# QinLab-WFU/CLIP-based-Cross-Modal-Hashing

Measured on AMD Instinct MI355X. Metric: image+text pairs/s encoded+hashed per GPU; mAP@K eval wallclock (64-bit), higher is better.
Workload: dtype bf16

## Files before the change

### clip-based-cross-modal-hashing_amd/cmh_native.py

```python
from __future__ import annotations

import ctypes as C
import os
import threading

import torch

_HERE = os.path.dirname(os.path.abspath(__file__))
LIB_PATH = os.environ.get("CMH_LIB") or os.path.join(_HERE, "csrc", "build", "libcmh.so")

ABI_VERSION = 6
F32, BF16, FP8 = 0, 1, 2
ACT_NONE, ACT_TANH, ACT_RELU = 0, 1, 2
TIE_REFERENCE, TIE_STABLE = 0, 1


class NativeError(RuntimeError):
    pass


class BlockWeights(C.Structure):
    _fields_ = [(n, C.c_void_p) for n in (
        "in_proj_w", "in_proj_b", "out_proj_w", "out_proj_b", "ln1_w", "ln1_b", "ln2_w", "ln2_b",
        "fc_w", "fc_b", "proj_w", "proj_b",
        "in_proj_cs", "out_proj_cs", "fc_cs", "proj_cs")] + [("act_scale", C.c_float * 4)]


class GemmProblem(C.Structure):
    _fields_ = [("x", C.c_void_p), ("w", C.c_void_p), ("bias", C.c_void_p), ("residual", C.c_void_p), ("out", C.c_void_p),
                ("M", C.c_int32), ("N", C.c_int32), ("K", C.c_int32), ("m_dev", C.c_void_p), ("colscale", C.c_void_p),
                ("alpha", C.c_float), ("out_scale", C.c_float)]


class VitWeights(C.Structure):
    _fields_ = [("gemm_dtype", C.c_int32), ("resolution", C.c_int32), ("patch", C.c_int32),
                ("width", C.c_int32), ("layers", C.c_int32), ("embed_dim", C.c_int32),
                ("conv1_w", C.c_void_p), ("class_embedding", C.c_void_p),
                ("positional_embedding", C.c_void_p), ("ln_pre_w", C.c_void_p), ("ln_pre_b", C.c_void_p),
                ("ln_post_w", C.c_void_p), ("ln_post_b", C.c_void_p), ("proj_t", C.c_void_p),
                ("blocks", C.POINTER(BlockWeights))]


class TextWeights(C.Structure):
    _fields_ = [("gemm_dtype", C.c_int32), ("context_length", C.c_int32), ("vocab_size", C.c_int32),
                ("width", C.c_int32), ("layers", C.c_int32), ("embed_dim", C.c_int32),
                ("token_embedding", C.c_void_p), ("positional_embedding", C.c_void_p),
                ("ln_final_w", C.c_void_p), ("ln_final_b", C.c_void_p), ("text_projection_t", C.c_void_p),
                ("blocks", C.POINTER(BlockWeights))]


class BlockGrads(C.Structure):
    _fields_ = [(n, C.c_void_p) for n in (
        "in_proj_w", "in_proj_b", "out_proj_w", "out_proj_b", "ln1_w", "ln1_b", "ln2_w", "ln2_b",
        "fc_w", "fc_b", "proj_w", "proj_b")]


class VitGrads(C.Structure):
    _fields_ = [("conv1_w", C.c_void_p), ("class_embedding", C.c_void_p), ("positional_embedding", C.c_void_p),
                ("ln_pre_w", C.c_void_p), ("ln_pre_b", C.c_void_p), ("ln_post_w", C.c_void_p), ("ln_post_b", C.c_void_p),
                ("proj", C.c_void_p), ("blocks", C.POINTER(BlockGrads))]


class TextGrads(C.Structure):
    _fields_ = [("token_embedding", C.c_void_p), ("positional_embedding", C.c_void_p), ("ln_final_w", C.c_void_p),
                ("ln_final_b", C.c_void_p), ("text_projection", C.c_void_p), ("blocks", C.POINTER(BlockGrads))]


class AdamTensor(C.Structure):
    _fields_ = [("p", C.c_void_p), ("g", C.c_void_p), ("m", C.c_void_p), ("v", C.c_void_p), ("n", C.c_int64),
                ("lr", C.c_float), ("weight_decay", C.c_float), ("max_grad_norm", C.c_float), ("p_bf16", C.c_void_p)]


class Taps(C.Structure):
    _fields_ = [("ptrs", C.POINTER(C.c_void_p)), ("count", C.c_int32)]


_lib = None
_lock = threading.Lock()

_i32, _i64, _f, _p, _sz = C.c_int32, C.c_int64, C.c_float, C.c_void_p, C.c_size_t

SIGNATURES = {
    "cmh_last_error": (C.c_char_p, []),
    "cmh_version": (C.c_int, []),
    "cmh_vit_workspace_bytes": (_sz, [C.POINTER(VitWeights), _i32]),
    "cmh_text_workspace_bytes": (_sz, [C.POINTER(TextWeights), _i32, _i32]),
    "cmh_vit_encode": (C.c_int, [C.POINTER(VitWeights), _p, _i32, _p, _p, _sz, C.POINTER(Taps), _p]),
    "cmh_text_encode": (C.c_int, [C.POINTER(TextWeights), _p, _i32, _i32, _p, _p, _p, _sz, C.POINTER(Taps), _p]),
    "cmh_text_encode_packed": (C.c_int, [C.POINTER(TextWeights), _p, _i32, _i32, _p, _p, _p, _sz, _p]),
    "cmh_vit_calibrate_fp8": (C.c_int, [C.POINTER(VitWeights), _p, _i32, _p, _p, _p, _sz, _p]),
    "cmh_text_calibrate_fp8": (C.c_int, [C.POINTER(TextWeights), _p, _i32, _i32, _p, _p, _p, _sz, _p]),
    "cmh_linear_gemm": (C.c_int, [_i32, _p, _p, _p, _p, _p, _i32, _i32, _i32, _i32, _p]),
    "cmh_layernorm": (C.c_int, [_p, _p, _p, _p, _i32, _i32, _i32, _p]),
    "cmh_attention": (C.c_int, [_i32, _p, _p, _i32, _i32, _i32, _i32, _p, _p]),
    "cmh_gemm_tuning": (C.c_int, [_i32, _i32]),
    "cmh_set_pooled_tail": (C.c_int, [_i32]),
    "cmh_set_gemm_rows": (C.c_int, [_i32]),
    "cmh_set_gemm_grouped": (C.c_int, [_i32]),
    "cmh_set_gemm_lc": (C.c_int, [_i32]),
    "cmh_gemm_route": (C.c_int, [_i32] * 8),
    "cmh_gemm_plan": (C.c_int, [_i32, _i32, C.POINTER(_i32), C.POINTER(_i32), C.POINTER(_i32)]),
    "cmh_set_grad_stream16": (C.c_int, [_i32]),
    "cmh_set_text_token_packing": (C.c_int, [_i32]),
    "cmh_linear_gemm_grouped": (C.c_int, [_i32, C.POINTER(GemmProblem), C.POINTER(GemmProblem), _i32, _p]),
    "cmh_clip_encode_pair": (C.c_int, [C.POINTER(VitWeights), _p, C.POINTER(TextWeights), _p, _i32, _i32, _i32, _p, _p, _p, _p, _sz, _p, _sz, _p]),
    "cmh_clip_encode_pair2": (C.c_int, [C.POINTER(VitWeights), _p, _i32, _p, _i32, C.POINTER(TextWeights), _p, _i32, _i32, _p, _p, _p, _p, _sz, _p, _sz, _p]),
    "cmh_msl_workspace_bytes": (_sz, [_i32]),
    "cmh_msl_loss": (C.c_int, [_p, _p, _p, _i32, _i32, _i32, _p, _p, _sz, _p]),
    "cmh_msl_loss_backward": (C.c_int, [_p, _p, _p, _i32, _i32, _i32, _p, _p, _p, _p, _sz, _p]),
    "cmh_spl_workspace_bytes": (_sz, [_i32]),
    "cmh_spl_loss": (C.c_int, [_p, _p, _p, _i32, _i32, _i32, _f, _f, _p, _p, _sz, _p]),
    "cmh_spl_loss_backward": (C.c_int, [_p, _p, _p, _i32, _i32, _i32, _f, _f, _p, _p, _p, _p, _sz, _p]),
    "cmh_qmi_workspace_bytes": (_sz, [_i32]),
    "cmh_qmi_loss": (C.c_int, [_p, _p, _p, _i32, _i32, _i32, _f, _p, _p, _p, _sz, _p]),
    "cmh_qmi_loss_backward": (C.c_int, [_p, _p, _p, _i32, _i32, _i32, _f, _p, _p, _p, _p, _p, _sz, _p]),
    "cmh_fp8_quantize_weight": (C.c_int, [_p, _p, _p, _i32, _i32, _p]),
    "cmh_fp8_quantize": (C.c_int, [_p, _i32, _p, _i64, _f, _p]),
    "cmh_fp8_dequantize": (C.c_int, [_p, _p, _i64, _f, _p]),
    "cmh_amax": (C.c_int, [_p, _i32, _i64, _p, _p]),
    "cmh_linear_gemm_fp8": (C.c_int, [_p, _p, _p, _f, _p, _p, _p, _f, _i32, _i32, _i32, _i32, _p]),
    "cmh_prof_gemm_begin": (C.c_int, [_i32]),
    "cmh_prof_gemm_end": (C.c_int, [C.POINTER(C.c_double), C.POINTER(C.c_double), C.POINTER(C.c_int64)]),
    "cmh_prof_gemm_by_kernel": (C.c_int, [C.POINTER(C.c_double), C.POINTER(C.c_double), C.POINTER(C.c_int64)]),
    "cmh_cast_f32_to_bf16": (C.c_int, [_p, _p, _i64, _p]),
    "cmh_linear_act": (C.c_int, [_p, _p, _p, _p, _f, _i32, _p, _i32, _i32, _i32, _p]),
    "cmh_pair_softmax": (C.c_int, [_p, _p, _i32, _i32, _p]),
    "cmh_sign_codes": (C.c_int, [_p, _p, _i64, _p]),
    "cmh_pair_argmax_codes": (C.c_int, [_p, _p, _i32, _i32, _p]),
    "cmh_pack_codes": (C.c_int, [_p, _i64, _i32, _p, _p, _p, _p]),
    "cmh_unpack_codes": (C.c_int, [_p, _p, _i64, _i32, _p, _p]),
    "cmh_map_mean": (C.c_int, [_p, _i32, _p, _p]),
    "cmh_pack_labels": (C.c_int, [_p, _i64, _i32, _p, _p, _p]),
    "cmh_hamming_dist": (C.c_int, [_p, _p, _p, _p, _i32, _i64, _i32, _p, _p]),
    "cmh_calc_neighbor": (C.c_int, [_p, _p, _i32, _i32, _i32, _p, _p]),
    "cmh_map_workspace_bytes": (_sz, [_i32, _i64, _i32, _i32]),
    "cmh_hamming_map": (C.c_int, [_p, _p, _p, _p, _p, _p, _i32, _i64, _i32, _i32, _i64, _i32, _i32, _p, _p, _p,
                                  _p, _sz, _p]),
    "cmh_retrieval_workspace_bytes": (_sz, [_i32, _i64, _i32]),
    "cmh_hamming_hist": (C.c_int, [_p, _p, _p, _p, _p, _p, _i32, _i64, _i32, _i32, _p, _p, _sz, _p]),
    "cmh_hamming_topk": (C.c_int, [_p, _p, _p, _p, _p, _p, _i32, _i64, _i32, _i32, _i64, _p, _p, _p, _p, _p, _sz, _p]),
    "cmh_hamming_topk_graded": (C.c_int, [_p, _p, _p, _p, _p, _p, _i32, _i64, _i32, _i32, _i64, _p, _p, _p, _p, _p, _p, _sz, _p]),
    "cmh_label_overlap_workspace_bytes": (_sz, [_i32, _i64, _i32]),
    "cmh_label_overlap_hist": (C.c_int, [_p, _p, _i32, _i64, _i32, _p, _p, _sz, _p]),
    "cmh_loss_workspace_bytes": (_sz, [_i32, _i32, _i32]),
    "cmh_dsph_hyp_loss": (C.c_int, [_p, _p, _p, _p, _i32, _i32, _i32, _f, _f, _p, _p, _sz, _p]),
    "cmh_dchmt_loss": (C.c_int, [_p, _p, _p, _i32, _i32, _i32, _i32, _i32, _i32, _f, _f, _p, _p, _sz, _p]),
    "cmh_batchnorm1d_train": (C.c_int, [_p, _p, _p, _f, _p, _i32, _i32, _p]),
    "cmh_twdh_targets": (C.c_int, [_p, _p, _p, _p, _i32, _i32, _i32, _p]),
    "cmh_twdh_loss": (C.c_int, [_p, _p, _p, _i32, _i32, _p, _p, _sz, _p]),
    "cmh_dnph_loss": (C.c_int, [_p, _p, _p, _p, _p, _p, _p, _p, _i32, _i32, _i32, _f, _f, _p, _p, _sz, _p]),
    "cmh_vit_encode_tokens": (C.c_int, [C.POINTER(VitWeights), _p, _i32, _p, _p, _sz, _p]),
    "cmh_text_encode_tokens": (C.c_int, [C.POINTER(TextWeights), _p, _i32, _i32, _p, _p, _p, _p, _sz, _p]),
    "cmh_text_encode_tokens_packed": (C.c_int, [C.POINTER(TextWeights), _p, _i32, _i32, _p, _p, _p, _p, _sz, _p]),
    "cmh_blocks_workspace_bytes": (_sz, [_i32, _i32, _i32, _i32]),
    "cmh_transformer_blocks": (C.c_int, [C.POINTER(BlockWeights), _i32, _i32, _p, _i32, _i32, _i32, _i32, _p, _p, _sz, _p]),
    "cmh_mith_lta": (C.c_int, [_p, _p, _p, _p, _i32, _i32, _i32, _i32, _i32, _i32, _i32, _p]),
    "cmh_add_positional": (C.c_int, [_p, _p, _i32, _i32, _i32, _p]),
    "cmh_bitwise_hash": (C.c_int, [_p, _p, _p, _p, _i32, _i32, _i32, _p]),
    "cmh_l2_normalize_rows": (C.c_int, [_p, _p, _i32, _i32, _p]),
    "cmh_mith_mix": (C.c_int, [_p, _p, _p, _p, _f, _p, _p, _p, _i64, _p]),
    "cmh_sq_diff_sum": (C.c_int, [_p, _p, _i64, _p, _p, _sz, _p]),
    "cmh_mith_bayesian_loss": (C.c_int, [_p, _p, _p, _p, _i32, _i32, _i32, _i32, _p, _p, _sz, _p]),
    "cmh_info_nce": (C.c_int, [_p, _p, _i32, _i32, _i32, _f, _p, _p, _sz, _p]),
    "cmh_transpose": (C.c_int, [_p, _i32, _p, _i32, _i32, _i32, _p]),
    "cmh_colsum_workspace_bytes": (_sz, [_i32, _i32]),
    "cmh_colsum": (C.c_int, [_p, _i32, _i32, _i32, _p, _p, _sz, _p]),
    "cmh_layernorm_backward_workspace_bytes": (_sz, [_i32, _i32]),
    "cmh_layernorm_backward": (C.c_int, [_p, _i32, _p, _i32, _p, _i32, _i32, _p, _i32, _p, _p, _p, _sz, _p]),
    "cmh_quick_gelu": (C.c_int, [_p, _p, _i64, _i32, _p]),
    "cmh_attention_backward": (C.c_int, [_i32, _p, _p, _p, _p, _i32, _i32, _i32, _i32, _p, _p]),
    "cmh_linear_wgrad_workspace_bytes": (_sz, [_i32, _i32, _i32, _i32]),
    "cmh_linear_wgrad": (C.c_int, [_i32, _p, _i32, _p, _i32, _i32, _i32, _i32, _p, _p, _p, _sz, _p]),
    "cmh_linear_act_backward": (C.c_int, [_p, _p, _p, _p, _p, _f, _i32, _p, _p, _p, _i32, _i32, _i32, _p, _sz, _p]),
    "cmh_head_backward_workspace_bytes": (_sz, [_i32, _i32, _i32]),
    "cmh_pair_softmax_backward": (C.c_int, [_p, _p, _p, _i32, _i32, _p]),
    "cmh_dchmt_loss_backward": (C.c_int, [_p, _p, _p, _i32, _i32, _i32, _i32, _i32, _i32, _f, _f, _p, _p, _p, _p, _sz, _p]),
    "cmh_dsph_hyp_loss_backward": (C.c_int, [_p, _p, _p, _p, _i32, _i32, _i32, _f, _f, _p, _p, _p, _p, _p, _sz, _p]),
    "cmh_dnph_backward_workspace_bytes": (_sz, [_i32, _i32, _i32]),
    "cmh_dnph_loss_backward": (C.c_int, [_p] * 8 + [_i32, _i32, _i32, _f, _f, _p] + [_p] * 5 + [_p, _sz, _p]),
    "cmh_image_preprocess_workspace_bytes": (_sz, [_i32, _i32, _i32, _i32]),
    "cmh_image_preprocess": (C.c_int, [_p, _p, _p, _i32, _i32, _i32, _i32, _i32, C.POINTER(C.c_float), C.POINTER(C.c_float),
                                       _p, _p, _p, _sz, _p]),
    "cmh_vit_forward_train_tokens": (C.c_int, [C.POINTER(VitWeights), _p, _i32, _p, _p, _sz, _p]),
    "cmh_vit_backward_tokens": (C.c_int, [C.POINTER(VitWeights), _i32, _p, C.POINTER(VitGrads), _p, _sz, _p]),
    "cmh_text_forward_train_tokens": (C.c_int, [C.POINTER(TextWeights), _p, _i32, _i32, _p, _p, _p, _p, _sz, _p]),
    "cmh_text_forward_train_tokens_packed": (C.c_int, [C.POINTER(TextWeights), _p, _i32, _i32, _p, _p, _p, _p, _sz, _p]),
    "cmh_text_backward_tokens": (C.c_int, [C.POINTER(TextWeights), _p, _i32, _i32, _p, _p, C.POINTER(TextGrads), _p, _sz, _p]),
    "cmh_blocks_train_bytes": (_sz, [_i32, _i32, _i32, _i32, _i32]),
    "cmh_blocks_forward_train": (C.c_int, [C.POINTER(BlockWeights), _i32, _i32, _p, _p, _i32, _i32, _i32, _p, _sz, _p]),
    "cmh_blocks_backward": (C.c_int, [C.POINTER(BlockWeights), C.POINTER(BlockGrads), _i32, _i32, _p, _p, _i32, _i32, _i32, _p, _sz, _p]),
    "cmh_mith_lta_backward": (C.c_int, [_p, _p, _p, _p, _i32, _i32, _i32, _i32, _i32, _i32, _i32, _p]),
    "cmh_gelu": (C.c_int, [_p, _p, C.c_int64, _p]),
    "cmh_gelu_backward": (C.c_int, [_p, _p, _p, C.c_int64, _p]),
    "cmh_l2_normalize_backward": (C.c_int, [_p, _p, _p, _i32, _i32, _p]),
    "cmh_bitwise_hash_backward": (C.c_int, [_p, _p, _p, _p, _p, _p, _p, _i32, _i32, _i32, _p]),
    "cmh_mith_bayesian_backward_workspace_bytes": (_sz, [_i32, _i32]),
    "cmh_info_nce_workspace_bytes": (_sz, [_i32, _i32]),
    "cmh_mith_bayesian_loss_backward": (C.c_int, [_p, _p, _p, _p, _i32, _i32, _i32, _i32, _p, _p, _p, _sz, _p]),
    "cmh_info_nce_backward": (C.c_int, [_p, _p, _i32, _i32, _i32, _f, _p, _p, _p, _p, _sz, _p]),
    "cmh_sq_diff_sum_backward": (C.c_int, [_p, _p, C.c_int64, _p, _p, _p, _p]),
    "cmh_batchnorm1d_update_running": (C.c_int, [_p, _f, _p, _p, _i32, _i32, _p]),
    "cmh_batchnorm1d_backward": (C.c_int, [_p, _p, _f, _p, _p, _p, _p, _i32, _i32, _p]),
    "cmh_twdh_loss_backward": (C.c_int, [_p, _p, _p, _i32, _i32, _p, _p, _p, _p, _p]),
    "cmh_image_normalize": (C.c_int, [_p, _p, _i32, _i32, C.POINTER(C.c_float), C.POINTER(C.c_float), _p, _p]),
    "cmh_bpe_create": (C.c_int, [C.c_char_p, _sz, C.POINTER(_p)]),
    "cmh_bpe_destroy": (None, [_p]),
    "cmh_bpe_vocab_size": (_i32, [_p]),
    "cmh_bpe_encode_captions": (C.c_int, [_p, C.c_char_p, _p, _i32, _i32, _p, _p, _i32]),
    "cmh_vit_train_bytes": (_sz, [C.POINTER(VitWeights), _i32]),
    "cmh_vit_forward_train": (C.c_int, [C.POINTER(VitWeights), _p, _i32, _p, _p, _sz, _p]),
    "cmh_vit_backward": (C.c_int, [C.POINTER(VitWeights), _i32, _p, C.POINTER(VitGrads), _p, _sz, _p]),
    "cmh_vit_backward_part": (C.c_int, [C.POINTER(VitWeights), _i32, _p, C.POINTER(VitGrads), _p, _sz, _i32, _i32, _p]),
    "cmh_text_train_bytes": (_sz, [C.POINTER(TextWeights), _i32, _i32]),
    "cmh_text_forward_train": (C.c_int, [C.POINTER(TextWeights), _p, _i32, _i32, _p, _p, _p, _sz, _p]),
    "cmh_text_backward": (C.c_int, [C.POINTER(TextWeights), _p, _i32, _i32, _p, _p, C.POINTER(TextGrads), _p, _sz, _p]),
    "cmh_text_backward_part": (C.c_int, [C.POINTER(TextWeights), _p, _i32, _i32, _p, _p, C.POINTER(TextGrads), _p, _sz, _i32, _i32, _p]),
    "cmh_bert_adam_workspace_bytes": (_sz, [_i32, _i64]),
    "cmh_bert_adam_step": (C.c_int, [C.POINTER(AdamTensor), _i32, C.c_double, C.c_double, C.c_double, _p, _sz, _p]),
}


def lib():
    global _lib
    with _lock:
        if _lib is None:
            if not os.path.exists(LIB_PATH):
                raise NativeError(
                    f"{LIB_PATH} is missing: build it with `python __graft_entry__.py` (or `make -C "
                    f"{os.path.dirname(os.path.dirname(LIB_PATH))}`); there is no CPU fallback for the hot path")
            l = C.CDLL(LIB_PATH)
            for name, (res, args) in SIGNATURES.items():
                fn = getattr(l, name)
                fn.restype, fn.argtypes = res, args
            if l.cmh_version() != ABI_VERSION:
                raise NativeError(f"{LIB_PATH}: cmh_version() = {l.cmh_version()}, this binding was written for {ABI_VERSION}; rebuild it")
            _lib = l
    return _lib


def check(rc: int, what: str):
    if rc != 0:
        raise NativeError(f"{what} failed (code {rc}): {lib().cmh_last_error().decode(errors='replace')}")


def require_gpu(*tensors):
    for t in tensors:
        if t is not None and not t.is_cuda:
            raise NativeError("libcmh runs on the GPU only (tensor on %s); there is no CPU fallback" % t.device)


def ptr(t):
    return None if t is None else C.c_void_p(t.data_ptr())


def stream_ptr(device=None):
    return C.c_void_p(torch.cuda.current_stream(device).cuda_stream)


_ws_cache: dict = {}


def workspace(nbytes: int, device, tag: str = "") -> torch.Tensor:
    key = (str(device), int(torch.cuda.current_stream(device).cuda_stream) if torch.cuda.is_available() else 0, tag)
    buf = _ws_cache.get(key)
    if buf is None or buf.numel() < nbytes:
        buf = torch.empty(max(int(nbytes), 256), dtype=torch.uint8, device=device)
        _ws_cache[key] = buf
    return buf


def f32c(t: torch.Tensor) -> torch.Tensor:
    if t.dtype != torch.float32:
        t = t.float()
    return t.contiguous()


def cast_bf16(src: torch.Tensor) -> torch.Tensor:
    src = f32c(src)
    require_gpu(src)
    dst = torch.empty(src.shape, dtype=torch.bfloat16, device=src.device)
    check(lib().cmh_cast_f32_to_bf16(ptr(src), ptr(dst), src.numel(), stream_ptr(src.device)), "cmh_cast_f32_to_bf16")
    return dst


def _kind(t: torch.Tensor) -> int:
    return {torch.float32: 0, torch.bfloat16: 1, torch.float16: 2}[t.dtype]


def fp8_quantize_weight(w: torch.Tensor):
    w = f32c(w)
    require_gpu(w)
    Nn, K = w.shape
    q = torch.empty(Nn, K, dtype=torch.uint8, device=w.device)
    cs = torch.empty(Nn, dtype=torch.float32, device=w.device)
    check(lib().cmh_fp8_quantize_weight(ptr(w), ptr(q), ptr(cs), Nn, K, stream_ptr(w.device)), "cmh_fp8_quantize_weight")
    return q, cs


def fp8_quantize(x: torch.Tensor, scale: float) -> torch.Tensor:
    require_gpu(x)
    x = x.contiguous()
    q = torch.empty(x.shape, dtype=torch.uint8, device=x.device)
    check(lib().cmh_fp8_quantize(ptr(x), _kind(x), ptr(q), x.numel(), float(scale), stream_ptr(x.device)), "cmh_fp8_quantize")
    return q


def fp8_dequantize(q: torch.Tensor, scale: float = 1.0) -> torch.Tensor:
    require_gpu(q)
    q = q.contiguous()
    out = torch.empty(q.shape, dtype=torch.float32, device=q.device)
    check(lib().cmh_fp8_dequantize(ptr(q), ptr(out), q.numel(), float(scale), stream_ptr(q.device)), "cmh_fp8_dequantize")
    return out


def amax(x: torch.Tensor, into: torch.Tensor | None = None) -> torch.Tensor:
    require_gpu(x)
    x = x.contiguous()
    out = torch.zeros(1, dtype=torch.float32, device=x.device) if into is None else into
    check(lib().cmh_amax(ptr(x), _kind(x), x.numel(), ptr(out), stream_ptr(x.device)), "cmh_amax")
    return out


EPI_OUT_FP8 = 4096


def linear_gemm_fp8(x8, w8, colscale, alpha, bias=None, residual=None, quickgelu=False, out="f32", out_scale=1.0):
    require_gpu(x8, w8, colscale, bias, residual)
    if x8.dtype != torch.uint8 or w8.dtype != torch.uint8:
        raise NativeError("linear_gemm_fp8: operands are e4m3 bytes (uint8 tensors)")
    x8, w8 = x8.contiguous(), w8.contiguous()
    M, K = x8.shape
    Nn = w8.shape[0]
    if w8.shape[1] != K or colscale.numel() != Nn or (bias is not None and bias.numel() != Nn) or \
            (residual is not None and tuple(residual.shape) != (M, Nn)):
        raise NativeError(f"linear_gemm_fp8: x {tuple(x8.shape)}, w {tuple(w8.shape)}, colscale / bias / residual shapes do not fit together")
    odt = {"f32": torch.float32, "bf16": torch.bfloat16, "f16": torch.float16, "fp8": torch.uint8}[out]
    o = torch.empty(M, Nn, dtype=odt, device=x8.device)
    res_f16 = residual is not None and residual.dtype == torch.float16
    if residual is not None:
        residual = residual.contiguous() if res_f16 else f32c(residual)
    epi = (EPI_BIAS if bias is not None else 0) | (EPI_QUICKGELU if quickgelu else 0) | (EPI_RESIDUAL if residual is not None else 0) | \
          (EPI_RES_F16 if res_f16 else 0) | {"f32": 0, "bf16": EPI_OUT_BF16, "f16": EPI_OUT_F16, "fp8": EPI_OUT_FP8}[out]
    check(lib().cmh_linear_gemm_fp8(ptr(x8), ptr(w8), ptr(f32c(colscale)), float(alpha), ptr(None if bias is None else f32c(bias)),
                                    ptr(residual), ptr(o), float(out_scale), M, Nn, K, epi, stream_ptr(x8.device)), "cmh_linear_gemm_fp8")
    return o


def set_gemm_grouped(on: int = -1):
    check(lib().cmh_set_gemm_grouped(int(on)), "cmh_set_gemm_grouped")


def linear_gemm_grouped(problems, quickgelu=False, out="f32", m_dev=(None, None)):
    assert len(problems) == 2
    kinds = {("u8" if p["x"].dtype == torch.uint8 else ("bf16" if p["x"].dtype == torch.bfloat16 else "f32")) for p in problems}
    if len(kinds) != 1:
        raise NativeError("linear_gemm_grouped: both problems must share the operand type")
    kind = kinds.pop()
    dt = {"f32": F32, "bf16": BF16, "u8": FP8}[kind]
    odt = {"f32": torch.float32, "bf16": torch.bfloat16, "f16": torch.float16, "fp8": torch.uint8}[out]
    has_bias = problems[0].get("bias") is not None
    has_res = problems[0].get("residual") is not None
    res_f16 = has_res and problems[0]["residual"].dtype == torch.float16
    epi = (EPI_BIAS if has_bias else 0) | (EPI_QUICKGELU if quickgelu else 0) | (EPI_RESIDUAL if has_res else 0) | \
          (EPI_RES_F16 if res_f16 else 0) | {"f32": 0, "bf16": EPI_OUT_BF16, "f16": EPI_OUT_F16, "fp8": EPI_OUT_FP8}[out]
    structs, outs, keep = [], [], []
    for p, md in zip(problems, m_dev):
        x, w = p["x"].contiguous(), p["w"].contiguous()
        require_gpu(x, w, p.get("bias"), p.get("residual"), p.get("colscale"), md)
        M, K = x.shape
        Nn = w.shape[0]
        if w.shape[1] != K or (p.get("bias") is not None) != has_bias or (p.get("residual") is not None) != has_res or \
                (has_bias and p["bias"].numel() != Nn) or (has_res and tuple(p["residual"].shape) != (M, Nn)) or \
                (kind == "u8" and (p.get("colscale") is None or p["colscale"].numel() != Nn)):
            raise NativeError(f"linear_gemm_grouped: x {tuple(x.shape)}, w {tuple(w.shape)}: operand shapes / kinds do not fit together")
        o = torch.empty(M, Nn, dtype=odt, device=x.device)
        bias = f32c(p["bias"]) if has_bias else None
        res = None
        if has_res:
            res = p["residual"].contiguous() if res_f16 else f32c(p["residual"])
        cs = f32c(p["colscale"]) if kind == "u8" else None
        g = GemmProblem(ptr(x), ptr(w), ptr(bias), ptr(res), ptr(o), M, Nn, K, ptr(md), ptr(cs), float(p.get("alpha", 1.0)),
                        float(p.get("out_scale", 1.0)))
        structs.append(g)
        outs.append(o)
        keep += [x, w, bias, res, cs]
    check(lib().cmh_linear_gemm_grouped(dt, C.byref(structs[0]), C.byref(structs[1]), epi, stream_ptr(outs[0].device)),
          "cmh_linear_gemm_grouped")
    return outs


def set_pooled_tail(on: bool):
    check(lib().cmh_set_pooled_tail(1 if on else 0), "cmh_set_pooled_tail")


def set_gemm_rows(on: int = -1):
    check(lib().cmh_set_gemm_rows(int(on)), "cmh_set_gemm_rows")


def set_text_token_packing(on: int):
    check(lib().cmh_set_text_token_packing(int(on)), "cmh_set_text_token_packing")


def set_grad_stream16(on: int):
    check(lib().cmh_set_grad_stream16(int(on)), "cmh_set_grad_stream16")


def set_gemm_lc(mode: int):
    check(lib().cmh_set_gemm_lc(int(mode)), "cmh_set_gemm_lc")


def gemm_route(a, b=None, epi=0, dt=None):
    mb, nb, kb = b if b is not None else (0, 0, 0)
    rc = lib().cmh_gemm_route(BF16 if dt is None else dt, *a, mb, nb, kb, int(epi))
    if rc < 0:
        raise NativeError(f"cmh_gemm_route: {lib().cmh_last_error()}")
    return rc


PLAN_FIELDS = ("family", "rows", "grid", "order", "dge", "res", "grouped")


def gemm_plan(a, b=None, epi=0, dt=None):
    def five(s):
        return (_i32 * 5)(*(tuple(s) + (0, 0))[:5])
    out = (_i32 * 16)()
    check(lib().cmh_gemm_plan(BF16 if dt is None else dt, int(epi), five(a), None if b is None else five(b), out), "cmh_gemm_plan")
    return out[1], [dict(zip(PLAN_FIELDS, out[2 + 7 * i:9 + 7 * i])) for i in range(out[0])]


def gemm_tuning(tile_rows: int = -1, order_group: int = -1):
    check(lib().cmh_gemm_tuning(int(tile_rows), int(order_group)), "cmh_gemm_tuning")


def prof_gemm_begin(max_launches: int):
    check(lib().cmh_prof_gemm_begin(int(max_launches)), "cmh_prof_gemm_begin")


def prof_gemm_end():
    ms, fl, n = C.c_double(), C.c_double(), C.c_int64()
    check(lib().cmh_prof_gemm_end(C.byref(ms), C.byref(fl), C.byref(n)), "cmh_prof_gemm_end")
    return ms.value, fl.value, n.value


def prof_gemm_by_kernel():
    ms, fl, n = (C.c_double * 3)(), (C.c_double * 3)(), (C.c_int64 * 3)()
    check(lib().cmh_prof_gemm_by_kernel(ms, fl, n), "cmh_prof_gemm_by_kernel")
    return {k: (ms[i], fl[i], n[i]) for i, k in enumerate(("gemm_wide_kernel", "gemm_rows_kernel", "fallback"))}


EPI_BIAS, EPI_QUICKGELU, EPI_RESIDUAL, EPI_OUT_BF16 = 1, 2, 4, 8
EPI_RES_F16, EPI_OUT_F16 = 64, 128


def linear_gemm(x, w, bias=None, residual=None, quickgelu=False, out_bf16=False, out_f16=False):
    require_gpu(x, w, bias, residual)
    dt = BF16 if x.dtype == torch.bfloat16 else F32
    if (w.dtype == torch.bfloat16) != (dt == BF16):
        raise NativeError("linear_gemm: x and w must share a dtype")
    if out_bf16 and out_f16:
        raise NativeError("linear_gemm: out_bf16 and out_f16 exclude each other")
    x, w = x.contiguous(), w.contiguous()
    M, K = x.shape
    Nn = w.shape[0]
    if w.dim() != 2 or w.shape[1] != K or (bias is not None and bias.numel() != Nn) or \
            (residual is not None and tuple(residual.shape) != (M, Nn)):
        raise NativeError(f"linear_gemm: x {tuple(x.shape)}, w {tuple(w.shape)}, bias / residual shapes do not fit together")
    odt = torch.bfloat16 if out_bf16 else (torch.float16 if out_f16 else torch.float32)
    out = torch.empty(M, Nn, dtype=odt, device=x.device)
    res_f16 = residual is not None and residual.dtype == torch.float16
    if residual is not None:
        residual = residual.contiguous() if res_f16 else f32c(residual)
    epi = (EPI_BIAS if bias is not None else 0) | (EPI_QUICKGELU if quickgelu else 0) | \
          (EPI_RESIDUAL if residual is not None else 0) | (EPI_OUT_BF16 if out_bf16 else 0) | \
          (EPI_RES_F16 if res_f16 else 0) | (EPI_OUT_F16 if out_f16 else 0)
    check(lib().cmh_linear_gemm(dt, ptr(x), ptr(w), ptr(None if bias is None else f32c(bias)), ptr(residual), ptr(out),
                                M, Nn, K, epi, stream_ptr(x.device)), "cmh_linear_gemm")
    return out


def layernorm(x, w, b, out_bf16=False):
    x, w, b = f32c(x), f32c(w), f32c(b)
    require_gpu(x, w, b)
    M, d = x.shape
    if w.numel() != d or b.numel() != d:
        raise NativeError(f"layernorm: rows of {d} elements, weight {tuple(w.shape)}, bias {tuple(b.shape)}")
    out = torch.empty(M, d, dtype=torch.bfloat16 if out_bf16 else torch.float32, device=x.device)
    check(lib().cmh_layernorm(ptr(x), ptr(w), ptr(b), ptr(out), BF16 if out_bf16 else F32, M, d, stream_ptr(x.device)),
          "cmh_layernorm")
    return out


def attention(qkv, B, T, causal, key_padding_mask=None):
    require_gpu(qkv, key_padding_mask)
    qkv = qkv.contiguous()
    dt = BF16 if qkv.dtype == torch.bfloat16 else F32
    d = qkv.shape[1] // 3
    o = torch.empty(B * T, d, dtype=qkv.dtype, device=qkv.device)
    kpm = None if key_padding_mask is None else key_padding_mask.to(torch.uint8).contiguous()
    check(lib().cmh_attention(dt, ptr(qkv), ptr(o), B, T, d, int(bool(causal)), ptr(kpm), stream_ptr(qkv.device)),
          "cmh_attention")
    return o


def linear_act(x, w, b, act=ACT_NONE, drop_mask=None, p=0.2):
    x, w = f32c(x), f32c(w)
    b = None if b is None else f32c(b)
    require_gpu(x, w, b, drop_mask)
    M, K = x.shape
    N = w.shape[0]
    if w.shape[1] != K:
        raise NativeError(f"linear_act: x [{M},{K}] vs w {tuple(w.shape)}")
    y = torch.empty(M, N, dtype=torch.float32, device=x.device)
    dm = None if drop_mask is None else f32c(drop_mask)
    check(lib().cmh_linear_act(ptr(x), ptr(w), ptr(b), ptr(dm), 1.0 / (1.0 - p), act, ptr(y), M, N, K,
                               stream_ptr(x.device)), "cmh_linear_act")
    return y


def pair_softmax(z):
    z = f32c(z)
    require_gpu(z)
    M, K2 = z.shape
    out = torch.empty_like(z)
    check(lib().cmh_pair_softmax(ptr(z), ptr(out), M, K2 // 2, stream_ptr(z.device)), "cmh_pair_softmax")
    return out


def sign_codes(h):
    h = f32c(h)
    require_gpu(h)
    out = torch.empty_like(h)
    check(lib().cmh_sign_codes(ptr(h), ptr(out), h.numel(), stream_ptr(h.device)), "cmh_sign_codes")
    return out


def pair_argmax_codes(p):
    p = f32c(p)
    require_gpu(p)
    M, K2 = p.shape
    out = torch.empty(M, K2 // 2, dtype=torch.float32, device=p.device)
    check(lib().cmh_pair_argmax_codes(ptr(p), ptr(out), M, K2 // 2, stream_ptr(p.device)), "cmh_pair_argmax_codes")
    return out


def pack_codes(codes, validate=True):
    codes = f32c(codes)
    require_gpu(codes)
    n, K = codes.shape
    W = (K + 31) // 32
    sp = torch.empty(n, W, dtype=torch.int32, device=codes.device)
    nz = torch.empty(n, W, dtype=torch.int32, device=codes.device)
    bad = torch.zeros(1, dtype=torch.int32, device=codes.device)
    check(lib().cmh_pack_codes(ptr(codes), n, K, ptr(sp), ptr(nz), ptr(bad), stream_ptr(codes.device)), "cmh_pack_codes")
    if validate and int(bad.item()):
        raise NativeError("pack_codes: hash codes must be exactly -1, 0 or +1 (sign()/argmax codes)")
    return sp, nz


def unpack_codes(sign_plane, nz_plane, bits: int):
    require_gpu(sign_plane, nz_plane)
    sp, nz = sign_plane.contiguous(), nz_plane.contiguous()
    n, W = sp.shape
    if sp.dtype != torch.int32 or nz.dtype != torch.int32 or tuple(nz.shape) != (n, W) or W != (int(bits) + 31) // 32:
        raise NativeError(f"unpack_codes: planes {tuple(sp.shape)} / {tuple(nz.shape)} do not hold {bits}-bit codes")
    out = torch.empty(n, int(bits), dtype=torch.float32, device=sp.device)
    if n:
        check(lib().cmh_unpack_codes(ptr(sp), ptr(nz), n, int(bits), ptr(out), stream_ptr(sp.device)), "cmh_unpack_codes")
    return out


def map_mean(ap):
    ap = f32c(ap)
    require_gpu(ap)
    out = torch.empty(1, dtype=torch.float32, device=ap.device)
    check(lib().cmh_map_mean(ptr(ap), ap.numel(), ptr(out), stream_ptr(ap.device)), "cmh_map_mean")
    return out[0]


def pack_labels(labels):
    labels = f32c(labels)
    require_gpu(labels)
    n, Cn = labels.shape
    LW = (Cn + 31) // 32
    out = torch.empty(n, LW, dtype=torch.int32, device=labels.device)
    bad = torch.zeros(1, dtype=torch.int32, device=labels.device)
    check(lib().cmh_pack_labels(ptr(labels), n, Cn, ptr(out), ptr(bad), stream_ptr(labels.device)), "cmh_pack_labels")
    if int(bad.item()):
        raise NativeError("pack_labels: labels must be non-negative (multi-hot)")
    return out


def hamming_dist(q_planes, r_planes, bits):
    (qs, qn), (rs, rn) = q_planes, r_planes
    Q, N = qs.shape[0], rs.shape[0]
    W = (bits + 31) // 32
    fit("hamming_dist", (qs, (Q, W)), (qn, (Q, W)), (rs, (N, W)), (rn, (N, W)))
    out = torch.empty(Q, N, dtype=torch.float32, device=qs.device)
    check(lib().cmh_hamming_dist(ptr(qs), ptr(qn), ptr(rs), ptr(rn), Q, N, bits, ptr(out), stream_ptr(qs.device)),
          "cmh_hamming_dist")
    return out


def calc_neighbor(la, lb, classes):
    A, B = la.shape[0], lb.shape[0]
    fit("calc_neighbor", (la, (A, (classes + 31) // 32)), (lb, (B, (classes + 31) // 32)))
    out = torch.empty(A, B, dtype=torch.float32, device=la.device)
    check(lib().cmh_calc_neighbor(ptr(la), ptr(lb), A, B, classes, ptr(out), stream_ptr(la.device)), "cmh_calc_neighbor")
    return out


def hamming_map(q_planes, q_lab, r_planes, r_lab, bits, classes, topk=None, tie_order=TIE_REFERENCE,
                want_perm=False, depth_limit=-1):
    (qs, qn), (rs, rn) = q_planes, r_planes
    dev = qs.device
    Q, N = qs.shape[0], rs.shape[0]
    W, LW = (bits + 31) // 32, (classes + 31) // 32
    fit("hamming_map", (qs, (Q, W)), (qn, (Q, W)), (rs, (N, W)), (rn, (N, W)), (q_lab, (Q, LW)), (r_lab, (N, LW)))
    ap = torch.empty(Q, dtype=torch.float32, device=dev)
    mp = torch.empty(1, dtype=torch.float32, device=dev)
    perm = torch.empty(Q, N, dtype=torch.int32, device=dev) if want_perm else None
    need = lib().cmh_map_workspace_bytes(Q, N, bits, tie_order)
    ws = workspace(need, dev, "map")
    check(lib().cmh_hamming_map(ptr(qs), ptr(qn), ptr(q_lab), ptr(rs), ptr(rn), ptr(r_lab), Q, N, bits, classes,
                                0 if topk is None else int(topk), tie_order, depth_limit, ptr(ap), ptr(mp), ptr(perm),
                                ptr(ws), ws.numel(), stream_ptr(dev)), "cmh_hamming_map")
    return mp[0], ap, perm


def _retrieval_operands(what, q_planes, r_planes, bits, q_lab, r_lab):
    (qs, qn), (rs, rn) = q_planes, r_planes
    require_gpu(qs, qn, rs, rn, q_lab, r_lab)
    Q, N = qs.shape[0], rs.shape[0]
    W = (int(bits) + 31) // 32
    if (q_lab is None) != (r_lab is None):
        raise NativeError(f"{what}: labels on one side only")
    LW = 0 if q_lab is None else q_lab.shape[1]
    fit(what, (qs, (Q, W)), (qn, (Q, W)), (rs, (N, W)), (rn, (N, W)), (q_lab, (Q, LW)), (r_lab, (N, LW)))
    for t in (qs, qn, rs, rn, q_lab, r_lab):
        if t is not None and (t.dtype != torch.int32 or not t.is_contiguous()):
            raise NativeError(f"{what}: packed operands are contiguous int32 tensors (pack_codes / pack_labels)")
    return qs, qn, rs, rn, Q, N, LW


def hamming_hist(q_planes, r_planes, bits, q_lab=None, r_lab=None):
    qs, qn, rs, rn, Q, N, LW = _retrieval_operands("hamming_hist", q_planes, r_planes, bits, q_lab, r_lab)
    dev = qs.device
    counts = torch.empty(Q, 2 * int(bits) + 1, 2, dtype=torch.int32, device=dev)
    ws = workspace(lib().cmh_retrieval_workspace_bytes(Q, N, int(bits)), dev, "retrieval")
    check(lib().cmh_hamming_hist(ptr(qs), ptr(qn), ptr(q_lab), ptr(rs), ptr(rn), ptr(r_lab), Q, N, int(bits), 32 * LW,
                                 ptr(counts), ptr(ws), ws.numel(), stream_ptr(dev)), "cmh_hamming_hist")
    return counts


def hamming_topk(q_planes, r_planes, bits, k, q_lab=None, r_lab=None, want_counts=False):
    qs, qn, rs, rn, Q, N, LW = _retrieval_operands("hamming_topk", q_planes, r_planes, bits, q_lab, r_lab)
    dev = qs.device
    k = int(k)
    if not 1 <= k <= N:
        raise NativeError(f"hamming_topk: k={k} outside [1, N={N}]")
    idx = torch.empty(Q, k, dtype=torch.int32, device=dev)
    dist = torch.empty(Q, k, dtype=torch.float32, device=dev)
    rel = torch.empty(Q, k, dtype=torch.uint8, device=dev) if LW else None
    counts = torch.empty(Q, 2 * int(bits) + 1, 2, dtype=torch.int32, device=dev) if want_counts else None
    ws = workspace(lib().cmh_retrieval_workspace_bytes(Q, N, int(bits)), dev, "retrieval")
    check(lib().cmh_hamming_topk(ptr(qs), ptr(qn), ptr(q_lab), ptr(rs), ptr(rn), ptr(r_lab), Q, N, int(bits), 32 * LW, k,
                                 ptr(idx), ptr(dist), ptr(rel), ptr(counts), ptr(ws), ws.numel(), stream_ptr(dev)),
          "cmh_hamming_topk")
    return (idx, dist, rel, counts) if want_counts else (idx, dist, rel)


GRADE_CLASSES_MAX = 255


def _grade_classes(what, classes, LW):
    classes = min(32 * LW, GRADE_CLASSES_MAX) if classes is None else int(classes)
    if classes < 1 or (classes + 31) // 32 != LW:
        raise NativeError(f"{what}: classes={classes} does not fit label operands of {LW} words")
    return classes


def hamming_topk_graded(q_planes, r_planes, bits, k, q_lab, r_lab, want_counts=False, classes=None):
    if q_lab is None or r_lab is None:
        raise NativeError("hamming_topk_graded: needs the labels of both sides")
    qs, qn, rs, rn, Q, N, LW = _retrieval_operands("hamming_topk_graded", q_planes, r_planes, bits, q_lab, r_lab)
    dev = qs.device
    k = int(k)
    if not 1 <= k <= N:
        raise NativeError(f"hamming_topk_graded: k={k} outside [1, N={N}]")
    classes = _grade_classes("hamming_topk_graded", classes, LW)
    idx = torch.empty(Q, k, dtype=torch.int32, device=dev)
    dist = torch.empty(Q, k, dtype=torch.float32, device=dev)
    grade = torch.empty(Q, k, dtype=torch.uint8, device=dev)
    counts = torch.empty(Q, 2 * int(bits) + 1, 2, dtype=torch.int32, device=dev) if want_counts else None
    ws = workspace(lib().cmh_retrieval_workspace_bytes(Q, N, int(bits)), dev, "retrieval")
    check(lib().cmh_hamming_topk_graded(ptr(qs), ptr(qn), ptr(q_lab), ptr(rs), ptr(rn), ptr(r_lab), Q, N, int(bits), classes, k,
                                        ptr(idx), ptr(dist), None, ptr(grade), ptr(counts), ptr(ws), ws.numel(), stream_ptr(dev)),
          "cmh_hamming_topk_graded")
    return (idx, dist, grade, counts) if want_counts else (idx, dist, grade)


def label_overlap_hist(q_lab, r_lab, classes):
    if q_lab is None or r_lab is None:
        raise NativeError("label_overlap_hist: needs the labels of both sides")
    require_gpu(q_lab, r_lab)
    classes = int(classes)
    Q, N, LW = q_lab.shape[0], r_lab.shape[0], (classes + 31) // 32
    fit("label_overlap_hist", (q_lab, (Q, LW)), (r_lab, (N, LW)))
    for t in (q_lab, r_lab):
        if t.dtype != torch.int32 or not t.is_contiguous():
            raise NativeError("label_overlap_hist: packed operands are contiguous int32 tensors (pack_labels)")
    dev = q_lab.device
    out = torch.empty(Q, classes + 1, dtype=torch.int32, device=dev)
    ws = workspace(lib().cmh_label_overlap_workspace_bytes(Q, N, classes), dev, "retrieval")
    check(lib().cmh_label_overlap_hist(ptr(q_lab), ptr(r_lab), Q, N, classes, ptr(out), ptr(ws), ws.numel(), stream_ptr(dev)),
          "cmh_label_overlap_hist")
    return out


def fit(what, *pairs):
    for t, shape in pairs:
        if t is not None and tuple(t.shape) != tuple(shape):
            raise NativeError(f"{what}: operand of shape {tuple(t.shape)} where {tuple(shape)} is expected")


def dsph_hyp_loss(x, y, label, proxies, threshold, alpha):
    x, y, label, proxies = f32c(x), f32c(y), f32c(label), f32c(proxies)
    require_gpu(x, y, label, proxies)
    B, K = x.shape
    Cn = label.shape[1]
    fit("dsph_hyp_loss", (y, (B, K)), (label, (B, Cn)), (proxies, (Cn, K)))
    out = torch.empty(1, dtype=torch.float32, device=x.device)
    ws = workspace(lib().cmh_loss_workspace_bytes(B, K, Cn), x.device, "loss")
    check(lib().cmh_dsph_hyp_loss(ptr(x), ptr(y), ptr(label), ptr(proxies), B, K, Cn, float(threshold), float(alpha),
                                  ptr(out), ptr(ws), ws.numel(), stream_ptr(x.device)), "cmh_dsph_hyp_loss")
    return out[0]


def msl_loss(feats, labels, feat2=None):
    feats, labels = f32c(feats), f32c(labels)
    feat2 = None if feat2 is None else f32c(feat2)
    require_gpu(feats, labels, feat2)
    B, K = feats.shape
    fit("msl_loss", (labels, (B, labels.shape[1])))
    if feat2 is not None:
        fit("msl_loss", (feat2, (B, K)))
    out = torch.empty(1, dtype=torch.float32, device=feats.device)
    ws = workspace(lib().cmh_msl_workspace_bytes(B), feats.device, "loss")
    check(lib().cmh_msl_loss(ptr(feats), ptr(feat2), ptr(labels), B, K, labels.shape[1], ptr(out), ptr(ws), ws.numel(),
                             stream_ptr(feats.device)), "cmh_msl_loss")
    return out[0]


def msl_loss_backward(feats, labels, feat2, dloss):
    B, K = feats.shape
    dfeats = torch.empty_like(feats)
    dfeat2 = None if feat2 is None else torch.empty_like(feat2)
    ws = workspace(lib().cmh_msl_workspace_bytes(B), feats.device, "loss")
    check(lib().cmh_msl_loss_backward(ptr(feats), ptr(feat2), ptr(labels), B, K, labels.shape[1], ptr(f32c(dloss).reshape(1)),
                                      ptr(dfeats), ptr(dfeat2), ptr(ws), ws.numel(), stream_ptr(feats.device)), "cmh_msl_loss_backward")
    return dfeats, dfeat2


def spl_loss(a, b, labels, temperature, delta):
    a, labels = f32c(a), f32c(labels)
    b = None if b is None else f32c(b)
    require_gpu(a, labels, b)
    B, K = a.shape
    fit("spl_loss", (labels, (B, labels.shape[1])), (b, (B, K)))
    out = torch.empty(1, dtype=torch.float32, device=a.device)
    ws = workspace(lib().cmh_spl_workspace_bytes(B), a.device, "loss")
    check(lib().cmh_spl_loss(ptr(a), ptr(b), ptr(labels), B, K, labels.shape[1], float(temperature), float(delta), ptr(out), ptr(ws),
                             ws.numel(), stream_ptr(a.device)), "cmh_spl_loss")
    return out[0]


def spl_loss_backward(a, b, labels, temperature, delta, dloss):
    B, K = a.shape
    da = torch.empty_like(a)
    db = None if b is None else torch.empty_like(b)
    ws = workspace(lib().cmh_spl_workspace_bytes(B), a.device, "loss")
    check(lib().cmh_spl_loss_backward(ptr(a), ptr(b), ptr(labels), B, K, labels.shape[1], float(temperature), float(delta),
                                      ptr(f32c(dloss).reshape(1)), ptr(da), ptr(db), ptr(ws), ws.numel(), stream_ptr(a.device)),
          "cmh_spl_loss_backward")
    return da, db


def qmi_loss(img, txt, label, eps=1e-8):
    img, txt, label = f32c(img), f32c(txt), f32c(label)
    require_gpu(img, txt, label)
    B, K = img.shape
    Cn = label.shape[1]
    fit("qmi_loss", (txt, (B, K)), (label, (B, Cn)))
    packed = pack_labels(label)
    out = torch.empty(1, dtype=torch.float32, device=img.device)
    sum_d = torch.empty(1, dtype=torch.float32, device=img.device)
    ws = workspace(lib().cmh_qmi_workspace_bytes(B), img.device, "loss")
    check(lib().cmh_qmi_loss(ptr(img), ptr(txt), ptr(packed), B, K, Cn, float(eps), ptr(out), ptr(sum_d), ptr(ws), ws.numel(),
                             stream_ptr(img.device)), "cmh_qmi_loss")
    return out[0], sum_d, packed


def qmi_loss_backward(img, txt, packed, classes, sum_d, dloss, eps=1e-8):
    B, K = img.shape
    dimg, dtxt = torch.empty_like(img), torch.empty_like(txt)
    ws = workspace(lib().cmh_qmi_workspace_bytes(B), img.device, "loss")
    check(lib().cmh_qmi_loss_backward(ptr(img), ptr(txt), ptr(packed), B, K, int(classes), float(eps), ptr(sum_d), ptr(f32c(dloss).reshape(1)),
# ... 93 lines not shown
```

### clip-based-cross-modal-hashing_amd/csrc/attention.hip

```cpp
#include "cmh_common.h"

namespace cmh {

constexpr int HD = 64;
constexpr int KT = 32;

template <typename T>
__device__ __forceinline__ void load_row64(const T* __restrict__ p, float (&dst)[HD], float scale);

template <>
__device__ __forceinline__ void load_row64<float>(const float* __restrict__ p, float (&dst)[HD], float scale) {
#pragma unroll
  for (int i = 0; i < HD / 4; ++i) {
    const float4 v = *reinterpret_cast<const float4*>(p + 4 * i);
    dst[4 * i + 0] = v.x * scale; dst[4 * i + 1] = v.y * scale;
    dst[4 * i + 2] = v.z * scale; dst[4 * i + 3] = v.w * scale;
  }
}
template <>
__device__ __forceinline__ void load_row64<bf16_t>(const bf16_t* __restrict__ p, float (&dst)[HD], float scale) {
#pragma unroll
  for (int i = 0; i < HD / 8; ++i) {
    const uint4 v = *reinterpret_cast<const uint4*>(p + 8 * i);
    const uint32_t w[4] = {v.x, v.y, v.z, v.w};
#pragma unroll
    for (int j = 0; j < 4; ++j) {
      dst[8 * i + 2 * j + 0] = __uint_as_float(w[j] << 16) * scale;
      dst[8 * i + 2 * j + 1] = __uint_as_float(w[j] & 0xffff0000u) * scale;
    }
  }
}

template <typename T>
__global__ __launch_bounds__(64) void attention_kernel(const T* __restrict__ qkv, T* __restrict__ o, int B, int Tmax,
                                                       int d, int causal, const uint8_t* __restrict__ kpm,
                                                       const int32_t* __restrict__ seq_off) {
  __shared__ __attribute__((aligned(16))) float sK[KT][HD];
  __shared__ __attribute__((aligned(16))) float sV[KT][HD];

  const int lane = threadIdx.x;
  const int heads = d / HD;
  const int b = blockIdx.x / heads, h = blockIdx.x - b * heads;
  const int Tn = seq_off ? seq_off[b + 1] - seq_off[b] : Tmax;
  const size_t srow = seq_off ? static_cast<size_t>(seq_off[b]) : static_cast<size_t>(b) * Tmax;
  const int q0 = blockIdx.y * 64;
  const int row = q0 + lane;
  const bool active = row < Tn;
  const size_t ld = static_cast<size_t>(3) * d;
  const T* base = qkv + srow * ld + h * HD;

  float q[HD], acc[HD];
#pragma unroll
  for (int i = 0; i < HD; ++i) acc[i] = 0.f;
  if (active) {
    load_row64<T>(base + static_cast<size_t>(row) * ld, q, 0.125f);
  } else {
#pragma unroll
    for (int i = 0; i < HD; ++i) q[i] = 0.f;
  }
  float m = -1e30f, l = 0.f;

  const int last_row = (q0 + 63 < Tn ? q0 + 63 : Tn - 1);
  const int k_end = causal ? last_row + 1 : Tn;

  for (int k0 = 0; k0 < k_end; k0 += KT) {
    __syncthreads();
#pragma unroll
    for (int it = 0; it < KT * HD / 4 / 64; ++it) {
      const int slot = it * 64 + lane;
      const int kr = slot >> 4, c4 = slot & 15;
      const int kg = k0 + kr;
      float4 kv = float4{0.f, 0.f, 0.f, 0.f}, vv = kv;
      if (kg < Tn) {
        const T* kp = base + static_cast<size_t>(kg) * ld + d + c4 * 4;
        const T* vp = kp + d;
        if constexpr (sizeof(T) == 4) {
          kv = *reinterpret_cast<const float4*>(kp);
          vv = *reinterpret_cast<const float4*>(vp);
        } else {
          const uint2 a = *reinterpret_cast<const uint2*>(kp);
          const uint2 c = *reinterpret_cast<const uint2*>(vp);
          kv = float4{__uint_as_float(a.x << 16), __uint_as_float(a.x & 0xffff0000u),
                      __uint_as_float(a.y << 16), __uint_as_float(a.y & 0xffff0000u)};
          vv = float4{__uint_as_float(c.x << 16), __uint_as_float(c.x & 0xffff0000u),
                      __uint_as_float(c.y << 16), __uint_as_float(c.y & 0xffff0000u)};
        }
      }
      *reinterpret_cast<float4*>(&sK[kr][c4 * 4]) = kv;
      *reinterpret_cast<float4*>(&sV[kr][c4 * 4]) = vv;
    }
    __syncthreads();

    float s[KT];
    float tmax = -1e30f;
#pragma unroll
    for (int j = 0; j < KT; ++j) {
      float a0 = 0.f, a1 = 0.f, a2 = 0.f, a3 = 0.f;
#pragma unroll
      for (int i = 0; i < HD / 4; ++i) {
        const float4 kv = *reinterpret_cast<const float4*>(&sK[j][4 * i]);
        a0 = fmaf(q[4 * i + 0], kv.x, a0);
        a1 = fmaf(q[4 * i + 1], kv.y, a1);
        a2 = fmaf(q[4 * i + 2], kv.z, a2);
        a3 = fmaf(q[4 * i + 3], kv.w, a3);
      }
      const int kg = k0 + j;
      bool ok = kg < Tn && (!causal || kg <= row);
      if (kpm && kg < Tn) ok = ok && (kpm[static_cast<size_t>(b) * Tmax + kg] == 0);
      s[j] = ok ? (a0 + a1) + (a2 + a3) : -1e30f;
      tmax = fmaxf(tmax, s[j]);
    }
    const float m_new = fmaxf(m, tmax);
    const float alpha = expf(m - m_new);
    l *= alpha;
#pragma unroll
    for (int i = 0; i < HD; ++i) acc[i] *= alpha;
#pragma unroll
    for (int j = 0; j < KT; ++j) {
      const float p = s[j] > -1e29f ? expf(s[j] - m_new) : 0.f;
      l += p;
#pragma unroll
      for (int i = 0; i < HD / 4; ++i) {
        const float4 vv = *reinterpret_cast<const float4*>(&sV[j][4 * i]);
        acc[4 * i + 0] = fmaf(p, vv.x, acc[4 * i + 0]);
        acc[4 * i + 1] = fmaf(p, vv.y, acc[4 * i + 1]);
        acc[4 * i + 2] = fmaf(p, vv.z, acc[4 * i + 2]);
        acc[4 * i + 3] = fmaf(p, vv.w, acc[4 * i + 3]);
      }
    }
    m = m_new;
  }

  if (!active) return;
  const float inv = 1.0f / l;
  T* op = o + (srow + row) * d + h * HD;
  if constexpr (sizeof(T) == 4) {
#pragma unroll
    for (int i = 0; i < HD / 4; ++i)
      *reinterpret_cast<float4*>(op + 4 * i) =
          float4{acc[4 * i] * inv, acc[4 * i + 1] * inv, acc[4 * i + 2] * inv, acc[4 * i + 3] * inv};
  } else {
#pragma unroll
    for (int i = 0; i < HD / 8; ++i) {
      uint4 pk;
      uint32_t w[4];
#pragma unroll
      for (int j = 0; j < 4; ++j)
        w[j] = static_cast<uint32_t>(f32_to_bf16(acc[8 * i + 2 * j] * inv)) |
               (static_cast<uint32_t>(f32_to_bf16(acc[8 * i + 2 * j + 1] * inv)) << 16);
      pk.x = w[0]; pk.y = w[1]; pk.z = w[2]; pk.w = w[3];
      *reinterpret_cast<uint4*>(op + 8 * i) = pk;
    }
  }
}

typedef __attribute__((ext_vector_type(8))) __bf16 abf16x8_t;
typedef __attribute__((ext_vector_type(4))) float af32x4_t;

constexpr int kAttnVST = 80;

template <int NKT>
__device__ __forceinline__ void attention_mfma_body(const bf16_t* __restrict__ qkv, bf16_t* __restrict__ o, int Tmax, int d, int causal,
                                                    const uint8_t* __restrict__ kpm, const int32_t* __restrict__ seq_off,
                                                    float o8_inv_scale, int block, bf16_t* sV) {
  constexpr int NKS = NKT / 2;
  constexpr int TP = NKT * 16;
  constexpr int VST = kAttnVST;

  const int lane = threadIdx.x, g = lane >> 4, c = lane & 15;
  const int heads = d / HD;
  const int b = block / heads, h = block - b * heads;
  const int Tn = seq_off ? __builtin_amdgcn_readfirstlane(seq_off[b + 1] - seq_off[b]) : Tmax;
  const size_t srow = seq_off ? static_cast<size_t>(__builtin_amdgcn_readfirstlane(seq_off[b])) : static_cast<size_t>(b) * Tmax;
  const size_t ld = static_cast<size_t>(3) * d;
  const bf16_t* base = qkv + srow * ld + h * HD;
  if (Tn <= 0) return;

  abf16x8_t kf[NKT][2];
#pragma unroll
  for (int kt = 0; kt < NKT; ++kt) {
    int row = kt * 16 + c;
    row = row < Tn ? row : Tn - 1;
#pragma unroll
    for (int s = 0; s < 2; ++s)
      kf[kt][s] = *reinterpret_cast<const abf16x8_t*>(base + static_cast<size_t>(row) * ld + d + s * 32 + g * 8);
  }
  constexpr int VIT = TP * 8 / 64;
  constexpr int VB = NKT == 8 ? 8 : VIT;
  uint4 vst[VB];
  auto load_v = [&](int i0) {
#pragma unroll
    for (int i = 0; i < VB; ++i) {
      const int slot = lane + 64 * (i0 + i), row = slot >> 3, ch = slot & 7;
      const int rc = row < Tn ? row : Tn - 1;
      vst[i] = *reinterpret_cast<const uint4*>(base + static_cast<size_t>(rc) * ld + 2 * d + ch * 8);
    }
  };
  auto store_v = [&](int i0) {
#pragma unroll
    for (int i = 0; i < VB; ++i) {
      const int slot = lane + 64 * (i0 + i), row = slot >> 3, ch = slot & 7;
      *reinterpret_cast<uint4*>(&sV[row * VST + ch * 8]) = row < Tn ? vst[i] : uint4{0u, 0u, 0u, 0u};
    }
  };
  load_v(0);
  uint32_t padded = 0;
  if (kpm) {
    uint8_t kb[NKT][4];
#pragma unroll
    for (int kt = 0; kt < NKT; ++kt)
#pragma unroll
      for (int r = 0; r < 4; ++r) {
        const int key = kt * 16 + 4 * g + r;
        kb[kt][r] = kpm[static_cast<size_t>(b) * Tmax + (key < Tn ? key : Tn - 1)];
      }
#pragma unroll
    for (int kt = 0; kt < NKT; ++kt)
#pragma unroll
      for (int r = 0; r < 4; ++r) padded |= (kb[kt][r] != 0 ? 1u : 0u) << (kt * 4 + r);
  }
  store_v(0);
  if constexpr (VB < VIT) { load_v(VB); store_v(VB); }
  uint32_t keyok = 0;
#pragma unroll
  for (int kt = 0; kt < NKT; ++kt)
#pragma unroll
    for (int r = 0; r < 4; ++r) {
      const int key = kt * 16 + 4 * g + r;
      const bool ok = key < Tn && !((padded >> (kt * 4 + r)) & 1u);
      keyok |= (ok ? 1u : 0u) << (kt * 4 + r);
    }
  uint32_t tile_all = 0, tile_none = 0;
#pragma unroll
  for (int kt = 0; kt < NKT; ++kt) {
    const uint32_t bits = (keyok >> (kt * 4)) & 15u;
    if (__ballot(bits != 15u) == 0) tile_all |= 1u << kt;
    if (__ballot(bits != 0u) == 0) tile_none |= 1u << kt;
  }
  uint32_t diagok = 0;
#pragma unroll
  for (int r = 0; r < 4; ++r) diagok |= (4 * g + r <= c ? 1u : 0u) << r;
  __syncthreads();
  abf16x8_t vf[NKS][4];
  {
    typedef __attribute__((address_space(3))) void* lptr_t;
    const uint32_t a0 = static_cast<uint32_t>(reinterpret_cast<uintptr_t>((lptr_t)sV)) +
                        static_cast<uint32_t>(((4 * g + (c >> 2)) * VST + 4 * (c & 3)) * 2);
    uint2 raw[NKS][4][2];
#pragma unroll
    for (int s = 0; s < NKS; ++s)
#pragma unroll
      for (int dt = 0; dt < 4; ++dt)
#pragma unroll
        for (int hh = 0; hh < 2; ++hh)
          asm volatile("ds_read_b64_tr_b16 %0, %1 offset:%2"
                       : "=v"(raw[s][dt][hh])
                       : "v"(a0), "i"((32 * s + 16 * hh) * VST * 2 + 32 * dt));
#pragma unroll
    for (int s = 0; s < NKS; ++s) {
      asm volatile("s_waitcnt lgkmcnt(0)"
                   : "+v"(raw[s][0][0]), "+v"(raw[s][0][1]), "+v"(raw[s][1][0]), "+v"(raw[s][1][1]), "+v"(raw[s][2][0]),
                     "+v"(raw[s][2][1]), "+v"(raw[s][3][0]), "+v"(raw[s][3][1]));
#pragma unroll
      for (int dt = 0; dt < 4; ++dt)
        vf[s][dt] = __builtin_bit_cast(abf16x8_t, uint4{raw[s][dt][0].x, raw[s][dt][0].y, raw[s][dt][1].x, raw[s][dt][1].y});
    }
  }

#if defined(ATT_ABL) && ATT_ABL == 3
  {
    float keep = 0.f;
#pragma unroll
    for (int s = 0; s < NKS; ++s)
#pragma unroll
      for (int dt = 0; dt < 4; ++dt) keep += static_cast<float>(vf[s][dt][0]);
#pragma unroll
    for (int kt = 0; kt < NKT; ++kt) keep += static_cast<float>(kf[kt][0][0]) + static_cast<float>(kf[kt][1][0]);
    if (keep == 123.456f) o[0] = 1;
    return;
  }
#endif
  const int nqt = (Tn + 15) >> 4;
  auto load_q = [&](int qt, abf16x8_t (&q)[2]) {
    const int qrow = qt * 16 + c;
    const int qr = qrow < Tn ? qrow : Tn - 1;
#pragma unroll
    for (int s = 0; s < 2; ++s) q[s] = *reinterpret_cast<const abf16x8_t*>(base + static_cast<size_t>(qr) * ld + s * 32 + g * 8);
  };
  abf16x8_t qn[2];
  load_q(0, qn);
  for (int qt = 0; qt < nqt; ++qt) {
    const int qrow = qt * 16 + c;
    abf16x8_t qf[2] = {qn[0], qn[1]};
    load_q(qt + 1, qn);
    af32x4_t sc[NKT];
#pragma unroll
    for (int kt = 0; kt < NKT; ++kt) {
      if ((causal && kt > qt) || ((tile_none >> kt) & 1u)) {
        sc[kt] = af32x4_t{-1e30f, -1e30f, -1e30f, -1e30f};
      } else {
        sc[kt] = af32x4_t{0.f, 0.f, 0.f, 0.f};
#pragma unroll
        for (int s = 0; s < 2; ++s) sc[kt] = __builtin_amdgcn_mfma_f32_16x16x32_bf16(kf[kt][s], qf[s], sc[kt], 0, 0, 0);
        uint32_t okb = (keyok >> (kt * 4)) & 15u;
        if (causal && kt == qt) okb &= diagok;
        if (!((tile_all >> kt) & 1u) || (causal && kt == qt)) {
#pragma unroll
          for (int r = 0; r < 4; ++r) sc[kt][r] = ((okb >> r) & 1u) ? sc[kt][r] : -1e30f;
        }
      }
    }
    float m = -1e30f;
#pragma unroll
    for (int kt = 0; kt < NKT; ++kt) m = fmaxf(fmaxf(m, fmaxf(sc[kt][0], sc[kt][1])), fmaxf(sc[kt][2], sc[kt][3]));
    m = fmaxf(m, __shfl_xor(m, 16, 64));
    m = fmaxf(m, __shfl_xor(m, 32, 64));
    typedef __attribute__((ext_vector_type(2))) float af32x2_t;
    const float kC = 0.18033688011112042f;
    const af32x2_t mc = {-m * kC, -m * kC}, cc = {kC, kC};
    af32x2_t l2 = {0.f, 0.f};
#pragma unroll
    for (int kt = 0; kt < NKT; ++kt)
#pragma unroll
      for (int r = 0; r < 4; r += 2) {
        const af32x2_t e = __builtin_elementwise_fma(af32x2_t{sc[kt][r], sc[kt][r + 1]}, cc, mc);
        const af32x2_t p = {__builtin_amdgcn_exp2f(e[0]), __builtin_amdgcn_exp2f(e[1])};
        sc[kt][r] = p[0];
        sc[kt][r + 1] = p[1];
        l2 += p;
      }
    float l = l2[0] + l2[1];
    l += __shfl_xor(l, 16, 64);
    l += __shfl_xor(l, 32, 64);
    l = m > -1e29f ? l : 0.f;
    af32x4_t oc[4];
#pragma unroll
    for (int dt = 0; dt < 4; ++dt) oc[dt] = af32x4_t{0.f, 0.f, 0.f, 0.f};
#pragma unroll
    for (int s = 0; s < NKS; ++s) {
      abf16x8_t pb;
#pragma unroll
      for (int j = 0; j < 8; ++j) pb[j] = static_cast<__bf16>(sc[2 * s + (j >> 2)][j & 3]);
#pragma unroll
      for (int dt = 0; dt < 4; ++dt) oc[dt] = __builtin_amdgcn_mfma_f32_16x16x32_bf16(vf[s][dt], pb, oc[dt], 0, 0, 0);
    }
#if defined(ATT_ABL) && (ATT_ABL == 1 || ATT_ABL == 2)
    {
      float keep = l;
#pragma unroll
      for (int dt = 0; dt < 4; ++dt) keep += oc[dt][0] + oc[dt][1] + oc[dt][2] + oc[dt][3];
      if (keep == 123.456f) o[0] = 1;
      continue;
    }
#endif
    if (qrow < Tn && o8_inv_scale > 0.f) {
      const float inv = o8_inv_scale / l;
      uint8_t* op8 = reinterpret_cast<uint8_t*>(o) + (srow + qrow) * d + h * HD + 4 * g;
#pragma unroll
      for (int dt = 0; dt < 4; ++dt) {
        auto cl = [](float v) { return fminf(fmaxf(v, -448.f), 448.f); };
        int w = __builtin_amdgcn_cvt_pk_fp8_f32(cl(oc[dt][0] * inv), cl(oc[dt][1] * inv), 0, false);
        w = __builtin_amdgcn_cvt_pk_fp8_f32(cl(oc[dt][2] * inv), cl(oc[dt][3] * inv), w, true);
        *reinterpret_cast<uint32_t*>(op8 + 16 * dt) = static_cast<uint32_t>(w);
      }
    } else {
      const float inv = 1.0f / l;
      bf16_t* op = o + (srow + (qrow < Tn ? qrow : Tn - 1)) * d + h * HD + (g & 1) * 16 + (g & 2) * 4;
#pragma unroll
      for (int pr = 0; pr < 2; ++pr) {
        uint32_t lo[2], hi[2];
#pragma unroll
        for (int w = 0; w < 2; ++w) {
          lo[w] = pack_bf16x2(oc[2 * pr][2 * w] * inv, oc[2 * pr][2 * w + 1] * inv);
          hi[w] = pack_bf16x2(oc[2 * pr + 1][2 * w] * inv, oc[2 * pr + 1][2 * w + 1] * inv);
        }
        typedef __attribute__((ext_vector_type(2))) unsigned au2_t;
        const au2_t s0 = __builtin_amdgcn_permlane16_swap(lo[0], hi[0], false, false);
        const au2_t s1 = __builtin_amdgcn_permlane16_swap(lo[1], hi[1], false, false);
        if (qrow < Tn) *reinterpret_cast<uint4*>(op + 32 * pr) = uint4{s0[0], s1[0], s0[1], s1[1]};
      }
    }
  }
}

template <int NKT>
__global__ __launch_bounds__(64) void attention_mfma_kernel(const bf16_t* __restrict__ qkv, bf16_t* __restrict__ o,
                                                            int B, int Tmax, int d, int causal,
                                                            const uint8_t* __restrict__ kpm,
                                                            const int32_t* __restrict__ seq_off, float o8_inv_scale) {
  __shared__ __attribute__((aligned(16))) bf16_t sV[NKT * 16 * kAttnVST];
  (void)B;
  attention_mfma_body<NKT>(qkv, o, Tmax, d, causal, kpm, seq_off, o8_inv_scale, blockIdx.x, sV);
}

template <int NKT>
static void launch_attention_mfma(const void* qkv, void* o, int B, int T, int d, int causal, const uint8_t* kpm,
                                  const int32_t* seq_off, hipStream_t st, float o8_inv_scale) {
  hipLaunchKernelGGL(attention_mfma_kernel<NKT>, dim3(B * (d / HD)), dim3(64), 0, st, static_cast<const bf16_t*>(qkv),
                     static_cast<bf16_t*>(o), B, T, d, causal, kpm, seq_off, o8_inv_scale);
}

int launch_attention(const void* qkv, void* o, int dt, int B, int T, int d, int causal,
                     const uint8_t* key_padding_mask, hipStream_t st) {
  return launch_attention_varlen(qkv, o, dt, B, T, d, causal, key_padding_mask, nullptr, st, 0.f);
}

int launch_attention_varlen(const void* qkv, void* o, int dt, int B, int T, int d, int causal,
                            const uint8_t* key_padding_mask, const int32_t* seq_off, hipStream_t st, float o8_inv_scale) {
  CMH_CHECK_ARG(d % HD == 0, "attention: width %d is not a multiple of 64", d);
  CMH_CHECK_ARG(B > 0 && T > 0, "attention: empty batch");
  CMH_CHECK_ARG(o8_inv_scale == 0.f || (dt == CMH_BF16 && T <= 128), "attention: e4m3 output needs bf16 qkv and T <= 128 (T=%d)", T);
  const dim3 grid(B * (d / HD), (T + 63) / 64);
  if (dt == CMH_BF16 && T <= 128) {
    if (T <= 32) launch_attention_mfma<2>(qkv, o, B, T, d, causal, key_padding_mask, seq_off, st, o8_inv_scale);
    else if (T <= 64) launch_attention_mfma<4>(qkv, o, B, T, d, causal, key_padding_mask, seq_off, st, o8_inv_scale);
    else if (T <= 96) launch_attention_mfma<6>(qkv, o, B, T, d, causal, key_padding_mask, seq_off, st, o8_inv_scale);
    else launch_attention_mfma<8>(qkv, o, B, T, d, causal, key_padding_mask, seq_off, st, o8_inv_scale);
    CMH_CHECK_LAUNCH("attention_mfma");
    return CMH_OK;
  }
  if (dt == CMH_F32)
    hipLaunchKernelGGL(attention_kernel<float>, grid, dim3(64), 0, st, static_cast<const float*>(qkv),
                       static_cast<float*>(o), B, T, d, causal, key_padding_mask, seq_off);
  else
    hipLaunchKernelGGL(attention_kernel<bf16_t>, grid, dim3(64), 0, st, static_cast<const bf16_t*>(qkv),
                       static_cast<bf16_t*>(o), B, T, d, causal, key_padding_mask, seq_off);
  CMH_CHECK_LAUNCH("attention");
  return CMH_OK;
}

}
```

### clip-based-cross-modal-hashing_amd/csrc/cmh_common.h

```cpp
#pragma once

#include <hip/hip_runtime.h>
#include <stdint.h>

#include <cstdarg>
#include <cstdio>

#include "../../include/cmh.h"

namespace cmh {

char* err_buf();
int fail(int code, const char* fmt, ...);

#define CMH_CHECK_ARG(cond, ...) \
  do {                           \
    if (!(cond)) return ::cmh::fail(CMH_ERR_INVALID, __VA_ARGS__); \
  } while (0)

#define CMH_CHECK_LAUNCH(what)                                                            \
  do {                                                                                    \
    hipError_t e__ = hipGetLastError();                                                   \
    if (e__ != hipSuccess)                                                                \
      return ::cmh::fail(CMH_ERR_LAUNCH, "%s: %s", what, hipGetErrorString(e__));          \
  } while (0)

static inline hipStream_t as_stream(void* s) { return reinterpret_cast<hipStream_t>(s); }
static inline size_t align_up(size_t x, size_t a) { return (x + a - 1) / a * a; }

typedef uint16_t bf16_t;

__device__ __forceinline__ float bf16_to_f32(bf16_t v) {
  return __uint_as_float(static_cast<uint32_t>(v) << 16);
}
__device__ __forceinline__ bf16_t f32_to_bf16(float f) {
  uint32_t u = __float_as_uint(f);
  if ((u & 0x7fffffffu) > 0x7f800000u) return static_cast<bf16_t>((u >> 16) | 0x40);
  u += 0x7fffu + ((u >> 16) & 1u);
  return static_cast<bf16_t>(u >> 16);
}

__device__ __forceinline__ uint32_t pack_bf16x2(float a, float b) {
  typedef __attribute__((ext_vector_type(2))) float f2_t;
  typedef __attribute__((ext_vector_type(2))) __bf16 b2_t;
  const f2_t v = {a, b};
  return __builtin_bit_cast(uint32_t, __builtin_convertvector(v, b2_t));
}

__device__ __forceinline__ uint32_t pack_f16x2(float a, float b) {
  typedef __attribute__((ext_vector_type(2))) float f2_t;
  typedef __attribute__((ext_vector_type(2))) _Float16 h2_t;
  const f2_t v = {a, b};
  return __builtin_bit_cast(uint32_t, __builtin_convertvector(v, h2_t));
}
__device__ __forceinline__ float f16lo_to_f32(uint32_t w) {
  typedef __attribute__((ext_vector_type(2))) _Float16 h2_t;
  return static_cast<float>(__builtin_bit_cast(h2_t, w)[0]);
}
__device__ __forceinline__ float f16hi_to_f32(uint32_t w) {
  typedef __attribute__((ext_vector_type(2))) _Float16 h2_t;
  return static_cast<float>(__builtin_bit_cast(h2_t, w)[1]);
}

constexpr int kF32 = 0, kBF16 = 1, kF16 = 2;

__device__ __forceinline__ float load_as_f32(const void* p, size_t i, int kind) {
  if (kind == kF32) return static_cast<const float*>(p)[i];
  const uint16_t h = static_cast<const uint16_t*>(p)[i];
  if (kind == kBF16) return bf16_to_f32(h);
  return static_cast<float>(__builtin_bit_cast(_Float16, h));
}
__device__ __forceinline__ void store_from_f32(void* p, size_t i, int kind, float v) {
  if (kind == kF32) static_cast<float*>(p)[i] = v;
  else if (kind == kBF16) static_cast<uint16_t*>(p)[i] = f32_to_bf16(v);
  else static_cast<uint16_t*>(p)[i] = __builtin_bit_cast(uint16_t, static_cast<_Float16>(v));
}

__device__ __forceinline__ float4 load4_as_f32(const void* p, size_t i, int kind) {
  if (kind == kF32) return *reinterpret_cast<const float4*>(static_cast<const float*>(p) + i);
  const uint2 u = *reinterpret_cast<const uint2*>(static_cast<const uint16_t*>(p) + i);
  if (kind == kBF16) return float4{__uint_as_float(u.x << 16), __uint_as_float(u.x & 0xffff0000u), __uint_as_float(u.y << 16),
                                   __uint_as_float(u.y & 0xffff0000u)};
  return float4{f16lo_to_f32(u.x), f16hi_to_f32(u.x), f16lo_to_f32(u.y), f16hi_to_f32(u.y)};
}
__device__ __forceinline__ void store4_from_f32(void* p, size_t i, int kind, float4 v) {
  if (kind == kF32) *reinterpret_cast<float4*>(static_cast<float*>(p) + i) = v;
  else if (kind == kBF16) *reinterpret_cast<uint2*>(static_cast<uint16_t*>(p) + i) = uint2{pack_bf16x2(v.x, v.y), pack_bf16x2(v.z, v.w)};
  else *reinterpret_cast<uint2*>(static_cast<uint16_t*>(p) + i) = uint2{pack_f16x2(v.x, v.y), pack_f16x2(v.z, v.w)};
}

enum : int {
  EPI_BIAS = 1,
  EPI_QUICKGELU = 2,
  EPI_RESIDUAL = 4,
  EPI_OUT_BF16 = 8,
  EPI_GELU = 16,
  EPI_RELU = 32,
  EPI_RES_F16 = 64,
  EPI_OUT_F16 = 128,
  EPI_MUL_DQGELU = 1024,
  EPI_SCALE = 2048,
  EPI_OUT_FP8 = 4096,
  EPI_SAVE_PRE = 8192
};

__device__ __forceinline__ float gelu_erf(float v) { return 0.5f * v * (1.0f + erff(v * 0.70710678118654752f)); }

bool gemm_wide_enabled();
struct GemmProblem {
  const void* A; const void* W; const float* bias; const float* residual; void* out;
  int M, N, K;
  const int32_t* m_dev; int m_hint;
  const float* colscale; float alpha, oscale;
};
int launch_gemm_grouped(int dt, const GemmProblem& a, const GemmProblem& b, int epi, hipStream_t st);
enum : int { GEMM_WIDE = 0, GEMM_ROWS = 1, GEMM_FALLBACK = 2, GEMM_LC = 3, GEMM_LC2 = 4, GEMM_LC3 = 5, GEMM_LC2Q = 6 };
struct GemmPlan {
  int launches;
  int family;
  int rows;
  int grid;
  int order;
  int res;
  bool dge;
  bool swap;
};
int plan_gemm(int dt, const GemmProblem& a, const GemmProblem* b, int epi, GemmPlan* p);
int gemm_cus();
int gemm_order_group(int N);
int launch_gemm_wide(int dt, const GemmProblem& a, const GemmProblem* b, int epi, const GemmPlan& p, hipStream_t st, hipEvent_t ev0,
                     hipEvent_t ev1);
int launch_gemm_lc(const GemmProblem& a, const GemmProblem* b, int epi, const GemmPlan& p, hipStream_t st, hipEvent_t ev0, hipEvent_t ev1);
int launch_gemm_lc2q(const GemmProblem& g, int epi, const GemmPlan& p, hipStream_t st, hipEvent_t ev0, hipEvent_t ev1);
int launch_gemm_rows(int dt, const GemmProblem& g, int epi, const GemmPlan& p, hipStream_t st, hipEvent_t ev0, hipEvent_t ev1);
int launch_gemm_glds(int dt, const GemmProblem& g, int epi, const GemmPlan& p, hipStream_t st);
bool gemm_wide_supported(int N);
int gemm_lc_mode();
bool gemm_lc_takes(int dt, int N, int K, int epi);
bool gemm_lc2q_takes(int N, int K, int epi);
bool gemm_rows_takes(int M, int N, int K, int epi);
int launch_gemm(int dt, const void* A, const void* W, const float* bias, const float* residual,
                void* out, int M, int N, int K, int epi, hipStream_t st, const int32_t* m_dev = nullptr, int m_hint = -1);
int launch_gemm_fp8(const void* A8, const void* W8, const float* colscale, float alpha, const float* bias, const float* residual,
                    void* out, float oscale, int M, int N, int K, int epi, hipStream_t st, const int32_t* m_dev = nullptr, int m_hint = -1);

bool gemm_wide_tn_supported(int Mm, int Nn, int Kd);
int launch_gemm_wide_tn(const void* Xk, const void* Wk, float* out, float* partials, size_t part_bytes, int Mm, int Nn, int Kd,
                        hipStream_t st, float* colsum_partial = nullptr, int* colsum_slices = nullptr);
struct TnMultiJob { const void* Xk; const void* Wk; float* out; float* colsum; int Mm, Nn, Kd; };
bool gemm_wide_tn_multi_enabled();
bool gemm_wide_tn_multi_fits(const TnMultiJob* jobs, int n);
int launch_gemm_wide_tn_multi(const TnMultiJob* jobs, int n, float* partials, size_t part_bytes, hipStream_t st, int* slices);

int launch_layernorm(const float* x, const int32_t* row_index, const float* w, const float* b,
                     void* out, int out_bf16, int M, int d, hipStream_t st);
int launch_layernorm_x(const void* x, int x_f16, const int32_t* row_index, const float* w, const float* b,
                       void* out, int out_bf16, int M, int d, hipStream_t st, const int32_t* m_dev = nullptr);

int launch_layernorm_h2b_pair(const void* x0, const float* w0, const float* b0, void* out0, int M0, int d0, const int32_t* md0,
                               const void* x1, const float* w1, const float* b1, void* out1, int M1, int d1, const int32_t* md1,
                               hipStream_t st);
static inline int conv1_k(int p, int dt) {
  const int pk = 3 * p * p, ks = dt == CMH_F32 ? 32 : 64;
  return p % 4 == 0 && pk % ks == 0 ? pk : static_cast<int>(align_up(static_cast<size_t>(pk), 256));
}
int launch_patchify(const float* image, void* patches, int dt, int B, int R, int p, int ld, hipStream_t st);
int launch_copy_cols(const void* src, int lds, void* dst, int ldd, int rows, int cols, int esz, hipStream_t st);
int launch_vit_assemble_lnpre(const float* patch_out, const float* cls, const float* pos,
                              const float* lnw, const float* lnb, void* x, int x_f16, int B, int g2, int d,
                              hipStream_t st);
int launch_text_embed(const int64_t* tokens, const float* tok_emb, const float* pos, void* x, int x_f16,
                      int32_t* eot_row, int B, int L, int d, int vocab, hipStream_t st);
int launch_text_pack_plan(const int64_t* tokens, int B, int L, int32_t* seq_off, hipStream_t st, const uint8_t* kpm = nullptr,
                          int32_t* eot_pos = nullptr);
int launch_text_embed_packed(const int64_t* tokens, const float* tok_emb, const float* pos, void* x, int x_f16, int32_t* eot_row,
                             int B, int L, int d, int vocab, const int32_t* seq_off, hipStream_t st, bool eot_is_pos = false);
bool text_token_packing();
int launch_unpack_token_rows(const float* packed, const int32_t* seq_off, float* dense, int B, int L, int E, const int32_t* eot_packed,
                             int32_t* eot_dense, hipStream_t st);
int launch_pack_token_rows(const float* dense, const int32_t* seq_off, float* packed, int B, int L, int E, hipStream_t st);
int launch_iota_rows(int32_t* rows, int B, int T, hipStream_t st);
int launch_scatter_rows(const void* src, const int32_t* rows, void* dst, int B, int row_bytes, hipStream_t st);
bool pooled_tail_enabled();
int launch_gather_rows2(const void* srcA, void* dstA, int bytesA, const void* srcB, void* dstB, int bytesB, const int32_t* rows, int B,
                        hipStream_t st);
int gemm_wide_splitk_plan(int dt, int M, int N, int K);
int launch_gemm_wide_splitk(int dt, const void* A, const void* W, float* out, float* partials, int S, int M, int N, int K,
                            hipStream_t st);
int launch_layernorm_any(const void* x, int x_kind, const int32_t* row_index, const float* w, const float* b, void* out,
                         int out_kind, int M, int d, hipStream_t st);
int launch_vit_assemble(const float* patch_out, const float* cls, const float* pos, float* x, int B, int g2, int d, hipStream_t st);
int launch_attention_backward(int dtype, const void* qkv, const void* o, const void* dout, void* dqkv, int B, int T, int d, int causal,
                              const uint8_t* key_padding_mask, const int32_t* seq_off, hipStream_t st);
int launch_transpose(const void* src, int skind, void* dst, int dkind, int rows, int cols, int dst_ld, hipStream_t st,
                     float* colsum_partial = nullptr);
bool transpose_is_vectorised(const void* src, const void* dst, int rows, int cols, int dst_ld);
int launch_transpose_multi(const void* const* src, void* const* dst, const int* R, const int* C, int n, int kind, hipStream_t st);
int launch_colsum_final(const float* partial, int slices, int cols, float* out, hipStream_t st);
struct FinalJobs {
  static constexpr int kMax = 8;
  int n = 0;
  const float* partial[kMax];
  int slices[kMax];
  int cols[kMax];
  float* out[kMax];
  void add(const float* p, int s, int c, float* o) { partial[n] = p; slices[n] = s; cols[n] = c; out[n] = o; ++n; }
};
int launch_final_jobs(FinalJobs& jobs, hipStream_t st);
int launch_colsum_partial(const void* x, int kind, int rows, int cols, float* partial, hipStream_t st);
int launch_layernorm_backward(const void* x, int x_kind, const void* dy, int dy_kind, const float* gamma, const int32_t* row_index,
                              int M, int d, float* dx, int accumulate, float* dgamma, float* dbeta, void* workspace,
                              size_t workspace_bytes, hipStream_t st, void* dx_bf16 = nullptr,
                              FinalJobs* defer = nullptr,
                              const void* acc16 = nullptr,
                              bool write_f32 = true);

int launch_attention(const void* qkv, void* o, int dt, int B, int T, int d, int causal,
                     const uint8_t* key_padding_mask, hipStream_t st);
int launch_attention_varlen(const void* qkv, void* o, int dt, int B, int T, int d, int causal,
                            const uint8_t* key_padding_mask, const int32_t* seq_off, hipStream_t st,
                            float o8_inv_scale = 0.f);
int launch_layernorm_q(const void* x_f16, const float* w, const float* b, void* out_fp8, float inv_scale, int M, int d, hipStream_t st,
                       const int32_t* m_dev = nullptr);
int launch_amax(const void* x, int kind, size_t n, float* out, hipStream_t st);

int launch_small_linear(int dt, const void* x, const void* w, const float* bias, const float* mask,
                        float keep_scale, int act, float* y, int M, int N, int K, hipStream_t st);

}
```

### clip-based-cross-modal-hashing_amd/csrc/encoder_blocks.h

```cpp
#pragma once

#include "cmh_common.h"

namespace cmh {

struct Arena {
  char* base;
  size_t off = 0;
  explicit Arena(void* p) : base(static_cast<char*>(p)) {}
  template <typename T = void> T* take(size_t bytes) {
    T* p = base ? reinterpret_cast<T*>(base + off) : nullptr;
    off += align_up(bytes, 256);
    return p;
  }
};

struct Lane {
  const cmh_block_weights* w = nullptr;
  int dtb = 0, xh = 0;
  int B = 0, T = 0, d = 0, causal = 0, M = 0;
  const uint8_t* kpm = nullptr;
  const int32_t* seq_off = nullptr;
  const int32_t* md = nullptr;
  int mh = -1;
  const void* x_in = nullptr;
  void *h1 = nullptr, *qkv = nullptr, *attn = nullptr, *x_mid = nullptr, *h2 = nullptr, *act = nullptr, *x_out = nullptr;
  float* amax = nullptr;
  void* pre = nullptr;
  const int32_t* pooled = nullptr;
  void* attn_p = nullptr;
};

int block_forward(const Lane& a, const Lane* b, hipStream_t st);

int resid_f16(int dt, int d);

int conv1_stem(const cmh_vit_weights* w, int dt, const float* image, const float* image_b, int batch_a, int B, void* patches,
               void* conv1_w_pad, float* patch_out, hipStream_t st);

int final_projection(int dt, const void* pool, const void* w_t, float* feat, int B, int embed, int d, hipStream_t st);

}
```

### clip-based-cross-modal-hashing_amd/csrc/encoders.hip

```cpp
#include <cstdlib>
#include <cstring>
#include <mutex>

#include "encoder_blocks.h"

namespace cmh {

static thread_local char g_err[512] = "";
char* err_buf() { return g_err; }
int fail(int code, const char* fmt, ...) {
  va_list ap;
  va_start(ap, fmt);
  vsnprintf(g_err, sizeof(g_err), fmt, ap);
  va_end(ap);
  return code;
}

struct TowerBufs {
  float* x;
  void* h;
  void* qkv;
  void* mlp;
  int32_t* rows;
  void* pool;
  int32_t* seq;
  void* conv1_w;
  size_t total;
};

static TowerBufs carve(void* ws, size_t M, size_t B, size_t d, size_t e, size_t extra_qkv, size_t extra_mlp, size_t conv1_w_bytes = 0) {
  Arena a(ws);
  TowerBufs t;
  t.x = a.take<float>(M * d * 4);
  t.h = a.take(M * d * e);
  size_t qkv_b = M * 3 * d * e, mlp_b = M * 4 * d * e;
  t.qkv = a.take(qkv_b > extra_qkv ? qkv_b : extra_qkv);
  t.mlp = a.take(mlp_b > extra_mlp ? mlp_b : extra_mlp);
  t.rows = a.take<int32_t>(B * 4);
  t.pool = a.take(B * d * e);
  t.seq = a.take<int32_t>((B + 2) * 4);
  t.conv1_w = a.take(conv1_w_bytes);
  t.total = a.off;
  return t;
}

static int tap(const cmh_taps* taps, int idx, const float* x, size_t bytes, hipStream_t st) {
  if (!taps || idx >= taps->count || !taps->ptrs[idx]) return CMH_OK;
  if (hipMemcpyAsync(taps->ptrs[idx], x, bytes, hipMemcpyDeviceToDevice, st) != hipSuccess)
    return fail(CMH_ERR_LAUNCH, "tap copy failed");
  return CMH_OK;
}

static int check_lane(const Lane& l) {
  CMH_CHECK_ARG(!l.amax || l.dtb == CMH_BF16, "fp8 calibration runs in bf16 mode");
  if (l.dtb != CMH_FP8) return CMH_OK;
  const cmh_block_weights& w = *l.w;
  const float* a = w.act_scale;
  CMH_CHECK_ARG(l.xh, "fp8 mode runs on the fp16 residual stream (width %% 256 == 0, no taps)");
  CMH_CHECK_ARG(w.in_proj_cs && w.out_proj_cs && w.fc_cs && w.proj_cs, "fp8 mode: weight scales missing");
  CMH_CHECK_ARG(a[0] > 0.f && a[1] > 0.f && a[2] > 0.f && a[3] > 0.f, "fp8 mode: activation scales missing (run the calibration pass)");
  return CMH_OK;
}

enum { OP_LN1 = 0, OP_ATTN = 1, OP_LN2 = 2, OP_ACT = 3 };
static float scale(const Lane& l, int i) { return l.w->act_scale[i]; }
static int amax_stage(const Lane& l, int i, const void* v, size_t n, hipStream_t st) {
  return l.amax ? launch_amax(v, kBF16, n, l.amax + i, st) : CMH_OK;
}

struct Rows { int M; const int32_t* md; int mh; };
static Rows head_rows(const Lane& l) { return Rows{l.M, l.md, l.mh}; }
static Rows tail_rows(const Lane& l) { return l.pooled ? Rows{l.B, nullptr, -1} : head_rows(l); }

struct LnArgs { const void* x; const float *g, *b; void* out; Rows r; };
static LnArgs ln_args(const Lane& l, int op) {
  if (op == OP_LN1) return LnArgs{l.x_in, l.w->ln1_w, l.w->ln1_b, l.h1, head_rows(l)};
  return LnArgs{l.x_mid, l.w->ln2_w, l.w->ln2_b, l.h2, tail_rows(l)};
}
static int ln_stage(const Lane* const* L, int n, int op, hipStream_t st) {
  const LnArgs p = ln_args(*L[0], op);
  int rc = 1;
  if (n == 2 && L[0]->dtb == CMH_BF16 && L[0]->xh && L[1]->xh) {
    const LnArgs q = ln_args(*L[1], op);
    rc = launch_layernorm_h2b_pair(p.x, p.g, p.b, p.out, p.r.M, L[0]->d, p.r.md, q.x, q.g, q.b, q.out, q.r.M, L[1]->d, q.r.md, st);
    if (rc < 0) return rc;
  }
  for (int i = 0; i < n; ++i) {
    const Lane& l = *L[i];
    const LnArgs a = i ? ln_args(l, op) : p;
    if (rc > 0) {
      const int r1 = l.dtb == CMH_FP8 ? launch_layernorm_q(a.x, a.g, a.b, a.out, 1.0f / scale(l, op), a.r.M, l.d, st, a.r.md)
                                      : launch_layernorm_x(a.x, l.xh, nullptr, a.g, a.b, a.out, l.dtb == CMH_BF16, a.r.M, l.d, st, a.r.md);
      if (r1) return r1;
    }
    if (int r2 = amax_stage(l, op, a.out, static_cast<size_t>(a.r.M) * l.d, st)) return r2;
  }
  return CMH_OK;
}

enum { G_IN_PROJ, G_OUT_PROJ, G_FC, G_PROJ };
static bool fc_pre_fused(const Lane& l) {
  static const bool fuse_act = []() { const char* e = getenv("CMH_FUSE_PRE"); return !(e && e[0] == '0'); }();
  return l.dtb == CMH_BF16 && (4 * l.d) % 256 == 0 && fuse_act;
}
static GemmProblem gemm_problem(const Lane& l, int which, int* epi) {
  const cmh_block_weights& w = *l.w;
  const bool q = l.dtb == CMH_FP8;
  const int d = l.d;
  const int obf = l.dtb == CMH_F32 ? 0 : EPI_OUT_BF16;
  const int rx = EPI_BIAS | EPI_RESIDUAL | (l.xh ? EPI_RES_F16 | EPI_OUT_F16 : 0);
  struct Row { const void* A; const void* W; const float* bias; const float* cs; const void* res; void* out; int N, K, op; float oscale; int epi; };
  const Row tab[4] = {
      {l.h1, w.in_proj_w, w.in_proj_b, w.in_proj_cs, nullptr, l.qkv, 3 * d, d, OP_LN1, 1.f, EPI_BIAS | obf},
      {l.pooled ? l.attn_p : l.attn, w.out_proj_w, w.out_proj_b, w.out_proj_cs, l.pooled ? l.x_mid : l.x_in, l.x_mid, d, d, OP_ATTN, 1.f, rx},
      {l.h2, w.fc_w, w.fc_b, w.fc_cs, nullptr, l.act, 4 * d, d, OP_LN2, q ? 1.0f / scale(l, OP_ACT) : 1.f,
       EPI_BIAS | EPI_QUICKGELU | (q ? EPI_OUT_FP8 : obf)},
      {l.act, w.proj_w, w.proj_b, w.proj_cs, l.x_mid, l.x_out, d, 4 * d, OP_ACT, 1.f, rx}};
  Row r = tab[which];
  if (which == G_FC && l.pre) {
    if (fc_pre_fused(l)) { r.res = l.pre; r.epi |= EPI_SAVE_PRE; }
    else { r.out = l.pre; r.epi &= ~EPI_QUICKGELU; }
  }
  const Rows m = which == G_IN_PROJ ? head_rows(l) : tail_rows(l);
  *epi = r.epi;
  return GemmProblem{r.A, r.W, r.bias, static_cast<const float*>(r.res), r.out, m.M, r.N, r.K, m.md, m.mh, q ? r.cs : nullptr,
                     q ? scale(l, r.op) : 1.f, r.oscale};
}
static int gemm_stage(const Lane* const* L, int n, int which, hipStream_t st) {
  int epi = 0, epi_b = 0;
  const GemmProblem p = gemm_problem(*L[0], which, &epi);
  if (n == 2) return launch_gemm_grouped(L[0]->dtb, p, gemm_problem(*L[1], which, &epi_b), epi, st);
  if (L[0]->dtb == CMH_FP8)
    return launch_gemm_fp8(p.A, p.W, p.colscale, p.alpha, p.bias, p.residual, p.out, p.oscale, p.M, p.N, p.K, epi, st, p.m_dev, p.m_hint);
  return launch_gemm(L[0]->dtb, p.A, p.W, p.bias, p.residual, p.out, p.M, p.N, p.K, epi, st, p.m_dev, p.m_hint);
}

static int block_tail(const Lane* const* L, int n, hipStream_t st) {
  int rc;
  for (int i = 0; i < n; ++i) {
    const Lane& l = *L[i];
    const int xe = l.xh ? 2 : 4, e = l.dtb == CMH_FP8 ? 1 : l.dtb == CMH_BF16 ? 2 : 4;
    if (l.pooled && (rc = launch_gather_rows2(l.x_in, l.x_mid, l.d * xe, l.attn, l.attn_p, l.d * e, l.pooled, l.B, st))) return rc;
  }
  if ((rc = gemm_stage(L, n, G_OUT_PROJ, st))) return rc;
  if ((rc = ln_stage(L, n, OP_LN2, st))) return rc;
  if ((rc = gemm_stage(L, n, G_FC, st))) return rc;
  for (int i = 0; i < n; ++i) {
    const Lane& l = *L[i];
    const size_t n_act = static_cast<size_t>(tail_rows(l).M) * 4 * l.d;
    if (l.pre && !fc_pre_fused(l) &&
        (rc = cmh_quick_gelu(l.pre, l.act, static_cast<int64_t>(n_act), l.dtb == CMH_BF16 ? kBF16 : kF32, st))) return rc;
    if ((rc = amax_stage(l, OP_ACT, l.act, n_act, st))) return rc;
  }
  return gemm_stage(L, n, G_PROJ, st);
}

int block_forward(const Lane& a, const Lane* b, hipStream_t st) {
  const Lane* const L[2] = {&a, b};
  const int n = b ? 2 : 1;
  int rc;
  for (int i = 0; i < n; ++i)
    if ((rc = check_lane(*L[i]))) return rc;
  CMH_CHECK_ARG(n == 1 || a.xh == b->xh,
                "block_forward: the towers' residual streams differ in kind (the caller runs such towers one by one)");
  if ((rc = ln_stage(L, n, OP_LN1, st))) return rc;
  if ((rc = gemm_stage(L, n, G_IN_PROJ, st))) return rc;
  for (int i = 0; i < n; ++i) {
    const Lane& l = *L[i];
    const bool q = l.dtb == CMH_FP8;
    if ((rc = launch_attention_varlen(l.qkv, l.attn, q ? CMH_BF16 : l.dtb, l.B, l.T, l.d, l.causal, l.kpm, l.seq_off, st,
                                      q ? 1.0f / scale(l, OP_ATTN) : 0.f))) return rc;
    if ((rc = amax_stage(l, OP_ATTN, l.attn, static_cast<size_t>(l.M) * l.d, st))) return rc;
  }
  if (n == 2 && (a.pooled || b->pooled)) {
    if ((rc = block_tail(&L[0], 1, st))) return rc;
    return block_tail(&L[1], 1, st);
  }
  return block_tail(L, n, st);
}

static int g_pooled_tail = -1;
bool pooled_tail_enabled() {
  static const bool env_on = []() { const char* e = getenv("CMH_POOLED_TAIL"); return !(e && !strcmp(e, "0")); }();
  return g_pooled_tail < 0 ? env_on : g_pooled_tail != 0;
}

static int g_pack_tokens = -1;
bool text_token_packing() {
  static const bool env_on = []() { const char* e = getenv("CMH_TEXT_PACK_TOKENS"); return !(e && !strcmp(e, "0")); }();
  return g_pack_tokens < 0 ? env_on : g_pack_tokens != 0;
}

struct TowerRun : Lane {
  TowerBufs t;
  bool packed_tokens = false;
};
static void lane_in_place(TowerRun& r) {
  r.x_in = r.x_mid = r.x_out = r.t.x;
  r.h1 = r.attn = r.h2 = r.t.h;
  r.qkv = r.t.qkv;
  r.act = r.t.mlp;
}
static void pool_the_tail(TowerRun& r) {
  char* scratch = static_cast<char*>(r.t.qkv);
  r.pooled = r.t.rows;
  r.x_mid = r.x_out = scratch;
  r.attn_p = r.h2 = scratch + align_up(static_cast<size_t>(r.B) * r.d * 4, 256);
}

namespace {
struct RowsHint { int B = 0, L = 0, hint = -1; int32_t* pinned = nullptr; hipEvent_t ev = nullptr; bool pending = false; };
std::mutex g_hint_mu;
RowsHint g_hint;
}
static int rows_hint_exchange(const int32_t* count_dev, int B, int L, hipStream_t st) {
  std::lock_guard<std::mutex> lk(g_hint_mu);
  RowsHint& h = g_hint;
  if (!h.pinned) {
    if (hipHostMalloc(reinterpret_cast<void**>(&h.pinned), 64, hipHostMallocDefault) != hipSuccess) { h.pinned = nullptr; return -1; }
    if (hipEventCreateWithFlags(&h.ev, hipEventDisableTiming) != hipSuccess) { h.ev = nullptr; return -1; }
  }
  if (!h.ev) return -1;
  if (h.pending && hipEventQuery(h.ev) == hipSuccess) {
    h.pending = false;
    if (h.B == B && h.L == L && *h.pinned > 0 && *h.pinned <= B * L) h.hint = *h.pinned;
  }
  const int out = (h.B == B && h.L == L) ? h.hint : -1;
  if (!h.pending) {
    if (h.B != B || h.L != L) { h.B = B; h.L = L; h.hint = -1; }
    if (hipMemcpyAsync(h.pinned, count_dev, 4, hipMemcpyDeviceToHost, st) == hipSuccess && hipEventRecord(h.ev, st) == hipSuccess) h.pending = true;
  }
  return out;
}

int final_projection(int dt, const void* pool, const void* w_t, float* feat, int B, int embed, int d, hipStream_t st) {
  const int bk = dt == CMH_F32 ? 32 : 64;
  if (embed % 128 == 0 && d % bk == 0) return launch_gemm(dt, pool, w_t, nullptr, nullptr, feat, B, embed, d, 0, st);
  return launch_small_linear(dt, pool, w_t, nullptr, nullptr, 1.f, CMH_ACT_NONE, feat, B, embed, d, st);
}

int resid_f16(int dt, int d) {
  static const bool off = []() { const char* e = getenv("CMH_RESID_F16"); return e && !strcmp(e, "0"); }();
  return dt == CMH_BF16 && d % 256 == 0 && !off;
}
static int tower_xh(int dtb, int d, const cmh_taps* taps) {
  if (taps) return 0;
  return dtb == CMH_FP8 ? d % 256 == 0 : resid_f16(dtb, d);
}

int conv1_stem(const cmh_vit_weights* w, int dt, const float* image, const float* image_b, int batch_a, int B, void* patches,
               void* conv1_w_pad, float* patch_out, hipStream_t st) {
  const int g = w->resolution / w->patch, g2 = g * g, d = w->width;
  const int pk = 3 * w->patch * w->patch, pkp = conv1_k(w->patch, dt);
  const size_t e = dt == CMH_BF16 ? 2 : 4;
  int rc;
  if (image_b) {
    CMH_CHECK_ARG(batch_a > 0 && batch_a < B, "vit_encode: split batch %d of %d", batch_a, B);
    if ((rc = launch_patchify(image, patches, dt, batch_a, w->resolution, w->patch, pkp, st))) return rc;
    if ((rc = launch_patchify(image_b, static_cast<char*>(patches) + static_cast<size_t>(batch_a) * g2 * pkp * e, dt, B - batch_a, w->resolution,
                              w->patch, pkp, st))) return rc;
  } else if ((rc = launch_patchify(image, patches, dt, B, w->resolution, w->patch, pkp, st))) return rc;
  const void* conv1_w = w->conv1_w;
  if (pkp != pk) {
    if ((rc = launch_copy_cols(w->conv1_w, pk, conv1_w_pad, pkp, d, pk, static_cast<int>(e), st))) return rc;
    conv1_w = conv1_w_pad;
  }
  return launch_gemm(dt, patches, conv1_w, nullptr, nullptr, patch_out, B * g2, d, pkp, 0, st);
}

static int check_tower(int dt, int width, int layers, int embed, const cmh_block_weights* blocks) {
  CMH_CHECK_ARG(dt == CMH_F32 || dt == CMH_BF16 || dt == CMH_FP8, "bad gemm_dtype %d", dt);
  CMH_CHECK_ARG(width > 0 && width % 128 == 0 && width <= 1024, "width %d must be a multiple of 128, <= 1024", width);
  CMH_CHECK_ARG(dt != CMH_FP8 || width % 256 == 0, "fp8 mode needs width %% 256 == 0 (width %d)", width);
  CMH_CHECK_ARG(layers >= 0 && embed > 0 && embed % 4 == 0, "bad layers/embed_dim");
  CMH_CHECK_ARG(layers == 0 || blocks, "blocks is null");
  return CMH_OK;
}

}

using namespace cmh;

extern "C" const char* cmh_last_error(void) { return err_buf(); }
extern "C" int cmh_set_pooled_tail(int32_t on) { g_pooled_tail = on ? 1 : 0; return CMH_OK; }
extern "C" int cmh_set_text_token_packing(int32_t on) {
  CMH_CHECK_ARG(on >= -1 && on <= 1, "set_text_token_packing: %d (-1 environment, 0 off, 1 on)", on);
  g_pack_tokens = on;
  return CMH_OK;
}
extern "C" int cmh_version(void) { return CMH_VERSION; }

extern "C" size_t cmh_vit_workspace_bytes(const cmh_vit_weights* w, int32_t batch) {
  if (!w || batch <= 0 || w->patch <= 0) return 0;
  const size_t g = w->resolution / w->patch, g2 = g * g, T = g2 + 1, d = w->width;
  const size_t e = w->gemm_dtype == CMH_F32 ? 4 : 2;
  const size_t B = batch, pk = 3ull * w->patch * w->patch, pkp = conv1_k(w->patch, w->gemm_dtype);
  return carve(nullptr, B * T, B, d, e, B * g2 * d * 4, B * g2 * pkp * e, pkp != pk ? d * pkp * e : 0).total;
}

static int vit_begin(const cmh_vit_weights* w, const float* image, int32_t batch, bool want_out, void* workspace, size_t workspace_bytes,
                     const cmh_taps* taps, hipStream_t st, float* amax, TowerRun& r, const float* image_b = nullptr, int32_t batch_a = 0) {
  CMH_CHECK_ARG(w && image && want_out && workspace, "vit_encode: null pointer");
  CMH_CHECK_ARG(batch > 0, "vit_encode: batch %d", batch);
  int rc = check_tower(w->gemm_dtype, w->width, w->layers, w->embed_dim, w->blocks);
  if (rc) return rc;
  CMH_CHECK_ARG(w->patch > 0 && w->resolution % w->patch == 0, "vit_encode: resolution %d / patch %d", w->resolution, w->patch);
  const int dtb = w->gemm_dtype, d = w->width, B = batch;
  const int dt = dtb == CMH_FP8 ? CMH_BF16 : dtb;
  const int g = w->resolution / w->patch, g2 = g * g, T = g2 + 1, M = B * T;
  const int pk = 3 * w->patch * w->patch, pkp = conv1_k(w->patch, dt);
  const size_t e = dt == CMH_BF16 ? 2 : 4;
  CMH_CHECK_ARG(!amax || dtb == CMH_BF16, "vit_calibrate_fp8: weights must be the bf16 mode's");
  CMH_CHECK_ARG(dtb != CMH_FP8 || pkp == pk, "fp8 mode: patch %d (3*patch^2 = %d) needs the K-padded conv1, which is not built for fp8",
                w->patch, pk);
  const size_t need = cmh_vit_workspace_bytes(w, batch);
  if (workspace_bytes < need) return fail(CMH_ERR_WORKSPACE, "vit_encode: workspace %zu < %zu bytes", workspace_bytes, need);
  CMH_CHECK_ARG((reinterpret_cast<uintptr_t>(workspace) & 255) == 0, "vit_encode: workspace must be 256-byte aligned");
  TowerBufs& t = r.t;
  t = carve(workspace, static_cast<size_t>(M), B, d, e, static_cast<size_t>(B) * g2 * d * 4, static_cast<size_t>(B) * g2 * pkp * e,
            pkp != pk ? static_cast<size_t>(d) * pkp * e : 0);
  r.dtb = dtb; r.xh = tower_xh(dtb, d, taps); r.d = d; r.B = B; r.T = T; r.M = M; r.causal = 0;
  lane_in_place(r);
  float* patch_out = static_cast<float*>(t.qkv);
  if ((rc = conv1_stem(w, dt, image, image_b, batch_a, B, t.mlp, t.conv1_w, patch_out, st))) return rc;
  if ((rc = launch_vit_assemble_lnpre(patch_out, w->class_embedding, w->positional_embedding, w->ln_pre_w,
                                      w->ln_pre_b, t.x, r.xh, B, g2, d, st))) return rc;
  return tap(taps, 0, t.x, static_cast<size_t>(M) * d * 4, st);
}

static int vit_finish(const cmh_vit_weights* w, const TowerRun& r, float* feat, float* tokens_out, hipStream_t st) {
  const TowerBufs& t = r.t;
  const void* x_pooled = r.pooled ? r.x_out : nullptr;
  const int dt = r.dtb == CMH_FP8 ? CMH_BF16 : r.dtb, d = r.d, B = r.B, T = r.T, M = r.M;
  int rc;
  if (tokens_out) {
    if ((rc = launch_layernorm_x(t.x, r.xh, nullptr, w->ln_post_w, w->ln_post_b, t.h, dt == CMH_BF16, M, d, st))) return rc;
    if ((rc = final_projection(dt, t.h, w->proj_t, tokens_out, M, w->embed_dim, d, st))) return rc;
  }
  if (feat) {
    if (x_pooled) {
      if ((rc = launch_layernorm_x(x_pooled, r.xh, nullptr, w->ln_post_w, w->ln_post_b, t.pool, dt == CMH_BF16, B, d, st))) return rc;
    } else {
      if ((rc = launch_iota_rows(t.rows, B, T, st))) return rc;
      if ((rc = launch_layernorm_x(t.x, r.xh, t.rows, w->ln_post_w, w->ln_post_b, t.pool, dt == CMH_BF16, B, d, st))) return rc;
    }
    if ((rc = final_projection(dt, t.pool, w->proj_t, feat, B, w->embed_dim, d, st))) return rc;
  }
  return CMH_OK;
}

static int run_tower(TowerRun& r, const cmh_block_weights* blocks, int layers, bool pool_last, float* amax, const cmh_taps* taps,
                     hipStream_t st) {
  int rc;
  for (int i = 0; i < layers; ++i) {
    r.w = &blocks[i];
    r.amax = amax ? amax + 4 * i : nullptr;
    if (pool_last && i == layers - 1) pool_the_tail(r);
    if ((rc = block_forward(r, nullptr, st))) return rc;
    if ((rc = tap(taps, 1 + i, r.t.x, static_cast<size_t>(r.B) * r.T * r.d * 4, st))) return rc;
  }
  return CMH_OK;
}

static int vit_encode_impl(const cmh_vit_weights* w, const float* image, int32_t batch, float* feat, float* tokens_out,
                           void* workspace, size_t workspace_bytes, const cmh_taps* taps, void* stream, float* amax = nullptr) {
  hipStream_t st = as_stream(stream);
  TowerRun r;
  int rc = vit_begin(w, image, batch, feat || tokens_out, workspace, workspace_bytes, taps, st, amax, r);
  if (rc) return rc;
  const bool tail = feat && !tokens_out && !taps && !amax && w->layers > 0 && pooled_tail_enabled();
  if (tail && (rc = launch_iota_rows(r.t.rows, r.B, r.T, st))) return rc;
  if ((rc = run_tower(r, w->blocks, w->layers, tail, amax, taps, st))) return rc;
  return vit_finish(w, r, feat, tokens_out, st);
}

extern "C" int cmh_vit_encode(const cmh_vit_weights* w, const float* image, int32_t batch, float* feat,
                              void* workspace, size_t workspace_bytes, const cmh_taps* taps, void* stream) {
  CMH_CHECK_ARG(feat, "vit_encode: null pointer");
  return vit_encode_impl(w, image, batch, feat, nullptr, workspace, workspace_bytes, taps, stream);
}

extern "C" int cmh_vit_encode_tokens(const cmh_vit_weights* w, const float* image, int32_t batch, float* tokens_out,
                                     void* workspace, size_t workspace_bytes, void* stream) {
  CMH_CHECK_ARG(tokens_out, "vit_encode_tokens: null pointer");
  return vit_encode_impl(w, image, batch, nullptr, tokens_out, workspace, workspace_bytes, nullptr, stream);
}

extern "C" size_t cmh_text_workspace_bytes(const cmh_text_weights* w, int32_t batch, int32_t seq_len) {
  if (!w || batch <= 0 || seq_len <= 0) return 0;
  const size_t e = w->gemm_dtype == CMH_F32 ? 4 : 2;
  return carve(nullptr, static_cast<size_t>(batch) * seq_len, batch, w->width, e, 0, 0).total;
}

static int text_begin(const cmh_text_weights* w, const int64_t* tokens, int32_t batch, int32_t seq_len, const uint8_t* key_padding_mask,
                      bool want_out, bool tokens_wanted, void* workspace, size_t workspace_bytes, const cmh_taps* taps, hipStream_t st,
                      bool packed, int32_t* rows_out, float* amax, TowerRun& r, bool pack_tokens_req = false) {
  CMH_CHECK_ARG(w && tokens && want_out && workspace, "text_encode: null pointer");
  CMH_CHECK_ARG(batch > 0 && seq_len > 0, "text_encode: batch %d seq_len %d", batch, seq_len);
  int rc = check_tower(w->gemm_dtype, w->width, w->layers, w->embed_dim, w->blocks);
  if (rc) return rc;
  CMH_CHECK_ARG(seq_len <= w->context_length, "text_encode: seq_len %d > context_length %d", seq_len, w->context_length);
  const int dtb = w->gemm_dtype, d = w->width, B = batch, L = seq_len, M = B * L;
  const int dt = dtb == CMH_FP8 ? CMH_BF16 : dtb;
  const size_t e = dt == CMH_BF16 ? 2 : 4;
  CMH_CHECK_ARG(!amax || dtb == CMH_BF16, "text_calibrate_fp8: weights must be the bf16 mode's");
  const size_t need = cmh_text_workspace_bytes(w, batch, seq_len);
  if (workspace_bytes < need) return fail(CMH_ERR_WORKSPACE, "text_encode: workspace %zu < %zu bytes", workspace_bytes, need);
  CMH_CHECK_ARG((reinterpret_cast<uintptr_t>(workspace) & 255) == 0, "text_encode: workspace must be 256-byte aligned");
  TowerBufs& t = r.t;
  t = carve(workspace, static_cast<size_t>(M), B, d, e, 0, 0);
  r.xh = tower_xh(dtb, d, taps);
  lane_in_place(r);

  const int32_t* seq_off = nullptr;
  const int32_t* md = nullptr;
  int rows = M, mh = -1;
  const bool pack_tokens = pack_tokens_req && tokens_wanted && key_padding_mask && !packed && !taps && !amax && text_token_packing() &&
                           w->embed_dim % 128 == 0 && d % (dt == CMH_F32 ? 32 : 64) == 0 &&
                           static_cast<size_t>(w->embed_dim) * 4 <= static_cast<size_t>(4) * d * e;
  r.packed_tokens = pack_tokens;
  if (packed || pack_tokens) {
    CMH_CHECK_ARG(pack_tokens || (!key_padding_mask && !tokens_wanted && !taps), "text_encode_packed: pooled features only, no mask / taps");
    if ((rc = launch_text_pack_plan(tokens, B, L, t.seq, st, pack_tokens ? key_padding_mask : nullptr, pack_tokens ? t.rows : nullptr))) return rc;
    seq_off = t.seq;
    if (amax || d % 256 != 0 || !gemm_wide_enabled()) {
      int32_t total = 0;
      if (hipMemcpyAsync(&total, t.seq + B, 4, hipMemcpyDeviceToHost, st) != hipSuccess || hipStreamSynchronize(st) != hipSuccess)
        return fail(CMH_ERR_LAUNCH, "text_encode_packed: reading the packed row count failed");
      CMH_CHECK_ARG(total > 0 && total <= M, "text_encode_packed: bad packed row count %d", total);
      rows = total;
    } else {
      md = t.seq + B;
      mh = rows_hint_exchange(t.seq + B, B, L, st);
    }
    if (packed && rows_out && hipMemcpyAsync(rows_out, t.seq + B, 4, hipMemcpyDeviceToDevice, st) != hipSuccess)
      return fail(CMH_ERR_LAUNCH, "text_encode_packed: copying the row count failed");
  }

  r.dtb = dtb; r.d = d; r.B = B; r.T = L; r.M = rows; r.causal = 1; r.kpm = key_padding_mask; r.seq_off = seq_off; r.md = md; r.mh = mh;
  return launch_text_embed_packed(tokens, w->token_embedding, w->positional_embedding, t.x, r.xh, t.rows, B, L, d, w->vocab_size, seq_off, st,
                                  pack_tokens);
}

static int text_finish(const cmh_text_weights* w, const TowerRun& r, float* feat, float* tokens_out, int32_t* eot_rows_out, hipStream_t st) {
  const TowerBufs& t = r.t;
  const void* x_pooled = r.pooled ? r.x_out : nullptr;
  const int dt = r.dtb == CMH_FP8 ? CMH_BF16 : r.dtb, d = r.d, B = r.B, M = r.B * r.T;
  int rc;
  if (tokens_out && r.packed_tokens) {
    float* tmp = static_cast<float*>(t.mlp);
    if ((rc = launch_layernorm_x(t.x, r.xh, nullptr, w->ln_final_w, w->ln_final_b, t.h, dt == CMH_BF16, r.M, d, st, r.md))) return rc;
    if ((rc = launch_gemm(dt, t.h, w->text_projection_t, nullptr, nullptr, tmp, r.M, w->embed_dim, d, 0, st, r.md, r.mh))) return rc;
    if ((rc = launch_unpack_token_rows(tmp, r.seq_off, tokens_out, B, r.T, w->embed_dim, t.rows, eot_rows_out, st))) return rc;
  } else if (tokens_out) {
    if ((rc = launch_layernorm_x(t.x, r.xh, nullptr, w->ln_final_w, w->ln_final_b, t.h, dt == CMH_BF16, M, d, st))) return rc;
    if ((rc = final_projection(dt, t.h, w->text_projection_t, tokens_out, M, w->embed_dim, d, st))) return rc;
  }
  if (eot_rows_out && !(tokens_out && r.packed_tokens) &&
      hipMemcpyAsync(eot_rows_out, t.rows, static_cast<size_t>(B) * 4, hipMemcpyDeviceToDevice, st) != hipSuccess)
    return fail(CMH_ERR_LAUNCH, "text_encode: eot row copy failed");
  if (feat) {
    if ((rc = launch_layernorm_x(x_pooled ? x_pooled : t.x, r.xh, x_pooled ? nullptr : t.rows, w->ln_final_w, w->ln_final_b, t.pool,
                                 dt == CMH_BF16, B, d, st))) return rc;
    if ((rc = final_projection(dt, t.pool, w->text_projection_t, feat, B, w->embed_dim, d, st))) return rc;
  }
  return CMH_OK;
}

static int text_encode_impl(const cmh_text_weights* w, const int64_t* tokens, int32_t batch, int32_t seq_len,
                            const uint8_t* key_padding_mask, float* feat, float* tokens_out, int32_t* eot_rows_out,
                            void* workspace, size_t workspace_bytes, const cmh_taps* taps, void* stream,
                            bool packed = false, int32_t* rows_out = nullptr, float* amax = nullptr, bool pack_tokens_req = false) {
  hipStream_t st = as_stream(stream);
  TowerRun r;
  int rc = text_begin(w, tokens, batch, seq_len, key_padding_mask, feat || tokens_out, tokens_out != nullptr, workspace, workspace_bytes,
                      taps, st, packed, rows_out, amax, r, pack_tokens_req);
  if (rc) return rc;
  const bool tail = feat && !tokens_out && !taps && !amax && !eot_rows_out && w->layers > 0 && pooled_tail_enabled();
  if ((rc = run_tower(r, w->blocks, w->layers, tail, amax, taps, st))) return rc;
  return text_finish(w, r, feat, tokens_out, eot_rows_out, st);
}

extern "C" int cmh_text_encode(const cmh_text_weights* w, const int64_t* tokens, int32_t batch, int32_t seq_len,
                               const uint8_t* key_padding_mask, float* feat, void* workspace,
                               size_t workspace_bytes, const cmh_taps* taps, void* stream) {
  CMH_CHECK_ARG(feat, "text_encode: null pointer");
  return text_encode_impl(w, tokens, batch, seq_len, key_padding_mask, feat, nullptr, nullptr, workspace,
                          workspace_bytes, taps, stream);
}

extern "C" int cmh_text_encode_packed(const cmh_text_weights* w, const int64_t* tokens, int32_t batch, int32_t seq_len, float* feat,
                                      int32_t* rows_computed_dev, void* workspace, size_t workspace_bytes, void* stream) {
  CMH_CHECK_ARG(feat, "text_encode_packed: null pointer");
  return text_encode_impl(w, tokens, batch, seq_len, nullptr, feat, nullptr, nullptr, workspace, workspace_bytes, nullptr, stream,
                          true, rows_computed_dev);
}

static int clip_encode_pair_impl(const cmh_vit_weights* vw, const float* image, const float* image_b, int32_t batch_a,
                                 const cmh_text_weights* tw, const int64_t* tokens,
                                 int32_t batch, int32_t seq_len, int32_t packed, float* feat_image, float* feat_text,
                                 int32_t* rows_computed_dev, void* ws_image, size_t ws_image_bytes, void* ws_text,
                                 size_t ws_text_bytes, void* stream) {
  CMH_CHECK_ARG(vw && tw && feat_image && feat_text, "clip_encode_pair: null pointer");
  CMH_CHECK_ARG(vw->gemm_dtype == tw->gemm_dtype, "clip_encode_pair: both towers must run in one arithmetic mode (%d / %d)", vw->gemm_dtype,
                tw->gemm_dtype);
  hipStream_t st = as_stream(stream);
  TowerRun a, b;
  int rc;
  if ((rc = vit_begin(vw, image, batch, true, ws_image, ws_image_bytes, nullptr, st, nullptr, a, image_b, batch_a))) return rc;
  if ((rc = text_begin(tw, tokens, batch, seq_len, nullptr, true, false, ws_text, ws_text_bytes, nullptr, st, packed != 0, rows_computed_dev,
                       nullptr, b))) return rc;
  const bool tail = pooled_tail_enabled();
  if (tail && vw->layers > 0 && (rc = launch_iota_rows(a.t.rows, a.B, a.T, st))) return rc;
  const int deepest = vw->layers > tw->layers ? vw->layers : tw->layers;
  for (int i = 0; i < deepest; ++i) {
    const bool has_a = i < vw->layers, has_b = i < tw->layers;
    const bool last_a = tail && i == vw->layers - 1, last_b = tail && i == tw->layers - 1;
    if (has_a) a.w = &vw->blocks[i];
    if (has_b) b.w = &tw->blocks[i];
    if (last_a) pool_the_tail(a);
    if (last_b) pool_the_tail(b);
    if (has_a && has_b && last_a == last_b && a.xh == b.xh) {
      if ((rc = block_forward(a, &b, st))) return rc;
      continue;
    }
    if (has_a && (rc = block_forward(a, nullptr, st))) return rc;
    if (has_b && (rc = block_forward(b, nullptr, st))) return rc;
  }
  if ((rc = vit_finish(vw, a, feat_image, nullptr, st))) return rc;
  return text_finish(tw, b, feat_text, nullptr, nullptr, st);
}

extern "C" int cmh_clip_encode_pair(const cmh_vit_weights* vw, const float* image, const cmh_text_weights* tw, const int64_t* tokens,
                                    int32_t batch, int32_t seq_len, int32_t packed, float* feat_image, float* feat_text,
                                    int32_t* rows_computed_dev, void* ws_image, size_t ws_image_bytes, void* ws_text,
                                    size_t ws_text_bytes, void* stream) {
  return clip_encode_pair_impl(vw, image, nullptr, 0, tw, tokens, batch, seq_len, packed, feat_image, feat_text, rows_computed_dev, ws_image,
                               ws_image_bytes, ws_text, ws_text_bytes, stream);
}

extern "C" int cmh_clip_encode_pair2(const cmh_vit_weights* vw, const float* image_a, int32_t batch_a, const float* image_b, int32_t batch_b,
                                     const cmh_text_weights* tw, const int64_t* tokens, int32_t seq_len, int32_t packed,
                                     float* feat_image, float* feat_text, int32_t* rows_computed_dev, void* ws_image,
                                     size_t ws_image_bytes, void* ws_text, size_t ws_text_bytes, void* stream) {
  CMH_CHECK_ARG(image_a && image_b && batch_a > 0 && batch_b > 0, "clip_encode_pair2: two non-empty batches");
  return clip_encode_pair_impl(vw, image_a, image_b, batch_a, tw, tokens, batch_a + batch_b, seq_len, packed, feat_image, feat_text,
                               rows_computed_dev, ws_image, ws_image_bytes, ws_text, ws_text_bytes, stream);
}

extern "C" int cmh_linear_gemm_grouped(int32_t dtype, const cmh_gemm_problem* pa, const cmh_gemm_problem* pb, int32_t epilogue, void* stream) {
  CMH_CHECK_ARG(pa && pb, "linear_gemm_grouped: null pointer");
  CMH_CHECK_ARG(dtype == CMH_F32 || dtype == CMH_BF16 || dtype == CMH_FP8, "linear_gemm_grouped: bad dtype %d", dtype);
  auto conv = [](const cmh_gemm_problem* g) {
    return GemmProblem{g->x, g->w, g->bias, static_cast<const float*>(g->residual), g->out, g->M, g->N, g->K, g->m_dev, -1, g->colscale,
                       g->alpha, g->out_scale > 0.f ? 1.0f / g->out_scale : 1.0f};
  };
  for (const cmh_gemm_problem* g : {pa, pb})
    CMH_CHECK_ARG(g->x && g->w && g->out && g->M > 0 && g->N > 0 && g->K > 0, "linear_gemm_grouped: null pointer / empty problem");
  return launch_gemm_grouped(dtype, conv(pa), conv(pb), epilogue, as_stream(stream));
}

extern "C" int cmh_vit_calibrate_fp8(const cmh_vit_weights* w, const float* image, int32_t batch, float* feat, float* amax,
                                     void* workspace, size_t workspace_bytes, void* stream) {
  CMH_CHECK_ARG(feat && amax, "vit_calibrate_fp8: null pointer");
  return vit_encode_impl(w, image, batch, feat, nullptr, workspace, workspace_bytes, nullptr, stream, amax);
}

extern "C" int cmh_text_calibrate_fp8(const cmh_text_weights* w, const int64_t* tokens, int32_t batch, int32_t seq_len, float* feat,
                                      float* amax, void* workspace, size_t workspace_bytes, void* stream) {
  CMH_CHECK_ARG(feat && amax, "text_calibrate_fp8: null pointer");
  return text_encode_impl(w, tokens, batch, seq_len, nullptr, feat, nullptr, nullptr, workspace, workspace_bytes, nullptr, stream,
                          true, nullptr, amax);
}

extern "C" int cmh_text_encode_tokens(const cmh_text_weights* w, const int64_t* tokens, int32_t batch, int32_t seq_len,
                                      const uint8_t* key_padding_mask, float* tokens_out, int32_t* eot_rows_out,
                                      void* workspace, size_t workspace_bytes, void* stream) {
  CMH_CHECK_ARG(tokens_out, "text_encode_tokens: null pointer");
  return text_encode_impl(w, tokens, batch, seq_len, key_padding_mask, nullptr, tokens_out, eot_rows_out, workspace,
                          workspace_bytes, nullptr, stream);
}

extern "C" int cmh_text_encode_tokens_packed(const cmh_text_weights* w, const int64_t* tokens, int32_t batch, int32_t seq_len,
                                             const uint8_t* key_padding_mask, float* tokens_out, int32_t* eot_rows_out,
                                             void* workspace, size_t workspace_bytes, void* stream) {
  CMH_CHECK_ARG(tokens_out, "text_encode_tokens_packed: null pointer");
  return text_encode_impl(w, tokens, batch, seq_len, key_padding_mask, nullptr, tokens_out, eot_rows_out, workspace,
                          workspace_bytes, nullptr, stream, false, nullptr, nullptr, true);
}

extern "C" size_t cmh_blocks_workspace_bytes(int32_t dtype, int32_t B, int32_t T, int32_t d) {
  if (B <= 0 || T <= 0 || d <= 0) return 0;
  return carve(nullptr, static_cast<size_t>(B) * T, B, d, dtype == CMH_BF16 ? 2 : 4, 0, 0).total;
}

extern "C" int cmh_transformer_blocks(const cmh_block_weights* blocks, int32_t layers, int32_t dtype, float* x, int32_t B,
                                      int32_t T, int32_t d, int32_t causal, const uint8_t* key_padding_mask,
                                      void* workspace, size_t workspace_bytes, void* stream) {
  CMH_CHECK_ARG(blocks && x && workspace && layers > 0 && B > 0 && T > 0, "transformer_blocks: bad arguments");
  CMH_CHECK_ARG(dtype != CMH_FP8, "transformer_blocks: f32 / bf16 only (the fp8 mode runs on the towers' fp16 residual stream)");
  int rc = check_tower(dtype, d, layers, 4, blocks);
  if (rc) return rc;
  if (workspace_bytes < cmh_blocks_workspace_bytes(dtype, B, T, d)) return fail(CMH_ERR_WORKSPACE, "transformer_blocks: workspace too small");
  hipStream_t st = as_stream(stream);
  const size_t M = static_cast<size_t>(B) * T;
  TowerRun r;
  r.t = carve(workspace, M, B, d, dtype == CMH_BF16 ? 2 : 4, 0, 0);
  r.dtb = dtype; r.d = d; r.B = B; r.T = T; r.M = B * T; r.causal = causal; r.kpm = key_padding_mask;
  lane_in_place(r);
  if (hipMemcpyAsync(r.t.x, x, M * d * 4, hipMemcpyDeviceToDevice, st) != hipSuccess) return fail(CMH_ERR_LAUNCH, "transformer_blocks: copy failed");
  if ((rc = run_tower(r, blocks, layers, false, nullptr, nullptr, st))) return rc;
  if (hipMemcpyAsync(x, r.t.x, M * d * 4, hipMemcpyDeviceToDevice, st) != hipSuccess) return fail(CMH_ERR_LAUNCH, "transformer_blocks: copy failed");
  return CMH_OK;
}

extern "C" int cmh_linear_gemm(int32_t dtype, const void* x, const void* w, const float* bias, const float* residual,
                               void* out, int32_t M, int32_t N, int32_t K, int32_t epilogue, void* stream) {
  CMH_CHECK_ARG(x && w && out, "linear_gemm: null pointer");
  return launch_gemm(dtype, x, w, bias, residual, out, M, N, K, epilogue, as_stream(stream));
}

extern "C" int cmh_layernorm(const float* x, const float* w, const float* b, void* out, int32_t out_dtype, int32_t M,
                             int32_t d, void* stream) {
  CMH_CHECK_ARG(x && w && b && out && M > 0, "layernorm: bad arguments");
  return launch_layernorm(x, nullptr, w, b, out, out_dtype == CMH_BF16, M, d, as_stream(stream));
}

extern "C" int cmh_attention(int32_t dtype, const void* qkv, void* o, int32_t B, int32_t T, int32_t d, int32_t causal,
                             const uint8_t* key_padding_mask, void* stream) {
  CMH_CHECK_ARG(qkv && o, "attention: null pointer");
  CMH_CHECK_ARG(dtype == CMH_F32 || dtype == CMH_BF16, "attention: bad dtype");
  return launch_attention(qkv, o, dtype, B, T, d, causal, key_padding_mask, as_stream(stream));
}
```

### clip-based-cross-modal-hashing_amd/csrc/norm_embed.hip

```cpp
#include "cmh_common.h"

namespace cmh {

__device__ __forceinline__ float wave_sum(float v) {
#pragma unroll
  for (int o = 32; o > 0; o >>= 1) v += __shfl_xor(v, o, 64);
  return v;
}

constexpr int kMaxVec = 4;
constexpr int kOutF32 = 0, kOutBf16 = 1, kOutF16 = 2;

__device__ __forceinline__ void ln_row(float4 (&v)[kMaxVec], int nv, int d, int lane, const float* __restrict__ w,
                                       const float* __restrict__ b, void* __restrict__ out_row, int out_kind) {
  float s = 0.f;
#pragma unroll
  for (int j = 0; j < kMaxVec; ++j)
    if (j < nv && lane * 4 + 256 * j < d) s += (v[j].x + v[j].y) + (v[j].z + v[j].w);
  const float mean = wave_sum(s) / static_cast<float>(d);
  float ss = 0.f;
#pragma unroll
  for (int j = 0; j < kMaxVec; ++j)
    if (j < nv && lane * 4 + 256 * j < d) {
      const float a = v[j].x - mean, bb = v[j].y - mean, c = v[j].z - mean, e = v[j].w - mean;
      ss += (a * a + bb * bb) + (c * c + e * e);
    }
  const float rstd = 1.0f / sqrtf(wave_sum(ss) / static_cast<float>(d) + 1e-5f);
#pragma unroll
  for (int j = 0; j < kMaxVec; ++j) {
    const int e0 = lane * 4 + 256 * j;
    if (j < nv && e0 < d) {
      const float4 wv = *reinterpret_cast<const float4*>(w + e0);
      const float4 bv = *reinterpret_cast<const float4*>(b + e0);
      float4 y;
      y.x = (v[j].x - mean) * rstd * wv.x + bv.x;
      y.y = (v[j].y - mean) * rstd * wv.y + bv.y;
      y.z = (v[j].z - mean) * rstd * wv.z + bv.z;
      y.w = (v[j].w - mean) * rstd * wv.w + bv.w;
      if (out_kind == kOutBf16) {
        uint2 pk;
        pk.x = static_cast<uint32_t>(f32_to_bf16(y.x)) | (static_cast<uint32_t>(f32_to_bf16(y.y)) << 16);
        pk.y = static_cast<uint32_t>(f32_to_bf16(y.z)) | (static_cast<uint32_t>(f32_to_bf16(y.w)) << 16);
        *reinterpret_cast<uint2*>(static_cast<bf16_t*>(out_row) + e0) = pk;
      } else if (out_kind == kOutF16) {
        *reinterpret_cast<uint2*>(static_cast<uint16_t*>(out_row) + e0) = uint2{pack_f16x2(y.x, y.y), pack_f16x2(y.z, y.w)};
      } else {
        *reinterpret_cast<float4*>(static_cast<float*>(out_row) + e0) = y;
      }
    }
  }
}

template <bool XH>
__device__ __forceinline__ float4 load_x4(const void* row, int e0) {
  if constexpr (XH) {
    const uint2 u = *reinterpret_cast<const uint2*>(static_cast<const uint16_t*>(row) + e0);
    return float4{f16lo_to_f32(u.x), f16hi_to_f32(u.x), f16lo_to_f32(u.y), f16hi_to_f32(u.y)};
  } else {
    return *reinterpret_cast<const float4*>(static_cast<const float*>(row) + e0);
  }
}

template <bool XH>
__global__ __launch_bounds__(256) void layernorm_kernel(const void* __restrict__ x, const int32_t* __restrict__ row_index,
                                                        const float* __restrict__ w, const float* __restrict__ b,
                                                        void* __restrict__ out, int out_kind, int M, int d,
                                                        const int32_t* __restrict__ m_dev) {
  const int lane = threadIdx.x & 63;
  const int row = blockIdx.x * 4 + (threadIdx.x >> 6);
  if (m_dev) { const int md = *m_dev; M = md < M ? md : M; }
  if (row >= M) return;
  const size_t src = row_index ? static_cast<size_t>(row_index[row]) : static_cast<size_t>(row);
  const char* xr = static_cast<const char*>(x) + src * d * (XH ? 2 : 4);
  const int nv = (d + 255) / 256;
  float4 v[kMaxVec];
#pragma unroll
  for (int j = 0; j < kMaxVec; ++j) {
    const int e0 = lane * 4 + 256 * j;
    v[j] = (j < nv && e0 < d) ? load_x4<XH>(xr, e0) : float4{0.f, 0.f, 0.f, 0.f};
  }
  char* orow = static_cast<char*>(out) + static_cast<size_t>(row) * d * (out_kind == kOutF32 ? 4 : 2);
  ln_row(v, nv, d, lane, w, b, orow, out_kind);
}

template <int NB>
__device__ __forceinline__ void layernorm_h2b_rows(const uint16_t* __restrict__ x, const int32_t* __restrict__ row_index,
                                                   const float* __restrict__ w, const float* __restrict__ b,
                                                   uint16_t* __restrict__ out, int M, const int32_t* __restrict__ m_dev, int block) {
  constexpr int d = NB * 256;
  if (m_dev) { const int md = *m_dev; M = md < M ? md : M; }
  constexpr int RPH = NB <= 2 ? 2 : 1;
  const int hl = threadIdx.x & 31;
  typedef __attribute__((ext_vector_type(4))) uint32_t u4;
  const int row0 = (block * 8 + (threadIdx.x >> 5)) * RPH;
  if (row0 >= M) return;
  float v[RPH][NB][8];
#pragma unroll
  for (int r = 0; r < RPH; ++r) {
    const int row = row0 + r < M ? row0 + r : M - 1;
    const size_t src = row_index ? static_cast<size_t>(row_index[row]) : static_cast<size_t>(row);
    const uint16_t* xr = x + src * d;
#pragma unroll
    for (int j = 0; j < NB; ++j) {
      const u4 u = *reinterpret_cast<const u4*>(xr + j * 256 + hl * 8);
#pragma unroll
      for (int k = 0; k < 4; ++k) { v[r][j][2 * k] = f16lo_to_f32(u[k]); v[r][j][2 * k + 1] = f16hi_to_f32(u[k]); }
    }
  }
  auto half_sum = [](float t) {
#pragma unroll
    for (int o = 16; o > 0; o >>= 1) t += __shfl_xor(t, o, 64);
    return t;
  };
#pragma unroll
  for (int r = 0; r < RPH; ++r) {
    const int row = row0 + r;
    float s = 0.f;
#pragma unroll
    for (int j = 0; j < NB; ++j)
#pragma unroll
      for (int k = 0; k < 8; ++k) s += v[r][j][k];
    const float mean = half_sum(s) / static_cast<float>(d);
    float ss = 0.f;
#pragma unroll
    for (int j = 0; j < NB; ++j)
#pragma unroll
      for (int k = 0; k < 8; ++k) { const float c = v[r][j][k] - mean; ss += c * c; }
    const float rstd = 1.0f / sqrtf(half_sum(ss) / static_cast<float>(d) + 1e-5f);
    if (row >= M) continue;
    uint16_t* orow = out + static_cast<size_t>(row) * d;
#pragma unroll
    for (int j = 0; j < NB; ++j) {
      const int e0 = j * 256 + hl * 8;
      const float4 w0 = *reinterpret_cast<const float4*>(w + e0), w1 = *reinterpret_cast<const float4*>(w + e0 + 4);
      const float4 b0 = *reinterpret_cast<const float4*>(b + e0), b1 = *reinterpret_cast<const float4*>(b + e0 + 4);
      const float wv[8] = {w0.x, w0.y, w0.z, w0.w, w1.x, w1.y, w1.z, w1.w};
      const float bv[8] = {b0.x, b0.y, b0.z, b0.w, b1.x, b1.y, b1.z, b1.w};
      u4 pk;
#pragma unroll
      for (int k = 0; k < 4; ++k)
        pk[k] = pack_bf16x2((v[r][j][2 * k] - mean) * rstd * wv[2 * k] + bv[2 * k],
                            (v[r][j][2 * k + 1] - mean) * rstd * wv[2 * k + 1] + bv[2 * k + 1]);
      *reinterpret_cast<u4*>(orow + e0) = pk;
    }
  }
}

template <int NB>
__global__ __launch_bounds__(256) void layernorm_h2b_kernel(const uint16_t* __restrict__ x, const int32_t* __restrict__ row_index,
                                                            const float* __restrict__ w, const float* __restrict__ b,
                                                            uint16_t* __restrict__ out, int M, const int32_t* __restrict__ m_dev) {
  layernorm_h2b_rows<NB>(x, row_index, w, b, out, M, m_dev, blockIdx.x);
}

struct LnRows { const uint16_t* x; const float* w; const float* b; uint16_t* out; int M; const int32_t* m_dev; };
template <int NB0, int NB1>
__global__ __launch_bounds__(256) void layernorm_h2b_pair_kernel(LnRows r0, LnRows r1, int blocks0) {
  if (static_cast<int>(blockIdx.x) < blocks0) layernorm_h2b_rows<NB0>(r0.x, nullptr, r0.w, r0.b, r0.out, r0.M, r0.m_dev, blockIdx.x);
  else layernorm_h2b_rows<NB1>(r1.x, nullptr, r1.w, r1.b, r1.out, r1.M, r1.m_dev, blockIdx.x - blocks0);
}

int launch_layernorm_h2b_pair(const void* x0, const float* w0, const float* b0, void* out0, int M0, int d0, const int32_t* md0,
                               const void* x1, const float* w1, const float* b1, void* out1, int M1, int d1, const int32_t* md1,
                               hipStream_t st) {
  static const bool off = []() { const char* e = getenv("CMH_PAIR_KERNELS"); return e && e[0] == '0'; }();
  if (off || M0 <= 0 || M1 <= 0) return 1;
  const LnRows r0{static_cast<const uint16_t*>(x0), w0, b0, static_cast<uint16_t*>(out0), M0, md0};
  const LnRows r1{static_cast<const uint16_t*>(x1), w1, b1, static_cast<uint16_t*>(out1), M1, md1};
  auto blocks = [](int M, int d) { return d <= 512 ? (M + 15) / 16 : (M + 7) / 8; };
  const int bl0 = blocks(M0, d0), bl1 = blocks(M1, d1);
  const dim3 grid(bl0 + bl1), block(256);
  if (d0 == 768 && d1 == 512) hipLaunchKernelGGL((layernorm_h2b_pair_kernel<3, 2>), grid, block, 0, st, r0, r1, bl0);
  else if (d0 == 768 && d1 == 768) hipLaunchKernelGGL((layernorm_h2b_pair_kernel<3, 3>), grid, block, 0, st, r0, r1, bl0);
  else if (d0 == 1024 && d1 == 768) hipLaunchKernelGGL((layernorm_h2b_pair_kernel<4, 3>), grid, block, 0, st, r0, r1, bl0);
  else if (d0 == 1024 && d1 == 512) hipLaunchKernelGGL((layernorm_h2b_pair_kernel<4, 2>), grid, block, 0, st, r0, r1, bl0);
  else if (d0 == 512 && d1 == 512) hipLaunchKernelGGL((layernorm_h2b_pair_kernel<2, 2>), grid, block, 0, st, r0, r1, bl0);
  else return 1;
  CMH_CHECK_LAUNCH("layernorm (pair)");
  return CMH_OK;
}

int launch_layernorm_x(const void* x, int x_f16, const int32_t* row_index, const float* w, const float* b, void* out,
                       int out_bf16, int M, int d, hipStream_t st, const int32_t* m_dev) {
  CMH_CHECK_ARG(d % 4 == 0 && d <= 256 * kMaxVec, "layernorm: d=%d must be a multiple of 4 and <= 1024", d);
  if (x_f16 && out_bf16 && d % 256 == 0) {
    const uint16_t* xh = static_cast<const uint16_t*>(x);
    uint16_t* oh = static_cast<uint16_t*>(out);
    const dim3 grid((M + 7) / 8), grid2((M + 15) / 16), block(256);
    switch (d / 256) {
      case 1: hipLaunchKernelGGL(layernorm_h2b_kernel<1>, grid2, block, 0, st, xh, row_index, w, b, oh, M, m_dev); break;
      case 2: hipLaunchKernelGGL(layernorm_h2b_kernel<2>, grid2, block, 0, st, xh, row_index, w, b, oh, M, m_dev); break;
      case 3: hipLaunchKernelGGL(layernorm_h2b_kernel<3>, grid, block, 0, st, xh, row_index, w, b, oh, M, m_dev); break;
      default: hipLaunchKernelGGL(layernorm_h2b_kernel<4>, grid, block, 0, st, xh, row_index, w, b, oh, M, m_dev); break;
    }
    CMH_CHECK_LAUNCH("layernorm");
    return CMH_OK;
  }
  if (x_f16)
    hipLaunchKernelGGL(layernorm_kernel<true>, dim3((M + 3) / 4), dim3(256), 0, st, x, row_index, w, b, out, out_bf16, M, d, m_dev);
  else
    hipLaunchKernelGGL(layernorm_kernel<false>, dim3((M + 3) / 4), dim3(256), 0, st, x, row_index, w, b, out, out_bf16, M, d, m_dev);
  CMH_CHECK_LAUNCH("layernorm");
  return CMH_OK;
}

int launch_layernorm(const float* x, const int32_t* row_index, const float* w, const float* b, void* out,
                     int out_bf16, int M, int d, hipStream_t st) {
  return launch_layernorm_x(x, 0, row_index, w, b, out, out_bf16, M, d, st, nullptr);
}

int launch_layernorm_any(const void* x, int x_kind, const int32_t* row_index, const float* w, const float* b, void* out,
                         int out_kind, int M, int d, hipStream_t st) {
  CMH_CHECK_ARG(d % 4 == 0 && d <= 256 * kMaxVec, "layernorm: d=%d must be a multiple of 4 and <= 1024", d);
  CMH_CHECK_ARG((x_kind == 0 || x_kind == 2) && out_kind >= 0 && out_kind <= 2, "layernorm: bad kinds %d -> %d", x_kind, out_kind);
  if (x_kind == 2)
    hipLaunchKernelGGL(layernorm_kernel<true>, dim3((M + 3) / 4), dim3(256), 0, st, x, row_index, w, b, out, out_kind, M, d, nullptr);
  else
    hipLaunchKernelGGL(layernorm_kernel<false>, dim3((M + 3) / 4), dim3(256), 0, st, x, row_index, w, b, out, out_kind, M, d, nullptr);
  CMH_CHECK_LAUNCH("layernorm");
  return CMH_OK;
}

__global__ __launch_bounds__(256) void vit_assemble_kernel(const float* __restrict__ patch_out, const float* __restrict__ cls,
                                                           const float* __restrict__ pos, float* __restrict__ x, int B, int g2,
                                                           int d) {
  const int T = g2 + 1;
  const size_t total4 = static_cast<size_t>(B) * T * d / 4;
  for (size_t i = static_cast<size_t>(blockIdx.x) * 256 + threadIdx.x; i < total4; i += static_cast<size_t>(gridDim.x) * 256) {
    const size_t e = i * 4;
    const int c = static_cast<int>(e % d);
    const size_t row = e / d;
    const int b = static_cast<int>(row / T), t = static_cast<int>(row - static_cast<size_t>(b) * T);
    const float4 a = *reinterpret_cast<const float4*>(t == 0 ? cls + c : patch_out + (static_cast<size_t>(b) * g2 + (t - 1)) * d + c);
    const float4 q = *reinterpret_cast<const float4*>(pos + static_cast<size_t>(t) * d + c);
    *reinterpret_cast<float4*>(x + e) = float4{a.x + q.x, a.y + q.y, a.z + q.z, a.w + q.w};
  }
}

int launch_vit_assemble(const float* patch_out, const float* cls, const float* pos, float* x, int B, int g2, int d, hipStream_t st) {
  CMH_CHECK_ARG(d % 4 == 0, "vit_assemble: width %d unsupported", d);
  const size_t total4 = static_cast<size_t>(B) * (g2 + 1) * d / 4;
  const size_t blocks = (total4 + 255) / 256;
  hipLaunchKernelGGL(vit_assemble_kernel, dim3(static_cast<unsigned>(blocks < 8192 ? blocks : 8192)), dim3(256), 0, st, patch_out, cls,
                     pos, x, B, g2, d);
  CMH_CHECK_LAUNCH("vit_assemble");
  return CMH_OK;
}

__global__ __launch_bounds__(256) void patchify_kernel(const float* __restrict__ image, void* __restrict__ patches,
                                                       int out_bf16, int B, int R, int p) {
  const int g = R / p;
  const size_t total4 = static_cast<size_t>(B) * 3 * R * R / 4;
  for (size_t i = static_cast<size_t>(blockIdx.x) * blockDim.x + threadIdx.x; i < total4;
       i += static_cast<size_t>(gridDim.x) * blockDim.x) {
    const size_t e = i * 4;
    const int x = static_cast<int>(e % R);
    const int y = static_cast<int>((e / R) % R);
    const int c = static_cast<int>((e / (static_cast<size_t>(R) * R)) % 3);
    const int b = static_cast<int>(e / (static_cast<size_t>(R) * R * 3));
    const int gx = x / p, px = x % p, gy = y / p, py = y % p;
    const float4 v = *reinterpret_cast<const float4*>(image + e);
    const size_t row = (static_cast<size_t>(b) * g + gy) * g + gx;
    const size_t col = (static_cast<size_t>(c) * p + py) * p + px;
    const size_t o = row * (3 * p * p) + col;
    if (out_bf16) {
      uint2 pk;
      pk.x = static_cast<uint32_t>(f32_to_bf16(v.x)) | (static_cast<uint32_t>(f32_to_bf16(v.y)) << 16);
      pk.y = static_cast<uint32_t>(f32_to_bf16(v.z)) | (static_cast<uint32_t>(f32_to_bf16(v.w)) << 16);
      *reinterpret_cast<uint2*>(static_cast<bf16_t*>(patches) + o) = pk;
    } else {
      *reinterpret_cast<float4*>(static_cast<float*>(patches) + o) = v;
    }
  }
}

__global__ __launch_bounds__(256) void patchify_any_kernel(const float* __restrict__ image, void* __restrict__ patches, int out_bf16,
                                                           int B, int R, int p, int ld) {
  const int g = R / p, pk = 3 * p * p, pad = ld - pk;
  const size_t pixels = static_cast<size_t>(B) * 3 * R * R;
  const size_t total = pixels + static_cast<size_t>(B) * g * g * pad;
  for (size_t i = static_cast<size_t>(blockIdx.x) * blockDim.x + threadIdx.x; i < total;
       i += static_cast<size_t>(gridDim.x) * blockDim.x) {
    size_t o;
    float v = 0.f;
    if (i < pixels) {
      const int x = static_cast<int>(i % R);
      const size_t r = i / R;
      const int y = static_cast<int>(r % R), c = static_cast<int>((r / R) % 3);
      const size_t b = r / (static_cast<size_t>(R) * 3);
      v = image[i];
      o = ((b * g + y / p) * g + x / p) * ld + static_cast<size_t>(c * p + y % p) * p + x % p;
    } else {
      const size_t j = i - pixels;
      o = (j / pad) * ld + pk + j % pad;
    }
    if (out_bf16) static_cast<bf16_t*>(patches)[o] = f32_to_bf16(v);
    else static_cast<float*>(patches)[o] = v;
  }
}

int launch_patchify(const float* image, void* patches, int dt, int B, int R, int p, int ld, hipStream_t st) {
  CMH_CHECK_ARG(p > 0 && R % p == 0 && ld >= 3 * p * p, "patchify: resolution %d / patch %d / row stride %d unsupported", R, p, ld);
  if (p % 4 == 0 && ld == 3 * p * p) {
    const size_t total4 = static_cast<size_t>(B) * 3 * R * R / 4;
    const int blocks = static_cast<int>(total4 / 256 + 1 < 4096 ? total4 / 256 + 1 : 4096);
    hipLaunchKernelGGL(patchify_kernel, dim3(blocks), dim3(256), 0, st, image, patches, dt == CMH_BF16, B, R, p);
  } else {
    const size_t g = R / p, total = static_cast<size_t>(B) * 3 * R * R + static_cast<size_t>(B) * g * g * (ld - 3 * p * p);
    const int blocks = static_cast<int>(total / 256 + 1 < 8192 ? total / 256 + 1 : 8192);
    hipLaunchKernelGGL(patchify_any_kernel, dim3(blocks), dim3(256), 0, st, image, patches, dt == CMH_BF16, B, R, p, ld);
  }
  CMH_CHECK_LAUNCH("patchify");
  return CMH_OK;
}

template <typename E>
__global__ __launch_bounds__(256) void copy_cols_kernel(const E* __restrict__ src, int lds, E* __restrict__ dst, int ldd, int rows,
                                                        int cols) {
  const size_t total = static_cast<size_t>(rows) * ldd;
  for (size_t i = static_cast<size_t>(blockIdx.x) * blockDim.x + threadIdx.x; i < total;
       i += static_cast<size_t>(gridDim.x) * blockDim.x) {
    const size_t r = i / ldd;
    const int c = static_cast<int>(i % ldd);
    dst[i] = c < cols ? src[r * lds + c] : E(0);
  }
}

int launch_copy_cols(const void* src, int lds, void* dst, int ldd, int rows, int cols, int esz, hipStream_t st) {
  CMH_CHECK_ARG((esz == 2 || esz == 4) && rows > 0 && cols > 0 && cols <= lds && cols <= ldd, "copy_cols: bad shape");
  const size_t total = static_cast<size_t>(rows) * ldd;
  const int blocks = static_cast<int>(total / 256 + 1 < 4096 ? total / 256 + 1 : 4096);
  if (esz == 2)
    hipLaunchKernelGGL(copy_cols_kernel<uint16_t>, dim3(blocks), dim3(256), 0, st, static_cast<const uint16_t*>(src), lds,
                       static_cast<uint16_t*>(dst), ldd, rows, cols);
  else
    hipLaunchKernelGGL(copy_cols_kernel<uint32_t>, dim3(blocks), dim3(256), 0, st, static_cast<const uint32_t*>(src), lds,
                       static_cast<uint32_t*>(dst), ldd, rows, cols);
  CMH_CHECK_LAUNCH("copy_cols");
  return CMH_OK;
}

__global__ __launch_bounds__(256) void vit_assemble_lnpre_kernel(const float* __restrict__ patch_out,
                                                                 const float* __restrict__ cls,
                                                                 const float* __restrict__ pos,
                                                                 const float* __restrict__ lnw,
                                                                 const float* __restrict__ lnb, void* __restrict__ x,
                                                                 int x_f16, int B, int g2, int d) {
  const int lane = threadIdx.x & 63;
  const int T = g2 + 1;
  const int row = blockIdx.x * 4 + (threadIdx.x >> 6);
  if (row >= B * T) return;
  const int b = row / T, t = row - b * T;
  const float* src = t == 0 ? cls : patch_out + (static_cast<size_t>(b) * g2 + (t - 1)) * d;
  const float* pr = pos + static_cast<size_t>(t) * d;
  const int nv = (d + 255) / 256;
  float4 v[kMaxVec];
#pragma unroll
  for (int j = 0; j < kMaxVec; ++j) {
    const int e0 = lane * 4 + 256 * j;
    if (j < nv && e0 < d) {
      const float4 a = *reinterpret_cast<const float4*>(src + e0);
      const float4 q = *reinterpret_cast<const float4*>(pr + e0);
      v[j] = float4{a.x + q.x, a.y + q.y, a.z + q.z, a.w + q.w};
    } else {
      v[j] = float4{0.f, 0.f, 0.f, 0.f};
    }
  }
  ln_row(v, nv, d, lane, lnw, lnb, static_cast<char*>(x) + static_cast<size_t>(row) * d * (x_f16 ? 2 : 4),
         x_f16 ? kOutF16 : kOutF32);
}

int launch_vit_assemble_lnpre(const float* patch_out, const float* cls, const float* pos, const float* lnw,
                              const float* lnb, void* x, int x_f16, int B, int g2, int d, hipStream_t st) {
  CMH_CHECK_ARG(d % 4 == 0 && d <= 256 * kMaxVec, "vit_assemble: width %d unsupported", d);
  const int rows = B * (g2 + 1);
  hipLaunchKernelGGL(vit_assemble_lnpre_kernel, dim3((rows + 3) / 4), dim3(256), 0, st, patch_out, cls, pos, lnw,
                     lnb, x, x_f16, B, g2, d);
  CMH_CHECK_LAUNCH("vit_assemble_lnpre");
  return CMH_OK;
}

__global__ __launch_bounds__(256) void text_embed_kernel(const int64_t* __restrict__ tokens,
                                                         const float* __restrict__ tok_emb,
                                                         const float* __restrict__ pos, void* __restrict__ x,
                                                         int x_f16, int32_t* __restrict__ eot_row, int B, int L, int d,
                                                         int vocab, const int32_t* __restrict__ seq_off, int eot_is_pos) {
  const int lane = threadIdx.x & 63;
  int row = blockIdx.x * 4 + (threadIdx.x >> 6);
  if (row >= B * L) return;
  const int b = row / L, t = row - b * L;
  if (seq_off) {
    if (t >= seq_off[b + 1] - seq_off[b]) return;
    if (t == 0 && lane == 0) eot_row[b] = eot_is_pos ? seq_off[b] + eot_row[b] : seq_off[b + 1] - 1;
  }
  const int orow = seq_off ? seq_off[b] + t : row;
  int64_t id = tokens[row];
  id = id < 0 ? 0 : (id >= vocab ? vocab - 1 : id);
  const float* er = tok_emb + static_cast<size_t>(id) * d;
  const float* pr = pos + static_cast<size_t>(t) * d;
  char* xr = static_cast<char*>(x) + static_cast<size_t>(orow) * d * (x_f16 ? 2 : 4);
  for (int e0 = lane * 4; e0 < d; e0 += 256) {
    const float4 a = *reinterpret_cast<const float4*>(er + e0);
    const float4 q = *reinterpret_cast<const float4*>(pr + e0);
    const float4 y = float4{a.x + q.x, a.y + q.y, a.z + q.z, a.w + q.w};
    if (x_f16)
      *reinterpret_cast<uint2*>(reinterpret_cast<uint16_t*>(xr) + e0) = uint2{pack_f16x2(y.x, y.y), pack_f16x2(y.z, y.w)};
    else
      *reinterpret_cast<float4*>(reinterpret_cast<float*>(xr) + e0) = y;
  }
  if (t == 0 && !seq_off) {
    int64_t best = INT64_MIN;
    int besti = 0;
    for (int i = lane; i < L; i += 64) {
      const int64_t v = tokens[static_cast<size_t>(b) * L + i];
      if (v > best) { best = v; besti = i; }
    }
#pragma unroll
    for (int o = 32; o > 0; o >>= 1) {
      const int64_t ov = __shfl_xor(best, o, 64);
      const int oi = __shfl_xor(besti, o, 64);
      if (ov > best || (ov == best && oi < besti)) { best = ov; besti = oi; }
    }
    if (lane == 0) eot_row[b] = b * L + besti;
  }
}

__global__ __launch_bounds__(256) void text_pack_plan_kernel(const int64_t* __restrict__ tokens, int B, int L,
                                                             int32_t* __restrict__ seq_off, const uint8_t* __restrict__ kpm,
                                                             int32_t* __restrict__ eot_pos) {
  __shared__ int wsum[4];
  __shared__ int carry;
  const int tid = threadIdx.x, lane = tid & 63, wave = tid >> 6;
  if (tid == 0) carry = 0;
  __syncthreads();
  for (int base = 0; base < B; base += 256) {
    const int b = base + tid;
    int len = 0;
    if (b < B) {
      const int64_t* row = tokens + static_cast<size_t>(b) * L;
      long long best = INT64_MIN;
      int besti = 0;
      for (int i0 = 0; i0 < L; i0 += 16) {
        long long v[16];
#pragma unroll
        for (int u = 0; u < 16; ++u) v[u] = i0 + u < L ? row[i0 + u] : INT64_MIN;
#pragma unroll
        for (int u = 0; u < 16; ++u)
          if (v[u] > best) { best = v[u]; besti = i0 + u; }
      }
      len = besti + 1;
      if (kpm) {
        const uint8_t* mrow = kpm + static_cast<size_t>(b) * L;
        int last = -1;
        for (int i0 = 0; i0 < L; i0 += 16) {
          uint8_t m[16];
#pragma unroll
          for (int u = 0; u < 16; ++u) m[u] = i0 + u < L ? mrow[i0 + u] : 1;
#pragma unroll
          for (int u = 0; u < 16; ++u)
            if (!m[u]) last = i0 + u;
        }
        len = last + 1 > len ? last + 1 : len;
      }
      if (eot_pos) eot_pos[b] = besti;
    }
    int v = len;
#pragma unroll
    for (int o = 1; o < 64; o <<= 1) {
      const int t = __shfl_up(v, o, 64);
      if (lane >= o) v += t;
    }
    if (lane == 63) wsum[wave] = v;
    __syncthreads();
    int before = carry;
    for (int w = 0; w < wave; ++w) before += wsum[w];
    if (b < B) seq_off[b + 1] = before + v;
    __syncthreads();
    if (tid == 255) carry = before + v;
    __syncthreads();
// ... 149 lines not shown
```

### include/cmh.h

```cpp
#ifndef CMH_H_
#define CMH_H_

#include <stddef.h>
#include <stdint.h>

#ifdef __cplusplus
extern "C" {
#endif

#define CMH_VERSION 6

typedef enum cmh_status {
  CMH_OK = 0,
  CMH_ERR_INVALID = -1,
  CMH_ERR_WORKSPACE = -2,
  CMH_ERR_LAUNCH = -3,
  CMH_ERR_DATA = -4
} cmh_status;

typedef enum cmh_dtype { CMH_F32 = 0, CMH_BF16 = 1, CMH_FP8 = 2 } cmh_dtype;

const char* cmh_last_error(void);
int cmh_version(void);

typedef struct cmh_block_weights {
  const void* in_proj_w;
  const float* in_proj_b;
  const void* out_proj_w;
  const float* out_proj_b;
  const float* ln1_w;
  const float* ln1_b;
  const float* ln2_w;
  const float* ln2_b;
  const void* fc_w;
  const float* fc_b;
  const void* proj_w;
  const float* proj_b;
  const float* in_proj_cs;
  const float* out_proj_cs;
  const float* fc_cs;
  const float* proj_cs;
  float act_scale[4];
} cmh_block_weights;

typedef struct cmh_vit_weights {
  int32_t gemm_dtype;
  int32_t resolution;
  int32_t patch;
  int32_t width;
  int32_t layers;
  int32_t embed_dim;
  const void* conv1_w;
  const float* class_embedding;
  const float* positional_embedding;
  const float* ln_pre_w;  const float* ln_pre_b;
  const float* ln_post_w; const float* ln_post_b;
  const void* proj_t;
  const cmh_block_weights* blocks;
} cmh_vit_weights;

typedef struct cmh_text_weights {
  int32_t gemm_dtype;
  int32_t context_length;
  int32_t vocab_size;
  int32_t width;
  int32_t layers;
  int32_t embed_dim;
  const float* token_embedding;
  const float* positional_embedding;
  const float* ln_final_w; const float* ln_final_b;
  const void* text_projection_t;
  const cmh_block_weights* blocks;
} cmh_text_weights;

typedef struct cmh_taps {
  float* const* ptrs;
  int32_t count;
} cmh_taps;

size_t cmh_vit_workspace_bytes(const cmh_vit_weights* w, int32_t batch);
size_t cmh_text_workspace_bytes(const cmh_text_weights* w, int32_t batch, int32_t seq_len);

int cmh_vit_encode(const cmh_vit_weights* w, const float* image, int32_t batch, float* feat,
                   void* workspace, size_t workspace_bytes, const cmh_taps* taps, void* stream);

int cmh_text_encode(const cmh_text_weights* w, const int64_t* tokens, int32_t batch, int32_t seq_len,
                    const uint8_t* key_padding_mask, float* feat, void* workspace,
                    size_t workspace_bytes, const cmh_taps* taps, void* stream);

int cmh_vit_calibrate_fp8(const cmh_vit_weights* w, const float* image, int32_t batch, float* feat, float* amax, void* workspace,
                          size_t workspace_bytes, void* stream);
int cmh_text_calibrate_fp8(const cmh_text_weights* w, const int64_t* tokens, int32_t batch, int32_t seq_len, float* feat,
                           float* amax, void* workspace, size_t workspace_bytes, void* stream);

int cmh_text_encode_packed(const cmh_text_weights* w, const int64_t* tokens, int32_t batch, int32_t seq_len, float* feat,
                           int32_t* rows_computed_dev, void* workspace, size_t workspace_bytes, void* stream);
int cmh_clip_encode_pair(const cmh_vit_weights* vw, const float* image, const cmh_text_weights* tw, const int64_t* tokens,
                         int32_t batch, int32_t seq_len, int32_t packed, float* feat_image, float* feat_text,
                         int32_t* rows_computed_dev, void* ws_image, size_t ws_image_bytes, void* ws_text, size_t ws_text_bytes,
                         void* stream);
int cmh_clip_encode_pair2(const cmh_vit_weights* vw, const float* image_a, int32_t batch_a, const float* image_b, int32_t batch_b,
                          const cmh_text_weights* tw, const int64_t* tokens, int32_t seq_len, int32_t packed,
                          float* feat_image, float* feat_text, int32_t* rows_computed_dev, void* ws_image,
                          size_t ws_image_bytes, void* ws_text, size_t ws_text_bytes, void* stream);

#define CMH_EPI_BIAS 1
#define CMH_EPI_QUICKGELU 2
#define CMH_EPI_RESIDUAL 4
#define CMH_EPI_OUT_BF16 8
int cmh_linear_gemm(int32_t dtype, const void* x, const void* w, const float* bias, const float* residual,
                    void* out, int32_t M, int32_t N, int32_t K, int32_t epilogue, void* stream);
int cmh_layernorm(const float* x, const float* w, const float* b, void* out, int32_t out_dtype, int32_t M,
                  int32_t d, void* stream);
typedef struct cmh_gemm_problem {
  const void* x;
  const void* w;
  const float* bias;
  const void* residual;
  void* out;
  int32_t M, N, K;
  const int32_t* m_dev;
  const float* colscale;
  float alpha;
  float out_scale;
} cmh_gemm_problem;
int cmh_linear_gemm_grouped(int32_t dtype, const cmh_gemm_problem* a, const cmh_gemm_problem* b, int32_t epilogue, void* stream);
int cmh_set_gemm_grouped(int32_t on);
int cmh_attention(int32_t dtype, const void* qkv, void* o, int32_t B, int32_t T, int32_t d, int32_t causal,
                  const uint8_t* key_padding_mask, void* stream);

int cmh_prof_gemm_begin(int32_t max_launches);
int cmh_prof_gemm_end(double* total_ms, double* total_flops, int64_t* launches);
int cmh_prof_gemm_by_kernel(double* ms3, double* flops3, int64_t* launches3);

int cmh_gemm_tuning(int32_t tile_rows, int32_t order_group);
int cmh_set_gemm_rows(int32_t on);
int cmh_set_gemm_lc(int32_t mode);
int cmh_gemm_route(int32_t dt, int32_t Ma, int32_t Na, int32_t Ka, int32_t Mb, int32_t Nb, int32_t Kb, int32_t epi);
int cmh_gemm_plan(int32_t dt, int32_t epi, const int32_t* a5, const int32_t* b5, int32_t* out16);

int cmh_set_pooled_tail(int32_t on);

int cmh_set_grad_stream16(int32_t on);

int cmh_set_text_token_packing(int32_t on);

#define CMH_EPI_OUT_FP8 4096
#define CMH_FP8_MAX 448.0f

int cmh_fp8_quantize_weight(const float* w, void* w_fp8, float* colscale, int32_t N, int32_t K, void* stream);
int cmh_fp8_quantize(const void* x, int32_t kind, void* x_fp8, int64_t n, float scale, void* stream);
int cmh_fp8_dequantize(const void* x_fp8, float* out, int64_t n, float scale, void* stream);
int cmh_amax(const void* x, int32_t kind, int64_t n, float* amax_inout, void* stream);
int cmh_linear_gemm_fp8(const void* x_fp8, const void* w_fp8, const float* colscale, float alpha, const float* bias,
                        const float* residual, void* out, float out_scale, int32_t M, int32_t N, int32_t K, int32_t epilogue,
                        void* stream);

size_t cmh_qmi_workspace_bytes(int32_t B);
int cmh_qmi_loss(const float* img, const float* txt, const uint32_t* labels_packed, int32_t B, int32_t K, int32_t C, float eps,
                 float* loss, float* sum_d, void* workspace, size_t workspace_bytes, void* stream);
int cmh_qmi_loss_backward(const float* img, const float* txt, const uint32_t* labels_packed, int32_t B, int32_t K, int32_t C,
                          float eps, const float* sum_d, const float* dloss, float* dimg, float* dtxt, void* workspace,
                          size_t workspace_bytes, void* stream);

size_t cmh_msl_workspace_bytes(int32_t B);
int cmh_msl_loss(const float* feats, const float* feat2, const float* labels, int32_t B, int32_t K, int32_t Kl, float* loss,
                 void* workspace, size_t workspace_bytes, void* stream);
int cmh_msl_loss_backward(const float* feats, const float* feat2, const float* labels, int32_t B, int32_t K, int32_t Kl,
                          const float* dloss, float* dfeats, float* dfeat2, void* workspace, size_t workspace_bytes, void* stream);

size_t cmh_spl_workspace_bytes(int32_t B);
int cmh_spl_loss(const float* a, const float* b, const float* labels, int32_t B, int32_t K, int32_t C, float temperature, float delta,
                 float* loss, void* workspace, size_t workspace_bytes, void* stream);
int cmh_spl_loss_backward(const float* a, const float* b, const float* labels, int32_t B, int32_t K, int32_t C, float temperature,
                          float delta, const float* dloss, float* da, float* db, void* workspace, size_t workspace_bytes, void* stream);

int cmh_cast_f32_to_bf16(const float* src, void* dst_bf16, int64_t n, void* stream);

typedef enum cmh_act { CMH_ACT_NONE = 0, CMH_ACT_TANH = 1, CMH_ACT_RELU = 2 } cmh_act;

int cmh_linear_act(const float* x, const float* w, const float* b, const float* drop_mask,
                   float keep_scale, int32_t act, float* y, int32_t M, int32_t N, int32_t K,
                   void* stream);

int cmh_pair_softmax(const float* z, float* p, int32_t M, int32_t K, void* stream);

int cmh_sign_codes(const float* h, float* codes, int64_t n, void* stream);

int cmh_pair_argmax_codes(const float* p, float* codes, int32_t M, int32_t K, void* stream);

int cmh_pack_codes(const float* codes, int64_t n, int32_t bits, uint32_t* sign_plane,
                   uint32_t* nz_plane, int32_t* bad_flag, void* stream);
int cmh_unpack_codes(const uint32_t* sign_plane, const uint32_t* nz_plane, int64_t n, int32_t bits, float* codes, void* stream);
int cmh_pack_labels(const float* labels, int64_t n, int32_t classes, uint32_t* packed,
                    int32_t* bad_flag, void* stream);

int cmh_hamming_dist(const uint32_t* q_sign, const uint32_t* q_nz, const uint32_t* r_sign,
                     const uint32_t* r_nz, int32_t Q, int64_t N, int32_t bits, float* dist,
                     void* stream);

int cmh_calc_neighbor(const uint32_t* la, const uint32_t* lb, int32_t A, int32_t B, int32_t classes,
                      float* sim, void* stream);

typedef enum cmh_tie_order {
  CMH_TIE_REFERENCE = 0,
  CMH_TIE_STABLE = 1
} cmh_tie_order;

size_t cmh_map_workspace_bytes(int32_t Q, int64_t N, int32_t bits, int32_t tie_order);

int cmh_hamming_map(const uint32_t* q_sign, const uint32_t* q_nz, const uint32_t* q_label,
                    const uint32_t* r_sign, const uint32_t* r_nz, const uint32_t* r_label,
                    int32_t Q, int64_t N, int32_t bits, int32_t classes, int64_t topk,
                    int32_t tie_order, int32_t depth_limit_override, float* ap, float* map,
                    int32_t* perm, void* workspace, size_t workspace_bytes, void* stream);
int cmh_map_mean(const float* ap, int32_t Q, float* map, void* stream);

#define CMH_TOPK_MAX 524287
size_t cmh_retrieval_workspace_bytes(int32_t Q, int64_t N, int32_t bits);
int cmh_hamming_hist(const uint32_t* q_sign, const uint32_t* q_nz, const uint32_t* q_label, const uint32_t* r_sign,
                     const uint32_t* r_nz, const uint32_t* r_label, int32_t Q, int64_t N, int32_t bits, int32_t classes,
                     uint32_t* counts, void* workspace, size_t workspace_bytes, void* stream);
int cmh_hamming_topk(const uint32_t* q_sign, const uint32_t* q_nz, const uint32_t* q_label, const uint32_t* r_sign,
                     const uint32_t* r_nz, const uint32_t* r_label, int32_t Q, int64_t N, int32_t bits, int32_t classes,
                     int64_t k, int32_t* idx, float* dist, uint8_t* rel, uint32_t* counts, void* workspace,
                     size_t workspace_bytes, void* stream);
int cmh_hamming_topk_graded(const uint32_t* q_sign, const uint32_t* q_nz, const uint32_t* q_label, const uint32_t* r_sign,
                            const uint32_t* r_nz, const uint32_t* r_label, int32_t Q, int64_t N, int32_t bits, int32_t classes,
                            int64_t k, int32_t* idx, float* dist, uint8_t* rel, uint8_t* grade, uint32_t* counts,
                            void* workspace, size_t workspace_bytes, void* stream);
size_t cmh_label_overlap_workspace_bytes(int32_t Q, int64_t N, int32_t classes);
int cmh_label_overlap_hist(const uint32_t* q_label, const uint32_t* r_label, int32_t Q, int64_t N, int32_t classes,
                           uint32_t* grade_counts, void* workspace, size_t workspace_bytes, void* stream);

size_t cmh_loss_workspace_bytes(int32_t B, int32_t K, int32_t C);

int cmh_dsph_hyp_loss(const float* x, const float* y, const float* label, const float* proxies,
                      int32_t B, int32_t K, int32_t C, float threshold, float alpha, float* loss,
                      void* workspace, size_t workspace_bytes, void* stream);

int cmh_dchmt_loss(const float* img, const float* txt, const float* label, int32_t B, int32_t D,
                   int32_t C, int32_t output_dim, int32_t similarity, int32_t loss_type,
                   float vartheta, float sim_threshold, float* loss, void* workspace,
                   size_t workspace_bytes, void* stream);

int cmh_batchnorm1d_train(const float* x, const float* w, const float* b, float eps, float* y, int32_t B,
                          int32_t d, void* stream);

int cmh_batchnorm1d_update_running(const float* x, float momentum, float* running_mean, float* running_var, int32_t B,
                                   int32_t d, void* stream);
int cmh_batchnorm1d_backward(const float* x, const float* w, float eps, const float* dy, float* dx, float* dw, float* db,
                             int32_t B, int32_t d, void* stream);
int cmh_twdh_loss_backward(const float* p_img, const float* p_txt, const float* target, int32_t B, int32_t K,
                           const float* d_nce, const float* d_quan, float* dp_img, float* dp_txt, void* stream);

int cmh_twdh_targets(const float* label, const float* center, const float* random_center, float* code,
                     int32_t B, int32_t C, int32_t K, void* stream);

int cmh_twdh_loss(const float* p_img, const float* p_txt, const float* target, int32_t B, int32_t K,
                  float* out2, void* workspace, size_t workspace_bytes, void* stream);

int cmh_dnph_loss(const float* hash_img, const float* hash_txt, const float* pre_img, const float* pre_txt,
                  const float* label, const float* proxies, const float* noise_img, const float* noise_txt,
                  int32_t B, int32_t K, int32_t C, float margin, float noise_weight, float* out3,
                  void* workspace, size_t workspace_bytes, void* stream);

#define CMH_EPI_GELU 16
#define CMH_EPI_RELU 32
#define CMH_EPI_RES_F16 64
#define CMH_EPI_OUT_F16 128
#define CMH_EPI_MUL_DQGELU 1024

int cmh_vit_encode_tokens(const cmh_vit_weights* w, const float* image, int32_t batch, float* tokens_out,
                          void* workspace, size_t workspace_bytes, void* stream);
int cmh_text_encode_tokens(const cmh_text_weights* w, const int64_t* tokens, int32_t batch, int32_t seq_len,
                           const uint8_t* key_padding_mask, float* tokens_out, int32_t* eot_rows_out,
                           void* workspace, size_t workspace_bytes, void* stream);
int cmh_text_encode_tokens_packed(const cmh_text_weights* w, const int64_t* tokens, int32_t batch, int32_t seq_len,
                                  const uint8_t* key_padding_mask, float* tokens_out, int32_t* eot_rows_out,
                                  void* workspace, size_t workspace_bytes, void* stream);

size_t cmh_blocks_workspace_bytes(int32_t dtype, int32_t B, int32_t T, int32_t d);
int cmh_transformer_blocks(const cmh_block_weights* blocks, int32_t layers, int32_t dtype, float* x, int32_t B,
                           int32_t T, int32_t d, int32_t causal, const uint8_t* key_padding_mask,
                           void* workspace, size_t workspace_bytes, void* stream);

int cmh_mith_lta(const float* tokens, const float* sim, const uint8_t* key_padding_mask, float* out, int32_t B,
                 int32_t Ltot, int32_t l0, int32_t L, int32_t K, int32_t D, int32_t top_k, void* stream);
int cmh_add_positional(float* x, const float* pe, int32_t B, int32_t T, int32_t D, void* stream);
int cmh_bitwise_hash(const float* x, const float* w, const float* bias, float* out, int32_t B, int32_t K,
                     int32_t D, void* stream);
int cmh_l2_normalize_rows(const float* x, float* y, int32_t R, int32_t D, void* stream);
int cmh_mith_mix(const float* img_cls, const float* img_tok, const float* txt_cls, const float* txt_tok,
                 float hyper_lambda, float* B_codes, float* H_img, float* H_txt, int64_t n, void* stream);
int cmh_sq_diff_sum(const float* a, const float* b, int64_t n, float* out, void* workspace, size_t workspace_bytes,
                    void* stream);
int cmh_mith_bayesian_loss(const float* bank, const float* batch, const float* bank_label, const float* label,
                           int32_t Mb, int32_t B, int32_t K, int32_t C, float* out, void* workspace,
                           size_t workspace_bytes, void* stream);
int cmh_info_nce(const float* a, const float* b, int32_t R, int32_t G, int32_t D, float temperature, float* out,
                 void* workspace, size_t workspace_bytes, void* stream);
size_t cmh_info_nce_workspace_bytes(int32_t R, int32_t G);

typedef struct cmh_adam_tensor {
  float* p; float* g; float* m; float* v;
  int64_t n;
  float lr, weight_decay, max_grad_norm;
  void* p_bf16;
} cmh_adam_tensor;
size_t cmh_bert_adam_workspace_bytes(int32_t count, int64_t total_elems);
int cmh_bert_adam_step(const cmh_adam_tensor* tensors, int32_t count, double b1, double b2, double eps,
                       void* workspace, size_t workspace_bytes, void* stream);

#define CMH_KIND_F32 0
#define CMH_KIND_BF16 1
#define CMH_KIND_F16 2
int cmh_transpose(const void* src, int32_t src_kind, void* dst, int32_t dst_kind, int32_t rows, int32_t cols, void* stream);
size_t cmh_colsum_workspace_bytes(int32_t rows, int32_t cols);
int cmh_colsum(const void* x, int32_t kind, int32_t rows, int32_t cols, float* out, void* workspace, size_t workspace_bytes,
               void* stream);
size_t cmh_layernorm_backward_workspace_bytes(int32_t M, int32_t d);
int cmh_layernorm_backward(const void* x, int32_t x_kind, const void* dy, int32_t dy_kind, const float* gamma, int32_t M,
                           int32_t d, float* dx, int32_t accumulate, float* dgamma, float* dbeta, void* workspace,
                           size_t workspace_bytes, void* stream);
int cmh_attention_backward(int32_t dtype, const void* qkv, const void* o, const void* dout, void* dqkv, int32_t B, int32_t T,
                           int32_t d, int32_t causal, const uint8_t* key_padding_mask, void* stream);
int cmh_quick_gelu(const void* pre, void* out, int64_t n, int32_t kind, void* stream);

typedef struct cmh_block_grads {
  float *in_proj_w, *in_proj_b, *out_proj_w, *out_proj_b, *ln1_w, *ln1_b, *ln2_w, *ln2_b, *fc_w, *fc_b, *proj_w, *proj_b;
} cmh_block_grads;
typedef struct cmh_vit_grads {
  float* conv1_w;
  float* class_embedding;
  float* positional_embedding;
  float *ln_pre_w, *ln_pre_b, *ln_post_w, *ln_post_b;
  float* proj;
  const cmh_block_grads* blocks;
} cmh_vit_grads;
typedef struct cmh_text_grads {
  float* token_embedding;
  float* positional_embedding;
  float *ln_final_w, *ln_final_b;
  float* text_projection;
  const cmh_block_grads* blocks;
} cmh_text_grads;
size_t cmh_linear_wgrad_workspace_bytes(int32_t dtype, int32_t M, int32_t O, int32_t I);
int cmh_linear_wgrad(int32_t dtype, const void* dy, int32_t dy_kind, const void* x, int32_t x_kind, int32_t M, int32_t O,
                     int32_t I, float* dw, float* db, void* workspace, size_t workspace_bytes, void* stream);
int cmh_linear_act_backward(const float* x, const float* w, const float* y, const float* dy, const float* drop_mask,
                            float keep_scale, int32_t act, float* dx, float* dw, float* db, int32_t M, int32_t N, int32_t K,
                            void* workspace, size_t workspace_bytes, void* stream);
size_t cmh_head_backward_workspace_bytes(int32_t B, int32_t K, int32_t C);
int cmh_dsph_hyp_loss_backward(const float* x, const float* y, const float* label, const float* proxies, int32_t B, int32_t K,
                               int32_t C, float threshold, float alpha, const float* dloss, float* dx, float* dy,
                               float* dproxies, void* workspace, size_t workspace_bytes, void* stream);
int cmh_pair_softmax_backward(const float* p, const float* dp, float* dz, int32_t M, int32_t K, void* stream);
int cmh_dchmt_loss_backward(const float* img, const float* txt, const float* label, int32_t B, int32_t D, int32_t C,
                            int32_t output_dim, int32_t similarity, int32_t loss_type, float vartheta, float sim_threshold,
                            const float* dloss, float* dimg, float* dtxt, void* workspace, size_t workspace_bytes, void* stream);
size_t cmh_dnph_backward_workspace_bytes(int32_t B, int32_t K, int32_t C);
int cmh_dnph_loss_backward(const float* hash_img, const float* hash_txt, const float* pre_img, const float* pre_txt,
                           const float* label, const float* proxies, const float* noise_img, const float* noise_txt, int32_t B,
                           int32_t K, int32_t C, float margin, float noise_weight, const float* dloss, float* dhash_img,
                           float* dhash_txt, float* dpre_img, float* dpre_txt, float* dproxies, void* workspace,
                           size_t workspace_bytes, void* stream);
size_t cmh_image_preprocess_workspace_bytes(int32_t batch, int32_t max_h, int32_t max_w, int32_t R);
int cmh_image_preprocess(const uint8_t* pixels, const int64_t* offsets, const int32_t* hw, int32_t batch, int32_t max_h,
                         int32_t max_w, int32_t R, int32_t train, const float* mean, const float* stdv, float* out,
                         uint8_t* out_u8, void* workspace, size_t workspace_bytes, void* stream);

int cmh_image_normalize(const uint8_t* u8, const int64_t* rows, int32_t batch, int32_t R, const float* mean, const float* stdv,
                        float* out, void* stream);

typedef struct cmh_bpe cmh_bpe;
int cmh_bpe_create(const char* merges_utf8, size_t bytes, cmh_bpe** out);
void cmh_bpe_destroy(cmh_bpe* tokenizer);
int32_t cmh_bpe_vocab_size(const cmh_bpe* tokenizer);
int cmh_bpe_encode_captions(const cmh_bpe* tokenizer, const char* texts, const int64_t* offsets, int32_t n, int32_t max_words,
                            int64_t* out, uint8_t* status, int32_t threads);

size_t cmh_vit_train_bytes(const cmh_vit_weights* w, int32_t batch);
int cmh_vit_forward_train(const cmh_vit_weights* w, const float* image, int32_t batch, float* feat, void* tape, size_t tape_bytes,
                          void* stream);
int cmh_vit_backward(const cmh_vit_weights* w, int32_t batch, const float* dfeat, const cmh_vit_grads* grads, void* tape,
                     size_t tape_bytes, void* stream);
int cmh_vit_backward_part(const cmh_vit_weights* w, int32_t batch, const float* dfeat, const cmh_vit_grads* grads, void* tape,
                          size_t tape_bytes, int32_t layer_hi, int32_t layer_lo, void* stream);
int cmh_vit_forward_train_tokens(const cmh_vit_weights* w, const float* image, int32_t batch, float* tokens_out, void* tape,
                                 size_t tape_bytes, void* stream);
int cmh_vit_backward_tokens(const cmh_vit_weights* w, int32_t batch, const float* dtokens, const cmh_vit_grads* grads, void* tape,
                            size_t tape_bytes, void* stream);
size_t cmh_text_train_bytes(const cmh_text_weights* w, int32_t batch, int32_t seq_len);
int cmh_text_forward_train(const cmh_text_weights* w, const int64_t* tokens, int32_t batch, int32_t seq_len,
                           const uint8_t* key_padding_mask, float* feat, void* tape, size_t tape_bytes, void* stream);
int cmh_text_backward(const cmh_text_weights* w, const int64_t* tokens, int32_t batch, int32_t seq_len,
                      const uint8_t* key_padding_mask, const float* dfeat, const cmh_text_grads* grads, void* tape,
                      size_t tape_bytes, void* stream);
int cmh_text_backward_part(const cmh_text_weights* w, const int64_t* tokens, int32_t batch, int32_t seq_len,
                           const uint8_t* key_padding_mask, const float* dfeat, const cmh_text_grads* grads, void* tape,
                           size_t tape_bytes, int32_t layer_hi, int32_t layer_lo, void* stream);

int cmh_text_forward_train_tokens(const cmh_text_weights* w, const int64_t* tokens, int32_t batch, int32_t seq_len,
                                  const uint8_t* key_padding_mask, float* tokens_out, int32_t* eot_rows_out, void* tape,
                                  size_t tape_bytes, void* stream);
int cmh_text_forward_train_tokens_packed(const cmh_text_weights* w, const int64_t* tokens, int32_t batch, int32_t seq_len,
                                         const uint8_t* key_padding_mask, float* tokens_out, int32_t* eot_rows_out, void* tape,
                                         size_t tape_bytes, void* stream);
int cmh_text_backward_tokens(const cmh_text_weights* w, const int64_t* tokens, int32_t batch, int32_t seq_len,
                             const uint8_t* key_padding_mask, const float* dtokens, const cmh_text_grads* grads, void* tape,
                             size_t tape_bytes, void* stream);

size_t cmh_blocks_train_bytes(int32_t dtype, int32_t B, int32_t T, int32_t d, int32_t layers);
int cmh_blocks_forward_train(const cmh_block_weights* blocks, int32_t layers, int32_t dtype, const float* x, float* y, int32_t B,
                             int32_t T, int32_t d, void* tape, size_t tape_bytes, void* stream);
int cmh_blocks_backward(const cmh_block_weights* blocks, const cmh_block_grads* grads, int32_t layers, int32_t dtype,
                        const float* dy, float* dx, int32_t B, int32_t T, int32_t d, void* tape, size_t tape_bytes, void* stream);
int cmh_mith_lta_backward(const float* sim, const uint8_t* key_padding_mask, const float* dmerge, float* dtokens, int32_t B,
                          int32_t Ltot, int32_t l0, int32_t L, int32_t K, int32_t D, int32_t top_k, void* stream);
int cmh_gelu(const float* x, float* y, int64_t n, void* stream);
int cmh_gelu_backward(const float* x, const float* dy, float* dx, int64_t n, void* stream);
int cmh_l2_normalize_backward(const float* x, const float* dy, float* dx, int32_t R, int32_t D, void* stream);
int cmh_bitwise_hash_backward(const float* x, const float* w, const float* y, const float* dy, float* dx, float* dw, float* db,
                              int32_t B, int32_t K, int32_t D, void* stream);

size_t cmh_mith_bayesian_backward_workspace_bytes(int32_t B, int32_t K);
int cmh_mith_bayesian_loss_backward(const float* bank, const float* batch, const float* bank_label, const float* label, int32_t Mb,
                                    int32_t B, int32_t K, int32_t C, const float* dloss, float* dbatch, void* workspace,
                                    size_t workspace_bytes, void* stream);
int cmh_info_nce_backward(const float* a, const float* b, int32_t R, int32_t G, int32_t D, float temperature, const float* dloss,
                          float* da, float* db, void* workspace, size_t workspace_bytes, void* stream);
int cmh_sq_diff_sum_backward(const float* a, const float* b, int64_t n, const float* dloss, float* da, float* db, void* stream);

#ifdef __cplusplus
}
#endif
#endif
```

Baseline: 68360.

## Compute only pooled query rows in last-layer attention and trim padded key tiles

Adds a pooled-query mode to the MFMA attention kernel. In the last block it computes only the query tile holding the pooled row (the CLS token or EOT row) and writes one output row per sequence, gathering the matching residual row in the same pass. A separate trim mode skips key/value tiles that lie beyond the sequence length, are fully padded, or are causally masked, so the kernel does fewer loads and MFMA calls. The pair encoder also fuses the final layernorms of both towers when both are pooled. This adds kernel template variants and extra scratch-buffer reuse, which risks register pressure and correctness errors in edge cases.

Result: no change. 68520 (median of 4 runs) (+0.2%).

```diff
diff --git a/clip-based-cross-modal-hashing_amd/cmh_native.py b/clip-based-cross-modal-hashing_amd/cmh_native.py
--- a/clip-based-cross-modal-hashing_amd/cmh_native.py
+++ b/clip-based-cross-modal-hashing_amd/cmh_native.py
@@ -95,6 +95,9 @@
     "cmh_attention": (C.c_int, [_i32, _p, _p, _i32, _i32, _i32, _i32, _p, _p]),
     "cmh_gemm_tuning": (C.c_int, [_i32, _i32]),
     "cmh_set_pooled_tail": (C.c_int, [_i32]),
+    "cmh_set_pooled_query": (C.c_int, [_i32]),
+    "cmh_set_attention_trim": (C.c_int, [_i32]),
+    "cmh_attention_varlen": (C.c_int, [_i32, _p, _p, _i32, _i32, _i32, _i32, _p, _p, _i32, _p, _p, _p, _i32, _p]),
     "cmh_set_gemm_rows": (C.c_int, [_i32]),
     "cmh_set_gemm_grouped": (C.c_int, [_i32]),
     "cmh_set_gemm_lc": (C.c_int, [_i32]),
@@ -393,6 +396,14 @@
     check(lib().cmh_set_pooled_tail(1 if on else 0), "cmh_set_pooled_tail")
 
 
+def set_pooled_query(on: int):
+    check(lib().cmh_set_pooled_query(int(on)), "cmh_set_pooled_query")
+
+
+def set_attention_trim(on: int):
+    check(lib().cmh_set_attention_trim(int(on)), "cmh_set_attention_trim")
+
+
 def set_gemm_rows(on: int = -1):
     check(lib().cmh_set_gemm_rows(int(on)), "cmh_set_gemm_rows")
 
@@ -502,6 +513,42 @@
     return o
 
 
+def attention_varlen(qkv, B, T, causal, key_padding_mask=None, seq_off=None, pooled_rows=None, out=None, x_src=None, x_out=None):
+    require_gpu(qkv, key_padding_mask, seq_off, pooled_rows, out, x_src, x_out)
+    qkv = qkv.contiguous()
+    dt = BF16 if qkv.dtype == torch.bfloat16 else F32
+    rows, d = qkv.shape[0], qkv.shape[1] // 3
+    kpm = None if key_padding_mask is None else key_padding_mask.to(torch.uint8).contiguous()
+    if seq_off is not None:
+        seq_off = seq_off.to(torch.int32).contiguous()
+        if seq_off.numel() != B + 1:
+            raise NativeError(f"attention_varlen: seq_off holds {seq_off.numel()} offsets for {B} sequences")
+    elif rows != B * T:
+        raise NativeError(f"attention_varlen: {rows} rows for B={B}, T={T}")
+    if pooled_rows is not None:
+        pooled_rows = pooled_rows.to(torch.int32).contiguous()
+        if pooled_rows.numel() != B:
+            raise NativeError(f"attention_varlen: {pooled_rows.numel()} pooled rows for {B} sequences")
+    n_out = B if pooled_rows is not None else rows
+    if out is None:
+        out = torch.empty(n_out, d, dtype=qkv.dtype, device=qkv.device)
+    if out.shape != (n_out, d) or out.dtype != qkv.dtype or not out.is_contiguous():
+        raise NativeError(f"attention_varlen: out must be a contiguous {qkv.dtype} [{n_out}, {d}]")
+    esz = 0
+    if x_src is not None:
+        if pooled_rows is None or x_src.shape != (rows, d) or x_src.dtype not in (torch.float16, torch.float32) or not x_src.is_contiguous():
+            raise NativeError("attention_varlen: x_src goes with pooled_rows and is a contiguous fp16 / f32 [rows, d]")
+        if x_out is None:
+            x_out = torch.empty(B, d, dtype=x_src.dtype, device=x_src.device)
+        if x_out.shape != (B, d) or x_out.dtype != x_src.dtype or not x_out.is_contiguous():
+            raise NativeError("attention_varlen: x_out must be a contiguous [B, d] of x_src's type")
+        esz = x_src.element_size()
+    check(lib().cmh_attention_varlen(dt, ptr(qkv), ptr(out), B, T, d, int(bool(causal)), ptr(kpm), ptr(seq_off),
+                                     int(pooled_rows is not None), ptr(pooled_rows), ptr(x_src), ptr(x_out), esz, stream_ptr(qkv.device)),
+          "cmh_attention_varlen")
+    return (out, x_out) if x_src is not None else out
+
+
 def linear_act(x, w, b, act=ACT_NONE, drop_mask=None, p=0.2):
     x, w = f32c(x), f32c(w)
     b = None if b is None else f32c(b)
diff --git a/clip-based-cross-modal-hashing_amd/csrc/attention.hip b/clip-based-cross-modal-hashing_amd/csrc/attention.hip
--- a/clip-based-cross-modal-hashing_amd/csrc/attention.hip
+++ b/clip-based-cross-modal-hashing_amd/csrc/attention.hip
@@ -1,3 +1,6 @@
+#include <cstdlib>
+#include <cstring>
+
 #include "cmh_common.h"
 
 namespace cmh {
@@ -159,10 +162,18 @@
 
 constexpr int kAttnVST = 80;
 
-template <int NKT>
+struct AttnPool {
+  const int32_t* rows = nullptr;
+  const void* x_src = nullptr;
+  void* x_dst = nullptr;
+  int x_esz = 0;
+};
+
+template <int NKT, int MODE>
 __device__ __forceinline__ void attention_mfma_body(const bf16_t* __restrict__ qkv, bf16_t* __restrict__ o, int Tmax, int d, int causal,
                                                     const uint8_t* __restrict__ kpm, const int32_t* __restrict__ seq_off,
-                                                    float o8_inv_scale, int block, bf16_t* sV) {
+                                                    float o8_inv_scale, int block, bf16_t* sV, const AttnPool& pq) {
+  constexpr bool TRIM = (MODE & 1) != 0, POOL = (MODE & 2) != 0;
   constexpr int NKS = NKT / 2;
   constexpr int TP = NKT * 16;
   constexpr int VST = kAttnVST;
@@ -175,10 +186,26 @@
   const size_t ld = static_cast<size_t>(3) * d;
   const bf16_t* base = qkv + srow * ld + h * HD;
   if (Tn <= 0) return;
+  int prow = 0;
+  uint4 xrow = uint4{0u, 0u, 0u, 0u};
+  if constexpr (POOL) {
+    const long long grow = pq.rows ? static_cast<long long>(__builtin_amdgcn_readfirstlane(pq.rows[b])) : static_cast<long long>(b) * Tmax;
+    const long long loc = grow - static_cast<long long>(srow);
+    if (loc < 0 || loc >= Tn) return;
+    prow = static_cast<int>(loc);
+    if (pq.x_src && lane < 4 * pq.x_esz)
+      xrow = *reinterpret_cast<const uint4*>(static_cast<const char*>(pq.x_src) +
+                                             (static_cast<size_t>(grow) * d + h * HD) * pq.x_esz + lane * 16);
+  }
+  const int nkl = !TRIM ? NKT : (POOL && causal) ? (prow >> 4) + 1 : (Tn + 15) >> 4;
 
   abf16x8_t kf[NKT][2];
 #pragma unroll
   for (int kt = 0; kt < NKT; ++kt) {
+    if (TRIM && kt >= nkl) {
+      kf[kt][0] = kf[kt][1] = abf16x8_t{0, 0, 0, 0, 0, 0, 0, 0};
+      continue;
+    }
     int row = kt * 16 + c;
     row = row < Tn ? row : Tn - 1;
 #pragma unroll
@@ -192,6 +219,10 @@
 #pragma unroll
     for (int i = 0; i < VB; ++i) {
       const int slot = lane + 64 * (i0 + i), row = slot >> 3, ch = slot & 7;
+      if (TRIM && ((i0 + i) >> 1) >= nkl) {
+        vst[i] = uint4{0u, 0u, 0u, 0u};
+        continue;
+      }
       const int rc = row < Tn ? row : Tn - 1;
       vst[i] = *reinterpret_cast<const uint4*>(base + static_cast<size_t>(rc) * ld + 2 * d + ch * 8);
     }
@@ -218,6 +249,10 @@
     for (int kt = 0; kt < NKT; ++kt)
 #pragma unroll
       for (int r = 0; r < 4; ++r) padded |= (kb[kt][r] != 0 ? 1u : 0u) << (kt * 4 + r);
+  }
+  if constexpr (POOL) {
+    if (pq.x_src && lane < 4 * pq.x_esz)
+      *reinterpret_cast<uint4*>(static_cast<char*>(pq.x_dst) + (static_cast<size_t>(b) * d + h * HD) * pq.x_esz + lane * 16) = xrow;
   }
   store_v(0);
   if constexpr (VB < VIT) { load_v(VB); store_v(VB); }
@@ -288,15 +323,22 @@
     for (int s = 0; s < 2; ++s) q[s] = *reinterpret_cast<const abf16x8_t*>(base + static_cast<size_t>(qr) * ld + s * 32 + g * 8);
   };
   abf16x8_t qn[2];
-  load_q(0, qn);
-  for (int qt = 0; qt < nqt; ++qt) {
+  const int qt0 = POOL ? prow >> 4 : 0, qt1 = POOL ? qt0 + 1 : nqt;
+  load_q(qt0, qn);
+  for (int qt = qt0; qt < qt1; ++qt) {
     const int qrow = qt * 16 + c;
     abf16x8_t qf[2] = {qn[0], qn[1]};
-    load_q(qt + 1, qn);
+    uint32_t live = (1u << NKT) - 1u;
+    if constexpr (TRIM) live = __builtin_amdgcn_readfirstlane(live & ~tile_none & (causal ? (2u << qt) - 1u : ~0u));
+    if constexpr (!POOL) {
+      load_q(qt + 1, qn);
+    }
     af32x4_t sc[NKT];
 #pragma unroll
     for (int kt = 0; kt < NKT; ++kt) {
-      if ((causal && kt > qt) || ((tile_none >> kt) & 1u)) {
+      if (TRIM && !((live >> kt) & 1u)) {
+        sc[kt] = af32x4_t{0.f, 0.f, 0.f, 0.f};
+      } else if ((causal && kt > qt) || ((tile_none >> kt) & 1u)) {
         sc[kt] = af32x4_t{-1e30f, -1e30f, -1e30f, -1e30f};
       } else {
         sc[kt] = af32x4_t{0.f, 0.f, 0.f, 0.f};
@@ -312,7 +354,10 @@
     }
     float m = -1e30f;
 #pragma unroll
-    for (int kt = 0; kt < NKT; ++kt) m = fmaxf(fmaxf(m, fmaxf(sc[kt][0], sc[kt][1])), fmaxf(sc[kt][2], sc[kt][3]));
+    for (int kt = 0; kt < NKT; ++kt) {
+      if (TRIM && !((live >> kt) & 1u)) continue;
+      m = fmaxf(fmaxf(m, fmaxf(sc[kt][0], sc[kt][1])), fmaxf(sc[kt][2], sc[kt][3]));
+    }
     m = fmaxf(m, __shfl_xor(m, 16, 64));
     m = fmaxf(m, __shfl_xor(m, 32, 64));
     typedef __attribute__((ext_vector_type(2))) float af32x2_t;
@@ -320,7 +365,8 @@
     const af32x2_t mc = {-m * kC, -m * kC}, cc = {kC, kC};
     af32x2_t l2 = {0.f, 0.f};
 #pragma unroll
-    for (int kt = 0; kt < NKT; ++kt)
+    for (int kt = 0; kt < NKT; ++kt) {
+      if (TRIM && !((live >> kt) & 1u)) continue;
 #pragma unroll
       for (int r = 0; r < 4; r += 2) {
         const af32x2_t e = __builtin_elementwise_fma(af32x2_t{sc[kt][r], sc[kt][r + 1]}, cc, mc);
@@ -329,6 +375,7 @@
         sc[kt][r + 1] = p[1];
         l2 += p;
       }
+    }
     float l = l2[0] + l2[1];
     l += __shfl_xor(l, 16, 64);
     l += __shfl_xor(l, 32, 64);
@@ -338,6 +385,7 @@
     for (int dt = 0; dt < 4; ++dt) oc[dt] = af32x4_t{0.f, 0.f, 0.f, 0.f};
 #pragma unroll
     for (int s = 0; s < NKS; ++s) {
+      if (TRIM && !((live >> (2 * s)) & 3u)) continue;
       abf16x8_t pb;
 #pragma unroll
       for (int j = 0; j < 8; ++j) pb[j] = static_cast<__bf16>(sc[2 * s + (j >> 2)][j & 3]);
@@ -353,19 +401,20 @@
       continue;
     }
 #endif
-    if (qrow < Tn && o8_inv_scale > 0.f) {
+    const bool mine = POOL ? qrow == prow : qrow < Tn;
+    if ((POOL || qrow < Tn) && o8_inv_scale > 0.f) {
       const float inv = o8_inv_scale / l;
-      uint8_t* op8 = reinterpret_cast<uint8_t*>(o) + (srow + qrow) * d + h * HD + 4 * g;
+      uint8_t* op8 = reinterpret_cast<uint8_t*>(o) + (POOL ? static_cast<size_t>(b) : srow + qrow) * d + h * HD + 4 * g;
 #pragma unroll
       for (int dt = 0; dt < 4; ++dt) {
         auto cl = [](float v) { return fminf(fmaxf(v, -448.f), 448.f); };
         int w = __builtin_amdgcn_cvt_pk_fp8_f32(cl(oc[dt][0] * inv), cl(oc[dt][1] * inv), 0, false);
         w = __builtin_amdgcn_cvt_pk_fp8_f32(cl(oc[dt][2] * inv), cl(oc[dt][3] * inv), w, true);
-        *reinterpret_cast<uint32_t*>(op8 + 16 * dt) = static_cast<uint32_t>(w);
+        if (!POOL || mine) *reinterpret_cast<uint32_t*>(op8 + 16 * dt) = static_cast<uint32_t>(w);
       }
     } else {
       const float inv = 1.0f / l;
-      bf16_t* op = o + (srow + (qrow < Tn ? qrow : Tn - 1)) * d + h * HD + (g & 1) * 16 + (g & 2) * 4;
+      bf16_t* op = o + (POOL ? static_cast<size_t>(b) : srow + (qrow < Tn ? qrow : Tn - 1)) * d + h * HD + (g & 1) * 16 + (g & 2) * 4;
 #pragma unroll
       for (int pr = 0; pr < 2; ++pr) {
         uint32_t lo[2], hi[2];
@@ -377,27 +426,51 @@
         typedef __attribute__((ext_vector_type(2))) unsigned au2_t;
         const au2_t s0 = __builtin_amdgcn_permlane16_swap(lo[0], hi[0], false, false);
         const au2_t s1 = __builtin_amdgcn_permlane16_swap(lo[1], hi[1], false, false);
-        if (qrow < Tn) *reinterpret_cast<uint4*>(op + 32 * pr) = uint4{s0[0], s1[0], s0[1], s1[1]};
-      }
-    }
-  }
-}
-
-template <int NKT>
+        if (mine) *reinterpret_cast<uint4*>(op + 32 * pr) = uint4{s0[0], s1[0], s0[1], s1[1]};
+      }
+    }
+  }
+}
+
+template <int NKT, int MODE = 0>
 __global__ __launch_bounds__(64) void attention_mfma_kernel(const bf16_t* __restrict__ qkv, bf16_t* __restrict__ o,
                                                             int B, int Tmax, int d, int causal,
                                                             const uint8_t* __restrict__ kpm,
                                                             const int32_t* __restrict__ seq_off, float o8_inv_scale) {
   __shared__ __attribute__((aligned(16))) bf16_t sV[NKT * 16 * kAttnVST];
   (void)B;
-  attention_mfma_body<NKT>(qkv, o, Tmax, d, causal, kpm, seq_off, o8_inv_scale, blockIdx.x, sV);
+  attention_mfma_body<NKT, MODE>(qkv, o, Tmax, d, causal, kpm, seq_off, o8_inv_scale, blockIdx.x, sV, AttnPool{});
+}
+
+template <int NKT, int MODE>
+__global__ __launch_bounds__(64) void attention_mfma_pooled_kernel(const bf16_t* __restrict__ qkv, bf16_t* __restrict__ o,
+                                                                   int Tmax, int d, int causal, const uint8_t* __restrict__ kpm,
+                                                                   const int32_t* __restrict__ seq_off, float o8_inv_scale, AttnPool pq) {
+  __shared__ __attribute__((aligned(16))) bf16_t sV[NKT * 16 * kAttnVST];
+  attention_mfma_body<NKT, MODE>(qkv, o, Tmax, d, causal, kpm, seq_off, o8_inv_scale, blockIdx.x, sV, pq);
+}
+
+static int g_attn_trim = -1;
+static bool attention_trim_enabled() {
+  static const bool env_on = []() { const char* e = getenv("CMH_ATTN_TRIM"); return !(e && !strcmp(e, "0")); }();
+  return g_attn_trim < 0 ? env_on : g_attn_trim != 0;
 }
 
 template <int NKT>
 static void launch_attention_mfma(const void* qkv, void* o, int B, int T, int d, int causal, const uint8_t* kpm,
-                                  const int32_t* seq_off, hipStream_t st, float o8_inv_scale) {
-  hipLaunchKernelGGL(attention_mfma_kernel<NKT>, dim3(B * (d / HD)), dim3(64), 0, st, static_cast<const bf16_t*>(qkv),
-                     static_cast<bf16_t*>(o), B, T, d, causal, kpm, seq_off, o8_inv_scale);
+                                  const int32_t* seq_off, hipStream_t st, float o8_inv_scale, const AttnPool* pq) {
+  const dim3 grid(B * (d / HD)), block(64);
+  const bf16_t* q = static_cast<const bf16_t*>(qkv);
+  bf16_t* out = static_cast<bf16_t*>(o);
+  const bool trim = attention_trim_enabled();
+  if (pq) {
+    if (trim) hipLaunchKernelGGL((attention_mfma_pooled_kernel<NKT, 3>), grid, block, 0, st, q, out, T, d, causal, kpm, seq_off, o8_inv_scale, *pq);
+    else hipLaunchKernelGGL((attention_mfma_pooled_kernel<NKT, 2>), grid, block, 0, st, q, out, T, d, causal, kpm, seq_off, o8_inv_scale, *pq);
+  } else if (trim) {
+    hipLaunchKernelGGL((attention_mfma_kernel<NKT, 1>), grid, block, 0, st, q, out, B, T, d, causal, kpm, seq_off, o8_inv_scale);
+  } else {
+    hipLaunchKernelGGL((attention_mfma_kernel<NKT, 0>), grid, block, 0, st, q, out, B, T, d, causal, kpm, seq_off, o8_inv_scale);
+  }
 }
 
 int launch_attention(const void* qkv, void* o, int dt, int B, int T, int d, int causal,
@@ -406,16 +479,23 @@
 }
 
 int launch_attention_varlen(const void* qkv, void* o, int dt, int B, int T, int d, int causal,
-                            const uint8_t* key_padding_mask, const int32_t* seq_off, hipStream_t st, float o8_inv_scale) {
+                            const uint8_t* key_padding_mask, const int32_t* seq_off, hipStream_t st, float o8_inv_scale,
+                            int pooled_query, const int32_t* pooled_rows, const void* x_src, void* x_dst, int x_esz) {
   CMH_CHECK_ARG(d % HD == 0, "attention: width %d is not a multiple of 64", d);
   CMH_CHECK_ARG(B > 0 && T > 0, "attention: empty batch");
   CMH_CHECK_ARG(o8_inv_scale == 0.f || (dt == CMH_BF16 && T <= 128), "attention: e4m3 output needs bf16 qkv and T <= 128 (T=%d)", T);
+  CMH_CHECK_ARG(!pooled_query || (dt == CMH_BF16 && T <= 128), "attention: the pooled-query form needs bf16 qkv and T <= 128 (T=%d)", T);
+  CMH_CHECK_ARG(!pooled_query || pooled_rows || !seq_off, "attention: packed sequences need their pooled rows");
+  CMH_CHECK_ARG(!pooled_query || !x_src || (x_dst && x_dst != x_src && (x_esz == 2 || x_esz == 4)),
+                "attention: the pooled residual copy needs a destination and 2- or 4-byte elements");
   const dim3 grid(B * (d / HD), (T + 63) / 64);
   if (dt == CMH_BF16 && T <= 128) {
-    if (T <= 32) launch_attention_mfma<2>(qkv, o, B, T, d, causal, key_padding_mask, seq_off, st, o8_inv_scale);
-    else if (T <= 64) launch_attention_mfma<4>(qkv, o, B, T, d, causal, key_padding_mask, seq_off, st, o8_inv_scale);
-    else if (T <= 96) launch_attention_mfma<6>(qkv, o, B, T, d, causal, key_padding_mask, seq_off, st, o8_inv_scale);
-    else launch_attention_mfma<8>(qkv, o, B, T, d, causal, key_padding_mask, seq_off, st, o8_inv_scale);
+    const AttnPool pool{pooled_rows, x_src, x_dst, x_esz};
+    const AttnPool* pq = pooled_query ? &pool : nullptr;
+    if (T <= 32) launch_attention_mfma<2>(qkv, o, B, T, d, causal, key_padding_mask, seq_off, st, o8_inv_scale, pq);
+    else if (T <= 64) launch_attention_mfma<4>(qkv, o, B, T, d, causal, key_padding_mask, seq_off, st, o8_inv_scale, pq);
+    else if (T <= 96) launch_attention_mfma<6>(qkv, o, B, T, d, causal, key_padding_mask, seq_off, st, o8_inv_scale, pq);
+    else launch_attention_mfma<8>(qkv, o, B, T, d, causal, key_padding_mask, seq_off, st, o8_inv_scale, pq);
     CMH_CHECK_LAUNCH("attention_mfma");
     return CMH_OK;
   }
@@ -430,3 +510,9 @@
 }
 
 }
+
+extern "C" int cmh_set_attention_trim(int32_t on) {
+  CMH_CHECK_ARG(on >= -1 && on <= 1, "set_attention_trim: %d (-1 environment, 0 off, 1 on)", on);
+  cmh::g_attn_trim = on;
+  return CMH_OK;
+}
diff --git a/clip-based-cross-modal-hashing_amd/csrc/cmh_common.h b/clip-based-cross-modal-hashing_amd/csrc/cmh_common.h
--- a/clip-based-cross-modal-hashing_amd/csrc/cmh_common.h
+++ b/clip-based-cross-modal-hashing_amd/csrc/cmh_common.h
@@ -219,7 +219,9 @@
                      const uint8_t* key_padding_mask, hipStream_t st);
 int launch_attention_varlen(const void* qkv, void* o, int dt, int B, int T, int d, int causal,
                             const uint8_t* key_padding_mask, const int32_t* seq_off, hipStream_t st,
-                            float o8_inv_scale = 0.f);
+                            float o8_inv_scale = 0.f,
+                            int pooled_query = 0, const int32_t* pooled_rows = nullptr, const void* x_src = nullptr,
+                            void* x_dst = nullptr, int x_esz = 0);
 int launch_layernorm_q(const void* x_f16, const float* w, const float* b, void* out_fp8, float inv_scale, int M, int d, hipStream_t st,
                        const int32_t* m_dev = nullptr);
 int launch_amax(const void* x, int kind, size_t n, float* out, hipStream_t st);
diff --git a/clip-based-cross-modal-hashing_amd/csrc/encoder_blocks.h b/clip-based-cross-modal-hashing_amd/csrc/encoder_blocks.h
--- a/clip-based-cross-modal-hashing_amd/csrc/encoder_blocks.h
+++ b/clip-based-cross-modal-hashing_amd/csrc/encoder_blocks.h
@@ -29,6 +29,7 @@
   void* pre = nullptr;
   const int32_t* pooled = nullptr;
   void* attn_p = nullptr;
+  int pooled_query = 0;
 };
 
 int block_forward(const Lane& a, const Lane* b, hipStream_t st);
diff --git a/clip-based-cross-modal-hashing_amd/csrc/encoders.hip b/clip-based-cross-modal-hashing_amd/csrc/encoders.hip
--- a/clip-based-cross-modal-hashing_amd/csrc/encoders.hip
+++ b/clip-based-cross-modal-hashing_amd/csrc/encoders.hip
@@ -140,11 +140,17 @@
   for (int i = 0; i < n; ++i) {
     const Lane& l = *L[i];
     const int xe = l.xh ? 2 : 4, e = l.dtb == CMH_FP8 ? 1 : l.dtb == CMH_BF16 ? 2 : 4;
-    if (l.pooled && (rc = launch_gather_rows2(l.x_in, l.x_mid, l.d * xe, l.attn, l.attn_p, l.d * e, l.pooled, l.B, st))) return rc;
-  }
-  if ((rc = gemm_stage(L, n, G_OUT_PROJ, st))) return rc;
+    if (l.pooled && !l.pooled_query && (rc = launch_gather_rows2(l.x_in, l.x_mid, l.d * xe, l.attn, l.attn_p, l.d * e, l.pooled, l.B, st))) return rc;
+  }
+  const bool each = n == 2 && (L[0]->pooled || L[1]->pooled);
+  auto gemms = [&](int which) {
+    if (!each) return gemm_stage(L, n, which, st);
+    const int r0 = gemm_stage(&L[0], 1, which, st);
+    return r0 ? r0 : gemm_stage(&L[1], 1, which, st);
+  };
+  if ((rc = gemms(G_OUT_PROJ))) return rc;
   if ((rc = ln_stage(L, n, OP_LN2, st))) return rc;
-  if ((rc = gemm_stage(L, n, G_FC, st))) return rc;
+  if ((rc = gemms(G_FC))) return rc;
   for (int i = 0; i < n; ++i) {
     const Lane& l = *L[i];
     const size_t n_act = static_cast<size_t>(tail_rows(l).M) * 4 * l.d;
@@ -152,7 +158,7 @@
         (rc = cmh_quick_gelu(l.pre, l.act, static_cast<int64_t>(n_act), l.dtb == CMH_BF16 ? kBF16 : kF32, st))) return rc;
     if ((rc = amax_stage(l, OP_ACT, l.act, n_act, st))) return rc;
   }
-  return gemm_stage(L, n, G_PROJ, st);
+  return gemms(G_PROJ);
 }
 
 int block_forward(const Lane& a, const Lane* b, hipStream_t st) {
@@ -168,13 +174,16 @@
   for (int i = 0; i < n; ++i) {
     const Lane& l = *L[i];
     const bool q = l.dtb == CMH_FP8;
+    if (l.pooled_query) {
+      CMH_CHECK_ARG(l.pooled && !l.amax && l.dtb != CMH_F32 && l.x_mid != l.x_in, "block_forward: the pooled-query attention needs a pooled tail");
+      rc = launch_attention_varlen(l.qkv, l.attn_p, CMH_BF16, l.B, l.T, l.d, l.causal, l.kpm, l.seq_off, st, q ? 1.0f / scale(l, OP_ATTN) : 0.f,
+                                   1, l.pooled_query == 2 ? nullptr : l.pooled, l.x_in, l.x_mid, l.xh ? 2 : 4);
+      if (rc) return rc;
+      continue;
+    }
     if ((rc = launch_attention_varlen(l.qkv, l.attn, q ? CMH_BF16 : l.dtb, l.B, l.T, l.d, l.causal, l.kpm, l.seq_off, st,
                                       q ? 1.0f / scale(l, OP_ATTN) : 0.f))) return rc;
     if ((rc = amax_stage(l, OP_ATTN, l.attn, static_cast<size_t>(l.M) * l.d, st))) return rc;
-  }
-  if (n == 2 && (a.pooled || b->pooled)) {
-    if ((rc = block_tail(&L[0], 1, st))) return rc;
-    return block_tail(&L[1], 1, st);
   }
   return block_tail(L, n, st);
 }
@@ -183,6 +192,12 @@
 bool pooled_tail_enabled() {
   static const bool env_on = []() { const char* e = getenv("CMH_POOLED_TAIL"); return !(e && !strcmp(e, "0")); }();
   return g_pooled_tail < 0 ? env_on : g_pooled_tail != 0;
+}
+
+static int g_pooled_query = -1;
+static bool pooled_query_enabled() {
+  static const bool env_on = []() { const char* e = getenv("CMH_POOLED_QUERY"); return !(e && !strcmp(e, "0")); }();
+  return g_pooled_query < 0 ? env_on : g_pooled_query != 0;
 }
 
 static int g_pack_tokens = -1;
@@ -201,9 +216,14 @@
   r.qkv = r.t.qkv;
   r.act = r.t.mlp;
 }
-static void pool_the_tail(TowerRun& r) {
-  char* scratch = static_cast<char*>(r.t.qkv);
+static bool pooled_query_fits(const TowerRun& r) {
+  const size_t e = 2, need = align_up(static_cast<size_t>(r.B) * r.d * 4, 256) + static_cast<size_t>(r.B) * r.d * e;
+  return pooled_query_enabled() && r.dtb != CMH_F32 && r.T <= 128 && need <= static_cast<size_t>(r.B) * r.T * r.d * e;
+}
+static void pool_the_tail(TowerRun& r, int pooled_query = 0) {
+  char* scratch = static_cast<char*>(pooled_query ? r.t.h : r.t.qkv);
   r.pooled = r.t.rows;
+  r.pooled_query = pooled_query;
   r.x_mid = r.x_out = scratch;
   r.attn_p = r.h2 = scratch + align_up(static_cast<size_t>(r.B) * r.d * 4, 256);
 }
@@ -283,6 +303,11 @@
 
 extern "C" const char* cmh_last_error(void) { return err_buf(); }
 extern "C" int cmh_set_pooled_tail(int32_t on) { g_pooled_tail = on ? 1 : 0; return CMH_OK; }
+extern "C" int cmh_set_pooled_query(int32_t on) {
+  CMH_CHECK_ARG(on >= -1 && on <= 1, "set_pooled_query: %d (-1 environment, 0 off, 1 on)", on);
+  g_pooled_query = on;
+  return CMH_OK;
+}
 extern "C" int cmh_set_text_token_packing(int32_t on) {
   CMH_CHECK_ARG(on >= -1 && on <= 1, "set_text_token_packing: %d (-1 environment, 0 off, 1 on)", on);
   g_pack_tokens = on;
@@ -350,12 +375,12 @@
 }
 
 static int run_tower(TowerRun& r, const cmh_block_weights* blocks, int layers, bool pool_last, float* amax, const cmh_taps* taps,
-                     hipStream_t st) {
+                     hipStream_t st, int pooled_query = 0) {
   int rc;
   for (int i = 0; i < layers; ++i) {
     r.w = &blocks[i];
     r.amax = amax ? amax + 4 * i : nullptr;
-    if (pool_last && i == layers - 1) pool_the_tail(r);
+    if (pool_last && i == layers - 1) pool_the_tail(r, pooled_query);
     if ((rc = block_forward(r, nullptr, st))) return rc;
     if ((rc = tap(taps, 1 + i, r.t.x, static_cast<size_t>(r.B) * r.T * r.d * 4, st))) return rc;
   }
@@ -369,8 +394,9 @@
   int rc = vit_begin(w, image, batch, feat || tokens_out, workspace, workspace_bytes, taps, st, amax, r);
   if (rc) return rc;
   const bool tail = feat && !tokens_out && !taps && !amax && w->layers > 0 && pooled_tail_enabled();
-  if (tail && (rc = launch_iota_rows(r.t.rows, r.B, r.T, st))) return rc;
-  if ((rc = run_tower(r, w->blocks, w->layers, tail, amax, taps, st))) return rc;
+  const int pq = tail && pooled_query_fits(r) ? 2 : 0;
+  if (tail && !pq && (rc = launch_iota_rows(r.t.rows, r.B, r.T, st))) return rc;
+  if ((rc = run_tower(r, w->blocks, w->layers, tail, amax, taps, st, pq))) return rc;
   return vit_finish(w, r, feat, tokens_out, st);
 }
 
@@ -477,7 +503,7 @@
                       taps, st, packed, rows_out, amax, r, pack_tokens_req);
   if (rc) return rc;
   const bool tail = feat && !tokens_out && !taps && !amax && !eot_rows_out && w->layers > 0 && pooled_tail_enabled();
-  if ((rc = run_tower(r, w->blocks, w->layers, tail, amax, taps, st))) return rc;
+  if ((rc = run_tower(r, w->blocks, w->layers, tail, amax, taps, st, tail && pooled_query_fits(r) ? 1 : 0))) return rc;
   return text_finish(w, r, feat, tokens_out, eot_rows_out, st);
 }
 
@@ -511,21 +537,31 @@
   if ((rc = text_begin(tw, tokens, batch, seq_len, nullptr, true, false, ws_text, ws_text_bytes, nullptr, st, packed != 0, rows_computed_dev,
                        nullptr, b))) return rc;
   const bool tail = pooled_tail_enabled();
-  if (tail && vw->layers > 0 && (rc = launch_iota_rows(a.t.rows, a.B, a.T, st))) return rc;
+  const int pq_a = tail && pooled_query_fits(a) ? 2 : 0, pq_b = tail && pooled_query_fits(b) ? 1 : 0;
+  if (tail && !pq_a && vw->layers > 0 && (rc = launch_iota_rows(a.t.rows, a.B, a.T, st))) return rc;
   const int deepest = vw->layers > tw->layers ? vw->layers : tw->layers;
   for (int i = 0; i < deepest; ++i) {
     const bool has_a = i < vw->layers, has_b = i < tw->layers;
     const bool last_a = tail && i == vw->layers - 1, last_b = tail && i == tw->layers - 1;
     if (has_a) a.w = &vw->blocks[i];
     if (has_b) b.w = &tw->blocks[i];
-    if (last_a) pool_the_tail(a);
-    if (last_b) pool_the_tail(b);
+    if (last_a) pool_the_tail(a, pq_a);
+    if (last_b) pool_the_tail(b, pq_b);
     if (has_a && has_b && last_a == last_b && a.xh == b.xh) {
       if ((rc = block_forward(a, &b, st))) return rc;
       continue;
     }
     if (has_a && (rc = block_forward(a, nullptr, st))) return rc;
     if (has_b && (rc = block_forward(b, nullptr, st))) return rc;
+  }
+  if (a.pooled && b.pooled && a.xh && b.xh) {
+    rc = launch_layernorm_h2b_pair(a.x_out, vw->ln_post_w, vw->ln_post_b, a.t.pool, a.B, a.d, nullptr, b.x_out, tw->ln_final_w, tw->ln_final_b,
+                                   b.t.pool, b.B, b.d, nullptr, st);
+    if (rc < 0) return rc;
+    if (rc == 0) {
+      if ((rc = final_projection(CMH_BF16, a.t.pool, vw->proj_t, feat_image, a.B, vw->embed_dim, a.d, st))) return rc;
+      return final_projection(CMH_BF16, b.t.pool, tw->text_projection_t, feat_text, b.B, tw->embed_dim, b.d, st);
+    }
   }
   if ((rc = vit_finish(vw, a, feat_image, nullptr, st))) return rc;
   return text_finish(tw, b, feat_text, nullptr, nullptr, st);
@@ -626,6 +662,15 @@
   return launch_layernorm(x, nullptr, w, b, out, out_dtype == CMH_BF16, M, d, as_stream(stream));
 }
 
+extern "C" int cmh_attention_varlen(int32_t dtype, const void* qkv, void* o, int32_t B, int32_t T, int32_t d, int32_t causal,
+                                    const uint8_t* key_padding_mask, const int32_t* seq_off, int32_t pooled_query, const int32_t* pooled_rows,
+                                    const void* x_src, void* x_dst, int32_t x_elem_bytes, void* stream) {
+  CMH_CHECK_ARG(qkv && o, "attention_varlen: null pointer");
+  CMH_CHECK_ARG(dtype == CMH_F32 || dtype == CMH_BF16, "attention_varlen: bad dtype");
+  return launch_attention_varlen(qkv, o, dtype, B, T, d, causal, key_padding_mask, seq_off, as_stream(stream), 0.f, pooled_query ? 1 : 0,
+                                 pooled_rows, x_src, x_dst, x_elem_bytes);
+}
+
 extern "C" int cmh_attention(int32_t dtype, const void* qkv, void* o, int32_t B, int32_t T, int32_t d, int32_t causal,
                              const uint8_t* key_padding_mask, void* stream) {
   CMH_CHECK_ARG(qkv && o, "attention: null pointer");
diff --git a/clip-based-cross-modal-hashing_amd/csrc/norm_embed.hip b/clip-based-cross-modal-hashing_amd/csrc/norm_embed.hip
--- a/clip-based-cross-modal-hashing_amd/csrc/norm_embed.hip
+++ b/clip-based-cross-modal-hashing_amd/csrc/norm_embed.hip
@@ -175,6 +175,7 @@
   else if (d0 == 1024 && d1 == 768) hipLaunchKernelGGL((layernorm_h2b_pair_kernel<4, 3>), grid, block, 0, st, r0, r1, bl0);
   else if (d0 == 1024 && d1 == 512) hipLaunchKernelGGL((layernorm_h2b_pair_kernel<4, 2>), grid, block, 0, st, r0, r1, bl0);
   else if (d0 == 512 && d1 == 512) hipLaunchKernelGGL((layernorm_h2b_pair_kernel<2, 2>), grid, block, 0, st, r0, r1, bl0);
+  else if (d0 == 256 && d1 == 256) hipLaunchKernelGGL((layernorm_h2b_pair_kernel<1, 1>), grid, block, 0, st, r0, r1, bl0);
   else return 1;
   CMH_CHECK_LAUNCH("layernorm (pair)");
   return CMH_OK;
diff --git a/include/cmh.h b/include/cmh.h
--- a/include/cmh.h
+++ b/include/cmh.h
@@ -128,6 +128,10 @@
 int cmh_set_gemm_grouped(int32_t on);
 int cmh_attention(int32_t dtype, const void* qkv, void* o, int32_t B, int32_t T, int32_t d, int32_t causal,
                   const uint8_t* key_padding_mask, void* stream);
+int cmh_attention_varlen(int32_t dtype, const void* qkv, void* o, int32_t B, int32_t T, int32_t d, int32_t causal,
+                         const uint8_t* key_padding_mask, const int32_t* seq_off, int32_t pooled_query, const int32_t* pooled_rows,
+                         const void* x_src, void* x_dst, int32_t x_elem_bytes, void* stream);
+int cmh_set_attention_trim(int32_t on);
 
 int cmh_prof_gemm_begin(int32_t max_launches);
 int cmh_prof_gemm_end(double* total_ms, double* total_flops, int64_t* launches);
@@ -140,6 +144,7 @@
 int cmh_gemm_plan(int32_t dt, int32_t epi, const int32_t* a5, const int32_t* b5, int32_t* out16);
 
 int cmh_set_pooled_tail(int32_t on);
+int cmh_set_pooled_query(int32_t on);
 
 int cmh_set_grad_stream16(int32_t on);
 
```
